# Sin3DM/Sin3DM

Hardware: AMD Instinct MI355X
Metric: DDPM-1000 triplane samples/sec @128^2 latent (higher is better)
Workload: dtype f32; 1 GPU; BASELINE configs[1]: 128^2 triplane (H,W,D)=(128,128,128), 128-ch TriplaneUNetModelSmall, DDPM-1000, batch 1 per GPU; a step = 1 denoising step; batch_per_gpu=1, parallelism=1 independent samples, prewarm_steps=150

## Files before the change

include/sin3dm_hip.h:

```cpp
#ifndef SIN3DM_HIP_H
#define SIN3DM_HIP_H

#include <stddef.h>
#include <stdint.h>

#ifdef __cplusplus
extern "C" {
#endif

#define S3D_ABI_VERSION 13
#define S3D_API __attribute__((visibility("default")))

typedef enum {
    S3D_OK = 0,
    S3D_ERR_INVALID = -1,
    S3D_ERR_MISSING = -2,
    S3D_ERR_HIP = -3,
    S3D_ERR_UNSUPPORTED = -4,
    S3D_ERR_INTERNAL = -5
} s3d_status;

S3D_API int s3d_abi_version(void);

S3D_API int s3d_set_option(const char* name, const char* value);
S3D_API int s3d_get_option(const char* name, int* value);
S3D_API int s3d_set_riders(int on);
S3D_API const char* s3d_last_error(void);
S3D_API int s3d_device_count(void);

typedef struct s3d_unet s3d_unet;

typedef struct {
    int32_t in_channels;
    int32_t model_channels;
    int32_t out_channels;
    int32_t num_res_blocks;
    int32_t n_levels;
    int32_t channel_mult[8];
    int32_t use_scale_shift_norm;
    int32_t is_rollout;
} s3d_unet_cfg;

S3D_API int s3d_unet_create(const s3d_unet_cfg* cfg, s3d_unet** out);
S3D_API void s3d_unet_destroy(s3d_unet* m);

S3D_API int s3d_unet_num_params(const s3d_unet* m);
S3D_API int s3d_unet_param_info(const s3d_unet* m, int i, const char** name, int64_t shape[4], int* ndim);

S3D_API int s3d_unet_set_param(s3d_unet* m, const char* name, const float* data, const int64_t* shape, int ndim);

S3D_API int s3d_unet_forward(s3d_unet* m, const float* x, const float* t, int B, int H, int W, int D,
                     float* out, void* stream);

S3D_API int s3d_unet_film_width(const s3d_unet* m);

#define S3D_MAX_LANES 16
S3D_API int s3d_unet_select_lane(s3d_unet* m, int lane);
S3D_API int s3d_unet_current_lane(const s3d_unet* m);
S3D_API int s3d_unet_film(s3d_unet* m, const float* t, int n, float* film, void* stream);
S3D_API int s3d_unet_forward_film(s3d_unet* m, const float* x, const float* film, int film_stride, int B, int H, int W, int D,
                          float* out, void* stream);

#define S3D_PROF_CLASSES 4
typedef struct {
    double ms[S3D_PROF_CLASSES];
    double flops[S3D_PROF_CLASSES];
    int64_t launches[S3D_PROF_CLASSES];
    int64_t forwards;
    double mfma_flops[S3D_PROF_CLASSES];
} s3d_profile;
S3D_API int s3d_unet_profile(s3d_unet* m, int every);
S3D_API int s3d_unet_profile_classes(s3d_unet* m, int mask);
S3D_API int s3d_unet_profile_read(s3d_unet* m, s3d_profile* out);
S3D_API const char* s3d_unet_profile_kernel(const s3d_unet* m, int cls);
enum { S3D_TAB_SQRT_RECIP = 0, S3D_TAB_SQRT_RECIPM1, S3D_TAB_COEF1, S3D_TAB_COEF2, S3D_TAB_LOGVAR,
       S3D_TAB_ACP, S3D_TAB_ACP_PREV, S3D_TAB_ROWS };
enum { S3D_STEP_DDPM = 0, S3D_STEP_DDIM = 1, S3D_STEP_MEAN_ONLY = 2 };
enum { S3D_MEAN_START_X = 0, S3D_MEAN_EPSILON = 1 };

typedef struct {
    int32_t mode;
    int32_t mean_type;
    int32_t clip_denoised;
    int32_t is_mask_t0;
    float eta;
    int32_t T;
    int64_t batch;
    int64_t per_sample;
    const float* model_out;
    const float* x;
    const float* noise;
    const int64_t* t;
    const float* tables;
    const float* y0;
    const float* mask;
    float* sample;
    float* pred_xstart;
    float* mean;
} s3d_sampler_args;

S3D_API int s3d_sampler_step(const s3d_sampler_args* a, void* stream);

S3D_API int s3d_unet_step_film(s3d_unet* m, const float* film, int film_stride, int B, int H, int W, int D,
                       const s3d_sampler_args* step, float* model_out, void* stream);
enum { S3D_CARRY_OUT = 1, S3D_CARRY_IN = 2 };
S3D_API int s3d_unet_step_film_carry(s3d_unet* m, const float* film, int film_stride, int B, int H, int W, int D,
                       const s3d_sampler_args* step, float* model_out, void* stream, int carry_flags);

enum { S3D_KTAB_SQRT_ACP_PREV = 0, S3D_KTAB_SQRT_1M_ACP_PREV, S3D_KTAB_SQRT_1M_BETA, S3D_KTAB_SQRT_BETA, S3D_KTAB_ROWS };
typedef struct {
    const float* y0;
    const float* mask;
    const float* noise;
    const float* tables;
} s3d_known_region;
S3D_API int s3d_sampler_step_known(const s3d_sampler_args* a, const s3d_known_region* known, void* stream);
S3D_API int s3d_unet_step_film_known(s3d_unet* m, const float* film, int film_stride, int B, int H, int W, int D,
                       const s3d_sampler_args* step, const s3d_known_region* known, float* model_out, void* stream, int carry_flags);
S3D_API int s3d_sampler_renoise(const float* x_prev, const float* noise, const float* known_tables, const int64_t* t, int32_t T,
                       int64_t batch, int64_t per_sample, float* x_t, void* stream);

S3D_API int s3d_op_triplane_conv(const float* const in[3], float* const out[3], int B, int C, int H, int W, int D,
                         int Cout, int ksize, int is_rollout, const float* const weight[3],
                         const float* const bias[3], void* stream);
S3D_API int s3d_op_triplane_norm_silu(const float* const in[3], float* const out[3], int B, int C, int H, int W, int D,
                              const float* const gamma[3], const float* const beta[3], void* stream);
S3D_API int s3d_op_triplane_resample(const float* const in[3], float* const out[3], int B, int C, const int hi[3],
                             const int wi[3], const int ho[3], const int wo[3], int mode, void* stream);
S3D_API int s3d_op_timestep_embed(const float* t, int B, int dim, float* out, void* stream);
S3D_API int s3d_op_triplane_resblock(const float* const in[3], float* const out[3], const float* emb, int B, int C,
                             int Cout, int H, int W, int D, int emb_dim, int use_scale_shift_norm, int is_rollout,
                             const char* const* names, const float* const* tensors, int n_tensors, void* stream);

typedef struct s3d_decoder s3d_decoder;

typedef struct {
    int32_t geo_feat_channels;
    int32_t tex_feat_channels;
    int32_t feat_channel_up;
    int32_t mlp_hidden_channels;
    int32_t mlp_hidden_layers;
    int32_t tex_channels;
} s3d_decoder_cfg;

S3D_API int s3d_decoder_create(const s3d_decoder_cfg* cfg, s3d_decoder** out);
S3D_API int s3d_decoder_create_variant(const s3d_decoder_cfg* cfg, int32_t variant, s3d_decoder** out);
S3D_API int s3d_decoder_out_channels(const s3d_decoder* d);
S3D_API void s3d_decoder_destroy(s3d_decoder* d);
S3D_API int s3d_decoder_num_params(const s3d_decoder* d);
S3D_API int s3d_decoder_param_info(const s3d_decoder* d, int i, const char** name, int64_t shape[4], int* ndim);
S3D_API int s3d_decoder_set_param(s3d_decoder* d, const char* name, const float* data, const int64_t* shape, int ndim);
S3D_API int s3d_decoder_prepare_triplane(s3d_decoder* d, const float* xy, const float* xz, const float* yz,
                                 int H, int W, int D, void* stream);
S3D_API int s3d_decoder_plane_features(s3d_decoder* d, int group, int plane, float* out, void* stream);
S3D_API int s3d_decoder_decode_points(s3d_decoder* d, const float* pts, int64_t N, const float aabb[6],
                              int clamp_color, float* out, void* stream);
S3D_API int s3d_decoder_grid_dims(const float aabb[6], int reso, int dims[3]);
S3D_API int s3d_decoder_decode_grid(s3d_decoder* d, int reso, const float aabb[6], float* out, void* stream);
S3D_API int s3d_decoder_sdf_grad(s3d_decoder* d, const float* pts, int64_t N, const float aabb[6], int iters, float max_step,
                         float max_move, float* pts_out, float* sdf, float* grad, void* stream);

S3D_API int64_t s3d_unet_param_numel(const s3d_unet* m);
S3D_API int s3d_unet_param_offset(const s3d_unet* m, int index, int64_t* offset);
S3D_API int s3d_unet_train_attach(s3d_unet* m, float* params, int64_t numel);
S3D_API int s3d_unet_repack(s3d_unet* m, void* stream);
S3D_API int s3d_unet_forward_train(s3d_unet* m, const float* x, const float* t, int B, int H, int W, int D, float* out,
                                   void* stream);
S3D_API int s3d_unet_backward(s3d_unet* m, const float* d_out, float* grads, void* stream);
S3D_API int s3d_unet_backward_marked(s3d_unet* m, const float* d_out, float* grads, void* stream, void** events, int n_events);

S3D_API int s3d_train_q_sample(const float* x0, int64_t x0_batch_stride, const float* noise, const float* sqrt_ac,
                               const float* sqrt_1mac, const int64_t* t, int B, int64_t per_sample, float* x_t, void* stream);
S3D_API int s3d_train_mse_terms(const float* model_out, const float* target, int64_t target_batch_stride, int B, int C, int H,
                                int W, int D, float* workspace, float* terms, void* stream);
S3D_API int s3d_train_mse_grad(const float* model_out, const float* target, int64_t target_batch_stride, const float* weight,
                               int weight_cols, float weight_divisor, int B, int C, int H, int W, int D, float* d_out,
                               void* stream);
S3D_API int s3d_train_adamw_ema(float* params, const float* grads, float* exp_avg, float* exp_avg_sq, float* const* ema,
                                const float* ema_rates, int n_ema, int64_t numel, float lr, float beta1, float beta2,
// ... 179 lines not shown
```

sin3dm_amd/_lib.py:

```python
from __future__ import annotations

import ctypes as C
import os

_HERE = os.path.dirname(os.path.abspath(__file__))
LIB_PATH = os.path.join(_HERE, "libsin3dm_hip.so")

c_fp = C.POINTER(C.c_float)
c_i64p = C.POINTER(C.c_int64)

ABI_VERSION = 13
TAB_ROWS = ("sqrt_recip", "sqrt_recipm1", "coef1", "coef2", "logvar", "acp", "acp_prev")
KTAB_ROWS = ("sqrt_acp_prev", "sqrt_1m_acp_prev", "sqrt_1m_beta", "sqrt_beta")
STEP_DDPM, STEP_DDIM, STEP_MEAN_ONLY = 0, 1, 2
CARRY_OUT, CARRY_IN = 1, 2
MEAN_START_X, MEAN_EPSILON = 0, 1
ERR_INVALID, ERR_MISSING, ERR_HIP, ERR_UNSUPPORTED, ERR_INTERNAL = -1, -2, -3, -4, -5
MAX_LANES = 16
MESHSDF_MAX_PAIRS = 1 << 27
RENDER_MAX_PAIRS = 1 << 27
RENDER_TILE, RENDER_SUBPIXEL, RENDER_MAX_COORD, RENDER_MAX_GRID = 16, 256, 1 << 20, 4096
IMGFEAT_INCEPTION, IMGFEAT_ALEXNET = 0, 1
RENDER_AMBIENT, RENDER_DIFFUSE = 0.35, 0.65
RENDER_MAX_LIGHTS, RENDER_PBR_MAX_MATERIALS, RENDER_MIN_ROUGHNESS = 4, 16, 0.089
RENDER_RIG_INTENSITY, RENDER_PBR_AMBIENT = 0.5, 0.1
RENDER_PASSES = ("shaded", "albedo", "metallic", "roughness", "normal", "geo")


class UNetCfg(C.Structure):
    _fields_ = [("in_channels", C.c_int32), ("model_channels", C.c_int32), ("out_channels", C.c_int32),
                ("num_res_blocks", C.c_int32), ("n_levels", C.c_int32), ("channel_mult", C.c_int32 * 8),
                ("use_scale_shift_norm", C.c_int32), ("is_rollout", C.c_int32)]


class SamplerArgs(C.Structure):
    _fields_ = [("mode", C.c_int32), ("mean_type", C.c_int32), ("clip_denoised", C.c_int32),
                ("is_mask_t0", C.c_int32), ("eta", C.c_float), ("T", C.c_int32), ("batch", C.c_int64),
                ("per_sample", C.c_int64), ("model_out", C.c_void_p), ("x", C.c_void_p), ("noise", C.c_void_p),
                ("t", C.c_void_p), ("tables", C.c_void_p), ("y0", C.c_void_p), ("mask", C.c_void_p),
                ("sample", C.c_void_p), ("pred_xstart", C.c_void_p), ("mean", C.c_void_p)]


class KnownRegionArgs(C.Structure):
    _fields_ = [("y0", C.c_void_p), ("mask", C.c_void_p), ("noise", C.c_void_p), ("tables", C.c_void_p)]


PROF_CLASSES = 4


class Profile(C.Structure):
    _fields_ = [("ms", C.c_double * PROF_CLASSES), ("flops", C.c_double * PROF_CLASSES), ("launches", C.c_int64 * PROF_CLASSES),
                ("forwards", C.c_int64), ("mfma_flops", C.c_double * PROF_CLASSES)]


class AeLossCfg(C.Structure):
    _fields_ = [("sdf_loss", C.c_int32), ("tex_loss", C.c_int32), ("sdf_threshold", C.c_float),
                ("tex_threshold_ratio", C.c_float), ("tex_weight", C.c_float)]


class DecoderCfg(C.Structure):
    _fields_ = [("geo_feat_channels", C.c_int32), ("tex_feat_channels", C.c_int32), ("feat_channel_up", C.c_int32),
                ("mlp_hidden_channels", C.c_int32), ("mlp_hidden_layers", C.c_int32), ("tex_channels", C.c_int32)]


SIGNATURES = {
    "s3d_abi_version": (C.c_int, []),
    "s3d_last_error": (C.c_char_p, []),
    "s3d_device_count": (C.c_int, []),
    "s3d_set_option": (C.c_int, [C.c_char_p, C.c_char_p]),
    "s3d_get_option": (C.c_int, [C.c_char_p, C.POINTER(C.c_int)]),
    "s3d_set_riders": (C.c_int, [C.c_int]),
    "s3d_unet_create": (C.c_int, [C.POINTER(UNetCfg), C.POINTER(C.c_void_p)]),
    "s3d_unet_destroy": (None, [C.c_void_p]),
    "s3d_unet_num_params": (C.c_int, [C.c_void_p]),
    "s3d_unet_param_info": (C.c_int, [C.c_void_p, C.c_int, C.POINTER(C.c_char_p), c_i64p, C.POINTER(C.c_int)]),
    "s3d_unet_set_param": (C.c_int, [C.c_void_p, C.c_char_p, C.c_void_p, c_i64p, C.c_int]),
    "s3d_unet_forward": (C.c_int, [C.c_void_p, C.c_void_p, C.c_void_p, C.c_int, C.c_int, C.c_int, C.c_int,
                                   C.c_void_p, C.c_void_p]),
    "s3d_unet_film_width": (C.c_int, [C.c_void_p]),
    "s3d_unet_film": (C.c_int, [C.c_void_p, C.c_void_p, C.c_int, C.c_void_p, C.c_void_p]),
    "s3d_unet_select_lane": (C.c_int, [C.c_void_p, C.c_int]),
    "s3d_unet_current_lane": (C.c_int, [C.c_void_p]),
    "s3d_unet_forward_film": (C.c_int, [C.c_void_p, C.c_void_p, C.c_void_p, C.c_int, C.c_int, C.c_int, C.c_int, C.c_int,
                                        C.c_void_p, C.c_void_p]),
    "s3d_unet_profile": (C.c_int, [C.c_void_p, C.c_int]),
    "s3d_unet_profile_classes": (C.c_int, [C.c_void_p, C.c_int]),
    "s3d_unet_profile_read": (C.c_int, [C.c_void_p, C.POINTER(Profile)]),
    "s3d_unet_profile_kernel": (C.c_char_p, [C.c_void_p, C.c_int]),
    "s3d_sampler_step": (C.c_int, [C.POINTER(SamplerArgs), C.c_void_p]),
    "s3d_unet_step_film": (C.c_int, [C.c_void_p, C.c_void_p, C.c_int, C.c_int, C.c_int, C.c_int, C.c_int,
                                     C.POINTER(SamplerArgs), C.c_void_p, C.c_void_p]),
    "s3d_unet_step_film_carry": (C.c_int, [C.c_void_p, C.c_void_p, C.c_int, C.c_int, C.c_int, C.c_int, C.c_int,
                                           C.POINTER(SamplerArgs), C.c_void_p, C.c_void_p, C.c_int]),
    "s3d_sampler_step_known": (C.c_int, [C.POINTER(SamplerArgs), C.POINTER(KnownRegionArgs), C.c_void_p]),
    "s3d_unet_step_film_known": (C.c_int, [C.c_void_p, C.c_void_p, C.c_int, C.c_int, C.c_int, C.c_int, C.c_int,
                                           C.POINTER(SamplerArgs), C.POINTER(KnownRegionArgs), C.c_void_p, C.c_void_p, C.c_int]),
    "s3d_sampler_renoise": (C.c_int, [C.c_void_p, C.c_void_p, C.c_void_p, C.c_void_p, C.c_int32, C.c_int64, C.c_int64, C.c_void_p,
                                      C.c_void_p]),
    "s3d_op_triplane_conv": (C.c_int, [C.POINTER(C.c_void_p), C.POINTER(C.c_void_p), C.c_int, C.c_int, C.c_int,
                                       C.c_int, C.c_int, C.c_int, C.c_int, C.c_int, C.POINTER(C.c_void_p),
                                       C.POINTER(C.c_void_p), C.c_void_p]),
    "s3d_op_triplane_norm_silu": (C.c_int, [C.POINTER(C.c_void_p), C.POINTER(C.c_void_p), C.c_int, C.c_int, C.c_int,
                                            C.c_int, C.c_int, C.POINTER(C.c_void_p), C.POINTER(C.c_void_p),
                                            C.c_void_p]),
    "s3d_op_triplane_resample": (C.c_int, [C.POINTER(C.c_void_p), C.POINTER(C.c_void_p), C.c_int, C.c_int,
                                           C.POINTER(C.c_int), C.POINTER(C.c_int), C.POINTER(C.c_int),
                                           C.POINTER(C.c_int), C.c_int, C.c_void_p]),
    "s3d_op_timestep_embed": (C.c_int, [C.c_void_p, C.c_int, C.c_int, C.c_void_p, C.c_void_p]),
    "s3d_op_triplane_resblock": (C.c_int, [C.POINTER(C.c_void_p), C.POINTER(C.c_void_p), C.c_void_p, C.c_int, C.c_int,
                                           C.c_int, C.c_int, C.c_int, C.c_int, C.c_int, C.c_int, C.c_int,
                                           C.POINTER(C.c_char_p), C.POINTER(C.c_void_p), C.c_int, C.c_void_p]),
    "s3d_decoder_create": (C.c_int, [C.POINTER(DecoderCfg), C.POINTER(C.c_void_p)]),
    "s3d_decoder_create_variant": (C.c_int, [C.POINTER(DecoderCfg), C.c_int32, C.POINTER(C.c_void_p)]),
    "s3d_decoder_out_channels": (C.c_int, [C.c_void_p]),
    "s3d_decoder_plane_features": (C.c_int, [C.c_void_p, C.c_int, C.c_int, C.c_void_p, C.c_void_p]),
    "s3d_decoder_destroy": (None, [C.c_void_p]),
    "s3d_decoder_num_params": (C.c_int, [C.c_void_p]),
    "s3d_decoder_param_info": (C.c_int, [C.c_void_p, C.c_int, C.POINTER(C.c_char_p), c_i64p, C.POINTER(C.c_int)]),
    "s3d_decoder_set_param": (C.c_int, [C.c_void_p, C.c_char_p, C.c_void_p, c_i64p, C.c_int]),
    "s3d_decoder_prepare_triplane": (C.c_int, [C.c_void_p, C.c_void_p, C.c_void_p, C.c_void_p, C.c_int, C.c_int,
                                               C.c_int, C.c_void_p]),
    "s3d_decoder_decode_points": (C.c_int, [C.c_void_p, C.c_void_p, C.c_int64, c_fp, C.c_int, C.c_void_p,
                                            C.c_void_p]),
    "s3d_decoder_sdf_grad": (C.c_int, [C.c_void_p, C.c_void_p, C.c_int64, c_fp, C.c_int, C.c_float, C.c_float, C.c_void_p,
                                       C.c_void_p, C.c_void_p, C.c_void_p]),
    "s3d_decoder_grid_dims": (C.c_int, [c_fp, C.c_int, C.POINTER(C.c_int)]),
    "s3d_decoder_decode_grid": (C.c_int, [C.c_void_p, C.c_int, c_fp, C.c_void_p, C.c_void_p]),
    "s3d_mc_create": (C.c_int, [C.POINTER(C.c_void_p)]),
    "s3d_mc_destroy": (None, [C.c_void_p]),
    "s3d_mc_count": (C.c_int, [C.c_void_p, C.c_void_p, C.c_int, C.c_int, C.c_int, C.c_int, C.c_float, C.c_int, C.c_float,
                               c_i64p, c_i64p, C.c_void_p]),
    "s3d_mc_extract": (C.c_int, [C.c_void_p, C.c_void_p, C.c_void_p, C.c_int, C.c_void_p, C.c_void_p]),
    "s3d_mesh_components": (C.c_int, [C.c_void_p, C.c_int64, C.c_int64, C.c_void_p, C.c_void_p]),
    "s3d_mesh_cluster_keys": (C.c_int, [C.c_void_p, C.c_int64, c_fp, C.c_float, C.POINTER(C.c_int), C.c_void_p, C.c_void_p]),
    "s3d_mesh_cluster_means": (C.c_int, [C.c_void_p, C.c_int, C.c_void_p, C.c_void_p, C.c_int64, C.c_int64, C.c_void_p, C.c_void_p]),
    "s3d_mesh_remap_faces": (C.c_int, [C.c_void_p, C.c_int64, C.c_void_p, C.c_int64, C.c_int64, C.c_void_p, C.c_void_p, C.c_void_p]),
    "s3d_tex_face_corner0": (C.c_int, [C.c_void_p, C.c_int64, C.c_void_p, C.c_int64, C.c_void_p, C.c_void_p]),
    "s3d_tex_texel_positions": (C.c_int, [C.c_void_p, C.c_int64, C.c_void_p, C.c_void_p, C.c_int64, C.c_int, C.c_int, C.c_int,
                                          C.c_void_p, C.c_void_p, C.c_void_p]),
    "s3d_tex_quantize": (C.c_int, [C.c_void_p, C.c_void_p, C.c_int64, C.c_int, C.c_int, C.c_void_p, C.c_void_p]),
    "s3d_tex_dilate": (C.c_int, [C.c_void_p, C.c_void_p, C.c_int, C.c_int, C.c_void_p, C.c_void_p]),
    "s3d_mesh_qem_quadrics": (C.c_int, [C.c_void_p, C.c_int64, C.c_void_p, C.c_int64, C.c_void_p, C.c_void_p, C.c_void_p, C.c_void_p]),
    "s3d_mesh_qem_edge_cost": (C.c_int, [C.c_void_p, C.c_int64, C.c_void_p, C.c_void_p, C.c_void_p, C.c_int64, C.c_void_p, C.c_void_p,
                                         C.c_void_p]),
    "s3d_mesh_qem_edge_valid": (C.c_int, [C.c_void_p, C.c_int64, C.c_void_p, C.c_int64, C.c_void_p, C.c_void_p, C.c_void_p, C.c_int64,
                                          C.c_void_p, C.c_void_p, C.c_int64, C.c_void_p, C.c_void_p, C.c_void_p, C.c_void_p, C.c_void_p,
                                          C.c_void_p]),
    "s3d_mesh_qem_select": (C.c_int, [C.c_void_p, C.c_void_p, C.c_void_p, C.c_void_p, C.c_int64, C.c_void_p, C.c_void_p, C.c_int64,
                                      C.c_int64, C.c_void_p, C.c_void_p, C.c_void_p, C.c_void_p, C.c_void_p]),
    "s3d_mesh_qem_apply": (C.c_int, [C.c_void_p, C.c_int64, C.c_void_p, C.c_void_p, C.c_int64, C.c_void_p, C.c_void_p, C.c_int64,
                                     C.c_void_p, C.c_void_p, C.c_int, C.c_void_p, C.c_void_p]),
    "s3d_mesh_qem_remap_faces": (C.c_int, [C.c_void_p, C.c_int64, C.c_void_p, C.c_int64, C.c_void_p, C.c_void_p, C.c_void_p]),
    "s3d_meshsdf_bin_count": (C.c_int, [C.c_void_p, C.c_int64, C.c_float, c_fp, C.c_float, C.POINTER(C.c_int), C.c_void_p, C.c_void_p]),
    "s3d_meshsdf_bin_fill": (C.c_int, [C.c_void_p, C.c_int64, C.c_float, c_fp, C.c_float, C.POINTER(C.c_int), C.c_void_p, C.c_int64,
                                       C.c_void_p, C.c_void_p, C.c_void_p]),
    "s3d_meshsdf_closest": (C.c_int, [C.c_void_p, C.c_int64, C.c_void_p, C.c_int64, C.c_float, c_fp, C.c_float, C.POINTER(C.c_int),
                                      C.c_void_p, C.c_void_p, C.c_int64, C.c_void_p, C.c_void_p, C.c_void_p, C.c_void_p]),
    "s3d_meshsdf_winding": (C.c_int, [C.c_void_p, C.c_int64, C.c_void_p, C.c_int64, C.c_void_p, C.c_void_p]),
    "s3d_meshsdf_face_areas": (C.c_int, [C.c_void_p, C.c_int64, C.c_void_p, C.c_void_p]),
    "s3d_meshsdf_sample_surface": (C.c_int, [C.c_void_p, C.c_int64, C.c_void_p, C.c_void_p, C.c_int64, C.c_void_p, C.c_void_p,
                                             C.c_void_p, C.c_void_p]),
    "s3d_meshsdf_texture": (C.c_int, [C.c_void_p, C.c_void_p, C.c_int64, C.c_void_p, C.c_void_p, C.c_int64, C.c_void_p, C.c_void_p,
                                      C.c_int, C.c_void_p, C.c_int64, C.c_void_p, C.c_void_p]),
    "s3d_meshsdf_texture_pbr": (C.c_int, [C.c_void_p, C.c_void_p, C.c_int64, C.c_void_p, C.c_void_p, C.c_int64, C.c_void_p, C.c_void_p,
                                          C.c_int, C.c_void_p, C.c_int64, C.c_void_p, C.c_void_p]),
    "s3d_eval_pool_or": (C.c_int, [C.c_void_p, C.POINTER(C.c_int), C.POINTER(C.c_int), C.c_void_p, C.c_void_p]),
    "s3d_eval_patch_counts": (C.c_int, [C.POINTER(C.c_int), C.c_int, C.c_int, C.POINTER(C.c_int)]),
    "s3d_eval_patch_valid": (C.c_int, [C.c_void_p, C.POINTER(C.c_int), C.c_int, C.c_int, C.c_void_p, C.c_void_p]),
    "s3d_eval_pack_patches": (C.c_int, [C.c_void_p, C.POINTER(C.c_int), C.c_int, C.c_int, C.c_void_p, C.c_int64, C.c_int, C.c_void_p,
                                        C.c_void_p, C.c_void_p]),
    "s3d_eval_lp_max": (C.c_int, [C.c_void_p, C.c_void_p, C.c_int64, C.c_void_p, C.c_void_p, C.c_int64, C.c_int, C.c_void_p, C.c_void_p,
                                  C.c_void_p]),
    "s3d_eval_pack_volumes": (C.c_int, [C.c_void_p, C.c_int64, C.c_int64, C.c_void_p, C.c_void_p]),
    "s3d_eval_pairwise_counts": (C.c_int, [C.c_void_p, C.c_int64, C.c_int64, C.c_void_p, C.c_void_p, C.c_void_p]),
    "s3d_ssfid_create": (C.c_int, [C.POINTER(C.c_void_p)]),
    "s3d_ssfid_destroy": (None, [C.c_void_p]),
    "s3d_ssfid_set_param": (C.c_int, [C.c_void_p, C.c_char_p, C.c_void_p, c_i64p, C.c_int]),
    "s3d_ssfid_out_dims": (C.c_int, [C.POINTER(C.c_int), C.c_int, C.POINTER(C.c_int), C.POINTER(C.c_int)]),
    "s3d_ssfid_features": (C.c_int, [C.c_void_p, C.c_void_p, C.POINTER(C.c_int), C.c_int, C.c_void_p, C.c_void_p, C.c_void_p, C.c_void_p]),
    "s3d_ssfid_profile": (C.c_int, [C.c_void_p, C.c_int]),
    "s3d_ssfid_profile_read": (C.c_int, [C.c_void_p, C.POINTER(C.c_double)]),
    "s3d_imgfeat_create": (C.c_int, [C.c_int, C.POINTER(C.c_void_p)]),
    "s3d_imgfeat_destroy": (None, [C.c_void_p]),
    "s3d_imgfeat_set_param": (C.c_int, [C.c_void_p, C.c_char_p, C.c_void_p, c_i64p, C.c_int]),
    "s3d_imgfeat_out_dims": (C.c_int, [C.c_int, C.c_int, C.c_int, C.c_int, C.POINTER(C.c_int), C.POINTER(C.c_int), C.POINTER(C.c_int)]),
    "s3d_imgfeat_features": (C.c_int, [C.c_void_p, C.c_void_p, C.c_int, C.c_int, C.c_int, C.c_int, C.c_int, C.POINTER(C.c_void_p),
                                       C.c_void_p]),
    "s3d_imgfeat_stats": (C.c_int, [C.c_void_p, C.c_void_p, C.c_void_p, C.c_void_p]),
    "s3d_imgfeat_pairs": (C.c_int, [C.c_void_p, C.c_void_p, C.c_void_p, C.c_void_p]),
    "s3d_imgfeat_profile": (C.c_int, [C.c_void_p, C.c_int]),
    "s3d_imgfeat_profile_read": (C.c_int, [C.c_void_p, C.POINTER(C.c_double)]),
    "s3d_render_project": (C.c_int, [C.c_void_p, C.c_int64, c_fp, C.c_int, C.c_int, C.c_float, C.c_void_p, C.c_void_p, C.c_void_p]),
    "s3d_render_bin_count": (C.c_int, [C.c_void_p, C.c_void_p, C.c_int64, C.c_void_p, C.c_int64, C.c_int, C.c_int, C.c_void_p, C.c_void_p,
                                       C.c_void_p]),
    "s3d_render_bin_fill": (C.c_int, [C.c_void_p, C.c_void_p, C.c_int64, C.c_void_p, C.c_int64, C.c_int, C.c_int, C.c_void_p, C.c_int64,
                                      C.c_void_p, C.c_void_p, C.c_void_p]),
    "s3d_render_raster": (C.c_int, [C.c_void_p, C.c_void_p, C.c_int64, C.c_void_p, C.c_int64, C.c_int, C.c_int, C.c_void_p, C.c_void_p,
                                    C.c_int64, C.c_void_p, C.c_void_p, C.c_void_p, C.c_void_p]),
    "s3d_render_shade": (C.c_int, [C.c_void_p, C.c_void_p, C.c_void_p, C.c_int64, C.c_void_p, C.c_int64, C.c_void_p, C.c_int, C.c_int, C.c_int,
                                   c_fp, c_fp, C.c_void_p, C.c_void_p, C.c_void_p, C.c_void_p, C.c_void_p, C.c_int, C.c_void_p, C.c_int64,
                                   C.c_void_p, C.c_void_p]),
    "s3d_pbr_vertex_normals": (C.c_int, [C.c_void_p, C.c_int64, C.c_void_p, C.c_int64, C.c_void_p, C.c_void_p, C.c_void_p, C.c_void_p]),
    "s3d_pbr_face_tangents": (C.c_int, [C.c_void_p, C.c_int64, C.c_void_p, C.c_int64, C.c_void_p, C.c_void_p, C.c_void_p]),
    "s3d_pbr_shade": (C.c_int, [C.c_void_p, C.c_void_p, C.c_void_p, C.c_int64, C.c_void_p, C.c_int64, C.c_void_p, C.c_int, C.c_int, C.c_int,
                                       c_fp, C.c_void_p, C.c_void_p, C.c_void_p, C.c_void_p, C.c_void_p, C.c_int, C.c_void_p, C.c_int64,
                                       C.c_void_p, C.c_void_p, c_i64p, c_fp, c_fp, c_fp, C.c_int, C.c_float, C.c_int, C.c_void_p, C.c_void_p]),
    "s3d_rng_create": (C.c_int, [C.POINTER(C.c_void_p)]),
    "s3d_rng_destroy": (None, [C.c_void_p]),
    "s3d_rng_set_state": (C.c_int, [C.c_void_p, C.POINTER(C.c_uint32), C.c_int, C.c_void_p]),
    "s3d_rng_get_state": (C.c_int, [C.c_void_p, C.POINTER(C.c_uint32), C.POINTER(C.c_int), C.c_void_p]),
    "s3d_rng_reserve": (C.c_int, [C.c_void_p, C.c_int64]),
    "s3d_rng_randn": (C.c_int, [C.c_void_p, C.c_void_p, C.c_int64, C.c_int, C.c_void_p]),
    "s3d_rng_rand": (C.c_int, [C.c_void_p, C.c_void_p, C.c_int64, C.c_void_p]),
    "s3d_ae_create": (C.c_int, [C.POINTER(DecoderCfg), C.POINTER(C.c_void_p)]),
    "s3d_ae_create_variant": (C.c_int, [C.POINTER(DecoderCfg), C.c_int32, C.POINTER(C.c_void_p)]),
    "s3d_ae_out_channels": (C.c_int, [C.c_void_p]),
    "s3d_ae_destroy": (None, [C.c_void_p]),
    "s3d_ae_num_params": (C.c_int, [C.c_void_p]),
    "s3d_ae_param_info": (C.c_int, [C.c_void_p, C.c_int, C.POINTER(C.c_char_p), c_i64p, C.POINTER(C.c_int), c_i64p]),
    "s3d_ae_param_numel": (C.c_int64, [C.c_void_p, c_i64p]),
    "s3d_ae_attach": (C.c_int, [C.c_void_p, C.c_void_p, C.c_int64]),
    "s3d_ae_repack": (C.c_int, [C.c_void_p, C.c_void_p]),
    "s3d_ae_set_volume": (C.c_int, [C.c_void_p, C.c_void_p, C.c_int, C.c_int, C.c_int, C.c_int, C.c_void_p]),
    "s3d_ae_encode": (C.c_int, [C.c_void_p, C.c_void_p, C.c_void_p, C.c_void_p, C.c_void_p]),
    "s3d_ae_forward": (C.c_int, [C.c_void_p, C.c_void_p, C.c_int64, c_fp, C.c_void_p, C.c_void_p]),
    "s3d_ae_loss_grads": (C.c_int, [C.c_void_p, C.c_void_p, C.c_void_p, C.c_void_p, C.c_int64, c_fp, C.POINTER(AeLossCfg),
                                    C.c_void_p, C.c_void_p, C.c_void_p, C.c_void_p]),
    "s3d_ae_loss_grads_groups": (C.c_int, [C.c_void_p, C.c_void_p, C.c_void_p, C.c_void_p, C.c_int64, c_fp, C.POINTER(AeLossCfg),
                                           C.c_void_p, C.c_void_p, C.c_void_p, C.c_void_p]),
    "s3d_unet_param_numel": (C.c_int64, [C.c_void_p]),
    "s3d_unet_param_offset": (C.c_int, [C.c_void_p, C.c_int, c_i64p]),
    "s3d_unet_train_attach": (C.c_int, [C.c_void_p, C.c_void_p, C.c_int64]),
    "s3d_unet_repack": (C.c_int, [C.c_void_p, C.c_void_p]),
    "s3d_unet_forward_train": (C.c_int, [C.c_void_p, C.c_void_p, C.c_void_p, C.c_int, C.c_int, C.c_int, C.c_int,
                                         C.c_void_p, C.c_void_p]),
    "s3d_unet_backward": (C.c_int, [C.c_void_p, C.c_void_p, C.c_void_p, C.c_void_p]),
    "s3d_unet_backward_marked": (C.c_int, [C.c_void_p, C.c_void_p, C.c_void_p, C.c_void_p, C.POINTER(C.c_void_p), C.c_int]),
    "s3d_train_q_sample": (C.c_int, [C.c_void_p, C.c_int64, C.c_void_p, C.c_void_p, C.c_void_p, C.c_void_p, C.c_int, C.c_int64,
                                     C.c_void_p, C.c_void_p]),
    "s3d_train_mse_terms": (C.c_int, [C.c_void_p, C.c_void_p, C.c_int64, C.c_int, C.c_int, C.c_int, C.c_int, C.c_int, C.c_void_p,
                                      C.c_void_p, C.c_void_p]),
    "s3d_train_mse_grad": (C.c_int, [C.c_void_p, C.c_void_p, C.c_int64, C.c_void_p, C.c_int, C.c_float, C.c_int, C.c_int, C.c_int,
                                     C.c_int, C.c_int, C.c_void_p, C.c_void_p]),
    "s3d_train_adamw_ema": (C.c_int, [C.c_void_p, C.c_void_p, C.c_void_p, C.c_void_p, C.POINTER(C.c_void_p), c_fp, C.c_int,
                                      C.c_int64, C.c_float, C.c_float, C.c_float, C.c_float, C.c_float, C.c_int,
                                      C.c_void_p]),
}

_lib = None


class Sin3DMHipError(RuntimeError):
    pass


def load():
    global _lib
    if _lib is not None:
        return _lib
    if not os.path.exists(LIB_PATH):
        raise ImportError(
            f"{LIB_PATH} is missing: build it with `python -c 'import __graft_entry__ as g; g.build()'` or "
            f"`make -C sin3dm_amd/csrc`. sin3dm_amd has no CPU fallback.")
    lib = C.CDLL(LIB_PATH)
    for name, (res, args) in SIGNATURES.items():
        fn = getattr(lib, name)
        fn.restype = res
        fn.argtypes = args
    v = lib.s3d_abi_version()
    if v != ABI_VERSION:
        raise ImportError(f"libsin3dm_hip.so ABI {v} != binding ABI {ABI_VERSION}")
    _lib = lib
    return lib


def last_error():
    return (load().s3d_last_error() or b"").decode(errors="replace")


def check(rc):
    if rc == 0:
        return
    msg = last_error()
    if rc == ERR_INVALID:
        raise AssertionError(msg)
    if rc == ERR_MISSING:
        raise RuntimeError("Error(s) in loading state_dict: " + msg)
    if rc == ERR_UNSUPPORTED:
        raise NotImplementedError(msg)
    raise Sin3DMHipError(msg)


def require_gpu(t=None):
    import torch
    if t is not None and not t.is_cuda:
        raise Sin3DMHipError("sin3dm_amd runs on an MI355X: tensor is on %s and there is no CPU fallback" % t.device)
    if not torch.cuda.is_available():
        raise Sin3DMHipError("sin3dm_amd needs a visible MI355X (torch.cuda.is_available() is False); "
                             "there is no CPU fallback")


def set_option(name, value):
    check(load().s3d_set_option(str(name).encode(), None if value is None else str(value).encode()))


def get_option(name):
    v = C.c_int(0)
    check(load().s3d_get_option(str(name).encode(), C.byref(v)))
    return None if v.value == -1 else v.value


def set_riders(on):
    check(load().s3d_set_riders(1 if on else 0))


def stream_ptr():
    import torch
    return C.c_void_p(torch.cuda.current_stream().cuda_stream)


def ptr(t):
    return C.c_void_p(t.data_ptr()) if t is not None else C.c_void_p(0)


def ptr3(ts):
    return (C.c_void_p * 3)(*[C.c_void_p(t.data_ptr()) for t in ts])
```

sin3dm_amd/csrc/s3d_common.h:

```cpp
#pragma once
#include <hip/hip_runtime.h>

#include <atomic>
#include <cstdarg>
#include <cstdint>
#include <cstdio>
#include <cstring>
#include <map>
#include <string>
#include <vector>

#include "../../include/sin3dm_hip.h"

namespace s3d {

void set_error(const char* fmt, ...) __attribute__((format(printf, 1, 2)));
const char* get_error();

#define S3D_HIP(call)                                                                              \
    do {                                                                                           \
        hipError_t e__ = (call);                                                                   \
        if (e__ != hipSuccess) {                                                                   \
            s3d::set_error("%s failed: %s (%s:%d)", #call, hipGetErrorString(e__), __FILE__, __LINE__); \
            return S3D_ERR_HIP;                                                                    \
        }                                                                                          \
    } while (0)

#define S3D_CHECK(cond, code, ...)                                                                 \
    do {                                                                                           \
        if (!(cond)) {                                                                             \
            s3d::set_error(__VA_ARGS__);                                                           \
            return (code);                                                                         \
        }                                                                                          \
    } while (0)

#define S3D_TRY(expr)                                                                              \
    do {                                                                                           \
        int rc__ = (expr);                                                                         \
        if (rc__ != 0) return rc__;                                                                \
    } while (0)

inline int ensure_dynamic_lds(const void* kernel, int bytes, std::atomic<unsigned long long>& opted) {
    int dev = 0;
    S3D_HIP(hipGetDevice(&dev));
    const unsigned long long bit = dev >= 0 && dev < 64 ? 1ull << dev : 0ull;
    if (bit && (opted.load(std::memory_order_acquire) & bit)) return 0;
    S3D_HIP(hipFuncSetAttribute(kernel, hipFuncAttributeMaxDynamicSharedMemorySize, bytes));
    if (bit) opted.fetch_or(bit, std::memory_order_release);
    return 0;
}

struct DevBuf {
    void* p = nullptr;
    size_t cap = 0;
    int reserve(size_t bytes);
    void release();
    ~DevBuf() { release(); }
    DevBuf() = default;
    DevBuf(const DevBuf&) = delete;
    DevBuf& operator=(const DevBuf&) = delete;
};

struct Arena {
    DevBuf buf;
    size_t off = 0, high = 0;
    size_t peak = 0;
    bool measuring = false;
    void reset() { off = 0; }
    template <class T>
    T* alloc(size_t n) {
        size_t bytes = (n * sizeof(T) + 255) & ~size_t(255);
        size_t o = off;
        off += bytes;
        if (off > high) high = off;
        if (off > peak) peak = off;
        if (measuring) return reinterpret_cast<T*>(uintptr_t(256));
        return reinterpret_cast<T*>(static_cast<char*>(buf.p) + o);
    }
};

int upload(DevBuf& dst, const void* host, size_t bytes);
int workspace_overrun(const char* what, size_t run_peak, size_t measured);

enum Opt { OPT_WINO = 0, OPT_WINO24W, OPT_VCAT, OPT_WGRAD_WINO, OPT_RANK1_SLICES, OPT_RANK1_BATCH, OPT_CONV_IMPL, OPT_CONV1X1_T,
           OPT_GN_FUSED, OPT_BWD_SIDE, OPT_GNB_FUSED, OPT_EDGE_SIGNAL, OPT_COUNT };
constexpr const char* kOptNames[] = {"WINO", "WINO24W", "VCAT", "WGRAD_WINO", "RANK1_SLICES", "RANK1_BATCH", "CONV_IMPL", "CONV1X1_T",
                                     "GN_FUSED", "BWD_SIDE", "GNB_FUSED", "EDGE_SIGNAL"};
static_assert(sizeof kOptNames / sizeof kOptNames[0] == OPT_COUNT, "one name per option");
constexpr int kOptUnset = -1;
int opt(Opt o);
long long opt_generation();
inline bool opt_on(Opt o) { return opt(o) != 0; }
bool riders_enabled();
int device_cus();

struct Geo {
    int h[3], w[3];
    static Geo from_hwd(int H, int W, int D) { return Geo{{H, H, W}, {W, D, D}}; }
    Geo half() const { return Geo{{h[0] / 2, h[1] / 2, h[2] / 2}, {w[0] / 2, w[1] / 2, w[2] / 2}}; }
    Geo twice() const { return Geo{{h[0] * 2, h[1] * 2, h[2] * 2}, {w[0] * 2, w[1] * 2, w[2] * 2}}; }
    bool operator==(const Geo& o) const {
        for (int i = 0; i < 3; ++i) if (h[i] != o.h[i] || w[i] != o.w[i]) return false;
        return true;
    }
    size_t pixels() const { return size_t(h[0]) * w[0] + size_t(h[1]) * w[1] + size_t(h[2]) * w[2]; }
};

struct GnPartials { double* p; int maxparts; int nparts[3]; int nsub; };
struct Tri {
    float* p[3] = {nullptr, nullptr, nullptr};
    int C = 0;
    Geo g{};
    float* gn = nullptr;
    GnPartials part{nullptr, 0, {0, 0, 0}, 0};
};

struct ConvJob {
    const float* in;
    const float* wgt;
    const float* wgt_wino;
    const float* wgt_wino24s;
    const float* wgt_r1f;
    const float* bias;
    const float* bbias;
    const float* rrow;
    const float* rcol;
    const float* res;
    int res_up;
    float* out;
    int h, w;
    int bbias_stride;
    double* gn_part;
    int tiles_x, tiles_per_img, n_tiles_n;
    int block_begin;
};
constexpr int kMaxConvJobs = 8;
struct GnbArgs {
    const float* x[3];
    const float* rowadd[3]; const float* coladd[3];
    float rowscale[3], colscale[3];
    const float* gamma[3]; const float* beta[3];
    const float* mr;
    const float* film; int film_stride;
    int groups;
};
struct ConvArgs {
    ConvJob job[kMaxConvJobs];
    int njobs;
    int B, cin, cout;
    int gn_sg, gn_nsub, gn_maxparts;
    int relu;
    int xcd_swizzle;
    int r1_slices;
    const GnbArgs* gnb;
};
enum ConvKind { CONV_3x3 = 0, CONV_1x1 = 1, CONV_1x3_VEC = 2, CONV_5x5 = 3, CONV_1x3_ROLL = 4 };
struct GnFinArgs {
    const double* part; float* mr;
    int maxparts, nparts[3], nsub, subs_per_group;
    double count[3];
};
struct GnPartUpArgs {
    const float* u[3];
    int hi[3], wi[3];
    int C, cq, pl, sg, nsub, maxparts;
    double* part;
};
struct GnFinCatArgs {
    const double* pu; const double* ps; float* mr;
    int maxparts_u, maxparts_s, nparts_u[3], nparts_s[3], nsub_u, nsub_s, subs_per_group;
    double count[3];
};
enum RiderKind { RIDER_NONE = 0, RIDER_GN_PARTIALS_UP, RIDER_GN_FINALIZE, RIDER_GN_FINALIZE_CAT };
struct ConvRider {
    int kind;
    int n_blocks;
    int gx;
    union { GnPartUpArgs up; GnFinArgs fin; GnFinCatArgs cat; };
};
constexpr int kRiderLdsBytes = 16384;
int launch_conv(ConvKind kind, ConvArgs& a, hipStream_t st, const ConvRider* rider = nullptr);
bool conv1x1_takes_rider(const Geo& g, int B, int cout);
int launch_conv_naive(ConvKind kind, ConvArgs& a, hipStream_t st);
bool conv_use_naive();
void conv_note_kernel(const char* name);
const char* conv_last_kernel();
double conv_exec_fraction(ConvKind kind, const ConvArgs& a);

struct ConvW {
    size_t dense[3] = {0, 0, 0};
    size_t bias[3] = {0, 0, 0};
    size_t rrow[3] = {0, 0, 0};
    size_t rcol[3] = {0, 0, 0};
    size_t rrow_f[3] = {0, 0, 0};
    size_t rcol_f[3] = {0, 0, 0};
    size_t wino[3] = {0, 0, 0};
    size_t wino24s[3] = {0, 0, 0};
    int cin = 0, cout = 0, k = 0;
    bool rollout = false;
    bool only24_current = false;
};
size_t push(std::vector<float>& stage, const float* src, size_t n);
__host__ __device__ inline size_t rank1_frag_index(int cin, int tap, int o, int co, int c) {
    const int g = co >> 5, i = co & 31, chunk = c >> 7, cc = c & 127, w = cc >> 5, k8 = (cc >> 3) & 3, half = (cc >> 2) & 1, e = cc & 3;
    const size_t step = size_t(g * 4 + w) * (cin / 128 * 12) + chunk * 12 + tap * 4 + k8;
    return ((step * 3 + o) * 64 + half * 32 + i) * 4 + e;
}
inline size_t rank1_frag_floats(int cin, int cout) { return size_t((cout + 31) / 32) * cin * 288; }
void pack_tconv_raw(std::vector<float>& stage, const float* const W[3], const float* const bias[3], int cin, int cout,
                    int k, bool roll, ConvW& cw);

int launch_nchw_to_nhwc(const float* in, float* out, int B, int C, int h, int w, hipStream_t st);
int launch_nhwc_to_nchw(const float* in, float* out, int B, int C, int h, int w, hipStream_t st);

struct GnPartials;
bool in_conv_gn_parts(const Geo& g, int Cin, int Cout, int nparts[3]);
int launch_in_conv(const float* x, int B, int Cin, int H, int W, int D, const float* wT, const float* bias,
                   int Cout, Tri& out, hipStream_t st, const GnPartials* part = nullptr);

constexpr int kGnChunks = 256;
struct GnStats { float* mr; };
inline int gn_subgroup(int C) {
    int cg = C / 32, sg = 1;
    while (sg < 32 && cg % (sg * 2) == 0) sg *= 2;
    return sg;
}
int launch_gn_partials(const Tri& x, int B, GnPartials out, hipStream_t st);
int launch_gn_finalize(const GnPartials& part, const Geo& g, int C, int B, GnStats out, hipStream_t st);
bool gn_finalize_rider(const GnPartials& part, const Geo& g, int C, int B, GnStats out, ConvRider& r);
bool gn_partials_up_rider(const Tri& u, int B, int sg, GnPartials out, ConvRider& r);
bool gn_finalize_cat_rider(const GnPartials& pu, const GnPartials& ps, const Geo& g, int C, int B, GnStats out, ConvRider& r);
void gn_up_parts(const Geo& out_g, int nparts[3]);
int launch_gn_partials_up(const Tri& u, int B, int sg, GnPartials out, hipStream_t st);
int launch_gn_finalize_cat(const GnPartials& pu, const GnPartials& ps, const Geo& g, int C, int B, GnStats out, hipStream_t st);
void conv_gn_parts(ConvKind kind, const Geo& g, int nparts[3], bool wino24 = false);
bool conv_use_wino();
void wino_gn_parts(const Geo& g, int nparts[3]);
size_t pack_wino_weights(std::vector<float>& stage, const float* W, int cout, int ctot, int cin);
int launch_conv_wino(ConvArgs& a, hipStream_t st);
double wino_exec_fraction();
bool conv_use_wino24();
bool conv_wino24_channels(int cin, int cout);
size_t wino24_packed_floats(int cout, int cin);
size_t pack_wino24s_weights(std::vector<float>& stage, const float* W, int cout, int ctot, int cin);
int launch_conv_wino24s(ConvArgs& a, hipStream_t st);
int launch_conv_wino24_narrow(ConvArgs& a, hipStream_t st);
int launch_conv_wino24_wide(ConvArgs& a, hipStream_t st);

struct ActArgs {
    const float* gamma[3];
    const float* beta[3];
    const float* film;
    int film_stride;
};
constexpr int kActRows = 8, kActCols = 8;
struct MeanPartials {
    float* rowpart[3];
    float* colpart[3];
};
int launch_gn_act(const Tri& x, int B, GnStats stats, const ActArgs& a, Tri& y, const MeanPartials* mp,
                  hipStream_t st, const GnPartials* stats_part = nullptr);
bool gn_act_can_add_parts(const GnPartials& part, int C);
bool gn_parts_in_consumer(long long consumer_blocks);
int gn_act_threads(int C);
long long gn_act_blocks(const Geo& g, int B);
int launch_gn_finalize_as(const GnPartials& part, const Geo& g, int C, int B, int threads, GnStats out, hipStream_t st);
int launch_gn_act_cat(const Tri& u, const Tri& sk, int B, GnStats stats, const ActArgs& a, Tri& y, const MeanPartials* mp,
                      hipStream_t st);
struct MeanVecs { float* rowmean[3]; float* colmean[3]; };
struct MeanFinArgs {
    const float* src[6];
    float* dst[6];
    int len[6], nt[6];
    float inv[6];
    int C, cq, B;
};
MeanFinArgs means_finalize_args(const Geo& g, int C, int B, const MeanPartials& mp, const MeanVecs& mv);
int launch_means_finalize(const Geo& g, int C, int B, const MeanPartials& mp, MeanVecs mv, hipStream_t st);

int conv_rank1_slices(int cin);

int launch_avgpool(const Tri& x, int B, Tri& y, hipStream_t st, const GnPartials* part = nullptr);
int launch_bilinear(const float* in, int B, int C, int hi, int wi, float* out, int ho, int wo, int out_cstride,
                    int out_coff, hipStream_t st);
bool upcat_gn_parts(const Geo& out_g, int C, int nparts[3]);
int launch_upcat(const Tri& u, const Tri& sk, int B, Tri& out, hipStream_t st, const GnPartials* part = nullptr);
int launch_copy_slice(const float* in, int B, int C, int h, int w, float* out, int out_cstride, int out_coff,
                      hipStream_t st);

struct InConvCarry { const float* wT; const float* bias; float* out[3]; double* part; int maxparts, Cin; };
int launch_out_head(const Tri& x, int B, GnStats stats, const ActArgs& a, const float* w ,
                    const float* bias , int Cout, int H, int W, int D, float* out, hipStream_t st,
                    const s3d_sampler_args* fuse = nullptr, const GnPartials* part = nullptr, const InConvCarry* carry = nullptr,
                    const s3d_known_region* known = nullptr);
bool out_head_can_carry(int C, int Cin, int Cout_head);
bool out_head_fuses_sampler(int C, int Cout, int B);
bool out_head_px_takes(int C, int Cout);
bool out_head_adds_parts(const GnPartials& part, int C, int Cout);
long long out_head_px_blocks(const Geo& g, int B);

int launch_linear(const float* in, int B, int I, const float* W, const float* bias, int O, float* out,
                  int in_mode, int out_silu, hipStream_t st);

int launch_sampler(const s3d_sampler_args& a, hipStream_t st);
int launch_sampler_known(const s3d_sampler_args& a, const s3d_known_region& kr, hipStream_t st);
int launch_renoise(const float* xprev, const float* er, const float* ktab, const int64_t* t, int T, long long batch, long long per_sample,
                   float* xt, hipStream_t st);

}
```

sin3dm_amd/csrc/s3d_conv.hip:

```cpp
#include "s3d_common.h"
#include "s3d_rank1.h"
#include "s3d_riders.h"

namespace s3d {

typedef float f32x16 __attribute__((ext_vector_type(16)));

#ifndef S3D_ABLATE
#define S3D_ABLATE 0
#endif
constexpr int KC = 32;
constexpr int LDP = KC + 4;

__device__ __forceinline__ float up2x_blend(float ly0, float ly1, float lx0, float lx1, float v00, float v01, float v10, float v11) {
    const float top = __fmaf_rn(lx1, v01, __fmul_rn(lx0, v00));
    const float bot = __fmaf_rn(lx1, v11, __fmul_rn(lx0, v10));
    return __fmaf_rn(ly1, bot, __fmul_rn(ly0, top));
}

template <int TH_, int TW_, int KH_, int KW_, int WM_, int WN_, int MTW_, int NTW_, int KS_ = 1, int PF_ = 0, bool TR_ = false>
struct ConvCfg {
    static constexpr int KS = KS_;
    static constexpr int PF = PF_;
    static constexpr bool TR = TR_;
    static constexpr int TH = TH_, TW = TW_, KH = KH_, KW = KW_, WM = WM_, WN = WN_, MTW = MTW_, NTW = NTW_;
    static constexpr int BM = TH * TW, BN = WN * NTW * 32;
    static constexpr int HH = TH + KH - 1, HW = TW + KW - 1;
    static constexpr int A_ELEMS = HH * HW * LDP, B_ELEMS = BN * LDP;
    static constexpr int A_ITEMS = HH * HW * (KC / 4), B_ITEMS = BN * (KC / 4);
    static constexpr int NA = (A_ITEMS + 255) / 256, NB = (B_ITEMS + 255) / 256;
    static_assert(WM * WN == 4, "4 waves per block");
    static_assert(BM == WM * MTW * 32, "pixel tile must match the wave grid");
    static_assert(32 % TW == 0 || TW % 32 == 0, "an MFMA row block must cover whole tile rows");
};

typedef float f32x4 __attribute__((ext_vector_type(4)));
typedef const f32x4 __attribute__((address_space(1)))* gf4ptr;
__device__ __forceinline__ gf4ptr to_global4(const float* p) { return (gf4ptr)(uintptr_t)p; }

__device__ __forceinline__ int edge_variant(int idx, int n) {
    return n == 1 ? 3 : (idx == 0 ? 1 : (idx == n - 1 ? 2 : 0));
}

template <bool RIDER> struct RiderArg {};
template <> struct RiderArg<true> { ConvRider r; };
template <class CFG, bool RIDER = false>
__global__ __launch_bounds__(256) void k_conv_mfma(ConvArgs args, RiderArg<RIDER> rider) {
    constexpr int TW = CFG::TW, KH = CFG::KH, KW = CFG::KW, MTW = CFG::MTW, NTW = CFG::NTW;
    constexpr int HW = CFG::HW, TAPS = KH * KW;
    __shared__ __attribute__((aligned(16))) float smem[2 * (CFG::A_ELEMS + CFG::B_ELEMS)];
    float* const Abase = smem;
    float* const Bbase = smem + 2 * CFG::A_ELEMS;

    int bid = blockIdx.x;
    int nblocks = gridDim.x;
    if constexpr (RIDER) {
        static_assert(sizeof smem >= size_t(kRiderLdsBytes) && KH == 1 && !CFG::TR, "the rider bodies work in the 1x1 convolution's LDS");
        if (bid < rider.r.n_blocks) { run_rider(rider.r, bid, smem); return; }
        bid -= rider.r.n_blocks; nblocks -= rider.r.n_blocks;
    }
    if (args.xcd_swizzle) {
        const int chunk = nblocks >> 3;
        if (bid < (chunk << 3)) bid = (bid & 7) * chunk + (bid >> 3);
    }
    int j = 0;
#pragma unroll
    for (int k = 1; k < kMaxConvJobs; ++k) j += (k < args.njobs && bid >= args.job[k].block_begin) ? 1 : 0;
    const ConvJob& J = args.job[j];
    int local = bid - J.block_begin;
    const int ntile = local % J.n_tiles_n; local /= J.n_tiles_n;
    const int b = local / J.tiles_per_img; local %= J.tiles_per_img;
    const int ty0 = (local / J.tiles_x) * CFG::TH, tx0 = (local % J.tiles_x) * TW;
    const int n0 = ntile * CFG::BN;
    const int h = J.h, w = J.w, cin = args.cin, cout = args.cout;

    const int tid = threadIdx.x, lane = tid & 63, wid = tid >> 6;
    const int wm = wid / CFG::WN, wn = wid % CFG::WN;

    int offA[MTW], offB[NTW];
#pragma unroll
    for (int mt = 0; mt < MTW; ++mt) {
        const int p = (wm * MTW + mt) * 32 + (lane & 31);
        offA[mt] = ((p / TW) * HW + (p % TW)) * LDP + (lane >> 5) * 4;
    }
#pragma unroll
    for (int nt = 0; nt < NTW; ++nt) offB[nt] = ((wn * NTW + nt) * 32 + (lane & 31)) * LDP + (lane >> 5) * 4;

    gf4ptr aSrc[CFG::NA]; int aDst[CFG::NA]; bool aOk[CFG::NA];
#pragma unroll
    for (int it = 0; it < CFG::NA; ++it) {
        const int idx = min(it * 256 + tid, CFG::A_ITEMS - 1);
        const int pix = idx >> 3, q = idx & 7;
        const int gy = ty0 + pix / HW - KH / 2, gx = tx0 + pix % HW - KW / 2;
        aOk[it] = gy >= 0 && gy < h && gx >= 0 && gx < w;
        aDst[it] = pix * LDP + q * 4;
        aSrc[it] = to_global4(J.in + ((size_t(b) * h + (aOk[it] ? gy : 0)) * w + (aOk[it] ? gx : 0)) * cin + q * 4);
    }
    gf4ptr bSrc[CFG::NB]; int bDst[CFG::NB]; bool bOk[CFG::NB];
#pragma unroll
    for (int it = 0; it < CFG::NB; ++it) {
        const int idx = min(it * 256 + tid, CFG::B_ITEMS - 1);
        const int n = idx >> 3, q = idx & 7;
        bOk[it] = n0 + n < cout;
        bDst[it] = n * LDP + q * 4;
        bSrc[it] = to_global4(J.wgt + size_t(bOk[it] ? n0 + n : 0) * cin + q * 4);
    }
    const size_t tapStride4 = size_t(cout) * cin / 4;

    constexpr int KS = CFG::KS;
    f32x16 acc[KS][MTW][NTW];
#pragma unroll
    for (int ks = 0; ks < KS; ++ks)
#pragma unroll
        for (int mt = 0; mt < MTW; ++mt)
#pragma unroll
            for (int nt = 0; nt < NTW; ++nt)
#pragma unroll
                for (int r = 0; r < 16; ++r) acc[ks][mt][nt][r] = 0.f;

    const int nchunks = cin / KC;
    f32x4 ra[CFG::NA], rb[CFG::NB];
    const f32x4 zero4 = {0.f, 0.f, 0.f, 0.f};

#pragma unroll
    for (int it = 0; it < CFG::NA; ++it) { ra[it] = aSrc[it][0]; if (!aOk[it]) ra[it] = zero4; }
#pragma unroll
    for (int it = 0; it < CFG::NB; ++it) { rb[it] = bSrc[it][0]; if (!bOk[it]) rb[it] = zero4; }
#pragma unroll
    for (int it = 0; it < CFG::NA; ++it) *reinterpret_cast<f32x4*>(Abase + aDst[it]) = ra[it];
#pragma unroll
    for (int it = 0; it < CFG::NB; ++it) *reinterpret_cast<f32x4*>(Bbase + bDst[it]) = rb[it];
    __syncthreads();

    if constexpr (TAPS == 1 && CFG::PF > 0) {
        constexpr int PF = CFG::PF;
        f32x4 qa[PF][CFG::NA], qb[PF][CFG::NB];
#pragma unroll
        for (int d = 0; d < PF; ++d) {
            const int ch = min(1 + d, nchunks - 1);
#pragma unroll
            for (int it = 0; it < CFG::NA; ++it) qa[d][it] = aSrc[it][ch * (KC / 4)];
#pragma unroll
            for (int it = 0; it < CFG::NB; ++it) qb[d][it] = bSrc[it][ch * (KC / 4)];
        }
        for (int c0 = 0; c0 < nchunks; c0 += PF) {
#pragma unroll
            for (int d = 0; d < PF; ++d) {
                const int chunk = c0 + d;
                if (chunk < nchunks) {
                    const float* As = Abase + (chunk & 1) * CFG::A_ELEMS;
                    const float* Bs = Bbase + (chunk & 1) * CFG::B_ELEMS;
#pragma unroll
                    for (int k8 = 0; k8 < KC / 8; ++k8) {
                        f32x4 a4[MTW], b4[NTW];
#pragma unroll
                        for (int mt = 0; mt < MTW; ++mt) a4[mt] = *reinterpret_cast<const f32x4*>(As + offA[mt] + k8 * 8);
#pragma unroll
                        for (int nt = 0; nt < NTW; ++nt) b4[nt] = *reinterpret_cast<const f32x4*>(Bs + offB[nt] + k8 * 8);
#pragma unroll
                        for (int e = 0; e < 4; ++e)
#pragma unroll
                            for (int mt = 0; mt < MTW; ++mt)
#pragma unroll
                                for (int nt = 0; nt < NTW; ++nt)
                                    acc[(k8 * 4 + e) % KS][mt][nt] = CFG::TR ? __builtin_amdgcn_mfma_f32_32x32x2f32(b4[nt][e], a4[mt][e], acc[(k8 * 4 + e) % KS][mt][nt], 0, 0, 0)
                                                                             : __builtin_amdgcn_mfma_f32_32x32x2f32(a4[mt][e], b4[nt][e], acc[(k8 * 4 + e) % KS][mt][nt], 0, 0, 0);
                    }
                    if (chunk + 1 < nchunks) {
                        float* Ad = Abase + ((chunk + 1) & 1) * CFG::A_ELEMS;
                        float* Bd = Bbase + ((chunk + 1) & 1) * CFG::B_ELEMS;
#pragma unroll
                        for (int it = 0; it < CFG::NA; ++it) if (!(S3D_ABLATE & 2)) *reinterpret_cast<f32x4*>(Ad + aDst[it]) = aOk[it] ? qa[d][it] : zero4; else asm volatile("" :: "v"(qa[d][it]));
#pragma unroll
                        for (int it = 0; it < CFG::NB; ++it) if (!(S3D_ABLATE & 2)) *reinterpret_cast<f32x4*>(Bd + bDst[it]) = bOk[it] ? qb[d][it] : zero4; else asm volatile("" :: "v"(qb[d][it]));
                        const int ch = min(chunk + 1 + PF, nchunks - 1);
                        if (chunk + 1 + PF < nchunks) {
#pragma unroll
                            for (int it = 0; it < CFG::NA; ++it) qa[d][it] = aSrc[it][ch * (KC / 4)];
#pragma unroll
                            for (int it = 0; it < CFG::NB; ++it) qb[d][it] = bSrc[it][ch * (KC / 4)];
                        }
                    }
                    __syncthreads();
                }
            }
        }
    } else
    for (int chunk = 0; chunk < nchunks; ++chunk) {
        const int nch = min(chunk + 1, nchunks - 1);
#pragma unroll
        for (int it = 0; it < CFG::NA; ++it) if (!(S3D_ABLATE & 1)) ra[it] = aSrc[it][nch * (KC / 4)];
#pragma unroll
        for (int tap = 0; tap < TAPS; ++tap) {
            constexpr int kLast = TAPS - 1;
            const int ntap = tap == kLast ? 0 : tap + 1;
            const int bch = tap == kLast ? nch : chunk;
#pragma unroll
            for (int it = 0; it < CFG::NB; ++it) if (!(S3D_ABLATE & 1)) rb[it] = bSrc[it][ntap * tapStride4 + bch * (KC / 4)];
            __builtin_amdgcn_sched_barrier(0);
            const int stage = chunk * TAPS + tap;
            const float* As = Abase + (chunk & 1) * CFG::A_ELEMS + ((tap / KW) * HW + (tap % KW)) * LDP;
            const float* Bs = Bbase + (stage & 1) * CFG::B_ELEMS;
#pragma unroll
            for (int k8 = 0; k8 < KC / 8; ++k8) {
                f32x4 a4[MTW], b4[NTW];
#pragma unroll
                for (int mt = 0; mt < MTW; ++mt)
                    a4[mt] = (S3D_ABLATE & 8) ? ra[0] + float(k8) : *reinterpret_cast<const f32x4*>(As + offA[mt] + k8 * 8);
#pragma unroll
                for (int nt = 0; nt < NTW; ++nt)
                    b4[nt] = (S3D_ABLATE & 8) ? rb[0] + float(k8) : *reinterpret_cast<const f32x4*>(Bs + offB[nt] + k8 * 8);
#pragma unroll
                for (int e = 0; e < 4; ++e)
#pragma unroll
                    for (int mt = 0; mt < MTW; ++mt)
#pragma unroll
                        for (int nt = 0; nt < NTW; ++nt) {
                            constexpr int dummy = 0; (void)dummy;
                            const int ks = (k8 * 4 + e) % KS;
                            acc[ks][mt][nt] = __builtin_amdgcn_mfma_f32_32x32x2f32(a4[mt][e], b4[nt][e], acc[ks][mt][nt], 0, 0, 0);
                        }
            }
            __builtin_amdgcn_sched_barrier(0);
            float* Bd = Bbase + ((stage + 1) & 1) * CFG::B_ELEMS;
// ... 95 lines not shown
        for (int mt = 0; mt < MTW; ++mt)
#pragma unroll
        for (int rh = 0; rh < 2; ++rh) {
            float addv[8];
            bool ok[8];
            unsigned oidx[8];
            const size_t plane0 = size_t(b) * h * w * cout;
#pragma unroll
            for (int rr = 0; rr < 8; ++rr) {
                const int r = rh * 8 + rr;
                const int p = (wm * MTW + mt) * 32 + (r & 3) + 8 * (r >> 2) + 4 * (lane >> 5);
                const int y = ty0 + p / TW, x = tx0 + p % TW;
                ok[rr] = y < h && x < w && co_ok;
                oidx[rr] = ok[rr] ? unsigned(y * w + x) * unsigned(cout) + unsigned(co) : 0u;
                addv[rr] = base;
            }
            if (p_rcol) {
#pragma unroll
                for (int rr = 0; rr < 8; ++rr) {
                    const int r = rh * 8 + rr;
                    const int p = (wm * MTW + mt) * 32 + (r & 3) + 8 * (r >> 2) + 4 * (lane >> 5);
                    const int y = ty0 + p / TW, x = tx0 + p % TW;
                    const float t = p_rcol[ok[rr] ? ((size_t(b) * w + x) * 4 + edge_variant(y, h)) * cout + co : 0];
                    addv[rr] += ok[rr] ? t : 0.f;
                }
            }
            if (p_rrow) {
#pragma unroll
                for (int rr = 0; rr < 8; ++rr) {
                    const int r = rh * 8 + rr;
                    const int p = (wm * MTW + mt) * 32 + (r & 3) + 8 * (r >> 2) + 4 * (lane >> 5);
                    const int y = ty0 + p / TW, x = tx0 + p % TW;
                    const float t = p_rrow[ok[rr] ? ((img + y) * 4 + edge_variant(x, w)) * cout + co : 0];
                    addv[rr] += ok[rr] ? t : 0.f;
                }
            }
            if (p_res && !J.res_up) {
#pragma unroll
                for (int rr = 0; rr < 8; ++rr) addv[rr] += p_res[plane0 + oidx[rr]];
            }
            if (p_res && J.res_up) {
                const int hi = h >> 1, wi = w >> 1;
                const float* rb = p_res + size_t(b) * hi * wi * cout + coc;
#pragma unroll
                for (int rr = 0; rr < 8; ++rr) {
                    const int r = rh * 8 + rr;
                    const int p = (wm * MTW + mt) * 32 + (r & 3) + 8 * (r >> 2) + 4 * (lane >> 5);
                    const int y = min(ty0 + p / TW, h - 1), x = min(tx0 + p % TW, w - 1);
                    float fy = 0.5f * (float(y) + 0.5f) - 0.5f; fy = fy < 0.f ? 0.f : fy;
                    float fx = 0.5f * (float(x) + 0.5f) - 0.5f; fx = fx < 0.f ? 0.f : fx;
                    int y0 = int(fy); y0 = y0 > hi - 1 ? hi - 1 : y0;
                    int x0 = int(fx); x0 = x0 > wi - 1 ? wi - 1 : x0;
                    const int y1 = y0 + (y0 < hi - 1 ? 1 : 0), x1 = x0 + (x0 < wi - 1 ? 1 : 0);
                    const float ly1 = fy - float(y0), ly0 = 1.f - ly1, lx1 = fx - float(x0), lx0 = 1.f - lx1;
                    const float v00 = rb[(size_t(y0) * wi + x0) * cout], v01 = rb[(size_t(y0) * wi + x1) * cout];
                    const float v10 = rb[(size_t(y1) * wi + x0) * cout], v11 = rb[(size_t(y1) * wi + x1) * cout];
                    addv[rr] += up2x_blend(ly0, ly1, lx0, lx1, v00, v01, v10, v11);
                }
            }
#pragma unroll
            for (int rr = 0; rr < 8; ++rr) {
                const int r = rh * 8 + rr;
                float v = acc[0][mt][nt][r];
#pragma unroll
                for (int ks = 1; ks < KS; ++ks) v += acc[ks][mt][nt][r];
                v += addv[rr];
                if (args.relu) v = fmaxf(v, 0.f);
                if (ok[rr]) {
                    p_out[plane0 + oidx[rr]] = v;
                    gs += v; gss = fmaf(v, v, gss);
                }
            }
        }
        if (p_gn) {
            gs += __shfl_xor(gs, 32, 64); gss += __shfl_xor(gss, 32, 64);
            for (int off = 1; off < args.gn_sg; off <<= 1) { gs += __shfl_xor(gs, off, 64); gss += __shfl_xor(gss, off, 64); }
            if (lane < 32 && co_ok && (co % args.gn_sg) == 0) {
                const int part = tile_idx * CFG::WM + wm;
                double* dst = p_gn + ((size_t(b) * 3 * args.gn_nsub + co / args.gn_sg) * args.gn_maxparts + part) * 2;
                dst[0] = double(gs); dst[1] = double(gss);
            }
        }
    }
}

__global__ void k_conv_naive(ConvArgs args, int KH, int KW) {
    for (int j = 0; j < args.njobs; ++j) {
        const ConvJob& J = args.job[j];
        const long long n = (long long)args.B * J.h * J.w * args.cout;
        for (long long i = (long long)blockIdx.x * blockDim.x + threadIdx.x; i < n; i += (long long)gridDim.x * blockDim.x) {
            const int co = int(i % args.cout);
            long long r = i / args.cout;
            const int x = int(r % J.w); r /= J.w;
            const int y = int(r % J.h);
            const int b = int(r / J.h);
            float acc = 0.f;
            for (int kh = 0; kh < KH; ++kh)
                for (int kw = 0; kw < KW; ++kw) {
                    const int gy = y + kh - KH / 2, gx = x + kw - KW / 2;
                    if (gy < 0 || gy >= J.h || gx < 0 || gx >= J.w) continue;
                    const float* xi = J.in + ((size_t(b) * J.h + gy) * J.w + gx) * args.cin;
                    const float* wr = J.wgt + (size_t(kh * KW + kw) * args.cout + co) * args.cin;
                    for (int c = 0; c < args.cin; ++c) acc = fmaf(xi[c], wr[c], acc);
                }
            float v = acc + (J.bias ? J.bias[co] : 0.f);
            if (J.bbias) v += J.bbias[size_t(b) * J.bbias_stride + co];
            if (J.rcol) v += J.rcol[((size_t(b) * J.w + x) * 4 + edge_variant(y, J.h)) * args.cout + co];
            if (J.rrow) v += J.rrow[((size_t(b) * J.h + y) * 4 + edge_variant(x, J.w)) * args.cout + co];
            if (J.res && !J.res_up) v += J.res[i];
            if (J.res && J.res_up) {
                const int hi = J.h / 2, wi = J.w / 2;
                float fy = 0.5f * (float(y) + 0.5f) - 0.5f; fy = fy < 0.f ? 0.f : fy;
                float fx = 0.5f * (float(x) + 0.5f) - 0.5f; fx = fx < 0.f ? 0.f : fx;
                int y0 = int(fy); y0 = y0 > hi - 1 ? hi - 1 : y0;
                int x0 = int(fx); x0 = x0 > wi - 1 ? wi - 1 : x0;
                const int y1 = y0 + (y0 < hi - 1 ? 1 : 0), x1 = x0 + (x0 < wi - 1 ? 1 : 0);
                const float ly1 = fy - float(y0), ly0 = 1.f - ly1, lx1 = fx - float(x0), lx0 = 1.f - lx1;
                const float* rb = J.res + size_t(b) * hi * wi * args.cout + co;
                v += ly0 * (lx0 * rb[(size_t(y0) * wi + x0) * args.cout] + lx1 * rb[(size_t(y0) * wi + x1) * args.cout]) +
                     ly1 * (lx0 * rb[(size_t(y1) * wi + x0) * args.cout] + lx1 * rb[(size_t(y1) * wi + x1) * args.cout]);
            }
            if (args.relu) v = fmaxf(v, 0.f);
            J.out[i] = v;
        }
    }
}

template <bool ROLL3, int NS = 1>
__global__ __launch_bounds__(256) void k_rank1(ConvArgs args) {
    extern __shared__ __attribute__((aligned(16))) float lds_dyn[];
    __shared__ __attribute__((aligned(16))) float lds_static[NS == 1 ? kR1LdsFloats : 4];
    float* lds = NS == 1 ? lds_static : lds_dyn;
    const int bid = blockIdx.x;
    int j = 0;
#pragma unroll
    for (int k = 1; k < kMaxConvJobs; ++k) j += (k < args.njobs && bid >= args.job[k].block_begin) ? 1 : 0;
    const ConvJob& J = args.job[j];
    int local = bid - J.block_begin;
    R1Block blk;
    const int nsl = ROLL3 && args.r1_slices > 1 ? args.r1_slices : 1;
    const int sl = local % nsl; local /= nsl;
    blk.ntile = local % J.n_tiles_n; local /= J.n_tiles_n;
    blk.b = (local / J.tiles_per_img) * NS; blk.mtile = local % J.tiles_per_img;
    blk.bcount = min(NS, args.B - blk.b);
    blk.vin = J.in; blk.wgt = J.wgt; blk.L = J.w; blk.cin = args.cin; blk.cout4 = args.cout; blk.n_tiles_n = J.n_tiles_n;
    blk.out = J.out + size_t(sl) * args.B * J.w * 4 * args.cout;
    if (nsl > 1) {
        const int nchunks = args.cin / kR1Chunk, first = (nchunks + 1) / 2;
        blk.chunk0 = sl ? first : 0; blk.nch = sl ? nchunks - first : first;
    }
    rank1_block<ROLL3, NS>(blk, lds);
}

constexpr int kR1bLdsFloats = 4 * 48 * 64;
__global__ __launch_bounds__(256) void k_rank1b(ConvArgs args) {
    extern __shared__ __attribute__((aligned(16))) float lds_dyn[];
    int bid = blockIdx.x;
    if ((gridDim.x & 7) == 0) bid = (bid & 7) * int(gridDim.x >> 3) + (bid >> 3);
    int j = 0;
#pragma unroll
    for (int k = 1; k < kMaxConvJobs; ++k) j += (k < args.njobs && bid >= args.job[k].block_begin) ? 1 : 0;
    const ConvJob& J = args.job[j];
    int local = bid - J.block_begin;
    const int L = J.w, cin = args.cin, cout = args.cout, B = args.B;
    const int mtile = local % J.tiles_per_img; local /= J.tiles_per_img;
    const int b = local % B; local /= B;
    const int g = local % J.n_tiles_n, sl = local / J.n_tiles_n;
    const int nchunks = cin / kR1Chunk;
    int chunk0 = 0, nch = nchunks;
    if (args.r1_slices > 1) { const int first = (nchunks + 1) / 2; chunk0 = sl ? first : 0; nch = sl ? nchunks - first : first; }
    const int csl = nch * kR1Chunk, ld = csl + 4;
    const int tid = threadIdx.x, lane = tid & 63, wid = __builtin_amdgcn_readfirstlane(tid >> 6), i = lane & 31, half = lane >> 5;
    const int nsteps = nch * 12;
    const r1_f32x4* pf = reinterpret_cast<const r1_f32x4*>(J.wgt_r1f) + (size_t(g * 4 + wid) * (nchunks * 12) + chunk0 * 12) * 192 + lane;
    constexpr int D = 3;
    r1_f32x4 ring[D][3];
    int pf_s = 0;
    auto prefetch = [&](int slot) {
        ring[slot][0] = ((r1_gf4ptr)(uintptr_t)pf)[0];
        ring[slot][1] = ((r1_gf4ptr)(uintptr_t)(pf + 64))[0];
        ring[slot][2] = ((r1_gf4ptr)(uintptr_t)(pf + 128))[0];
        ++pf_s;
        pf += pf_s < nsteps ? 192 : 0;
    };
#pragma unroll
    for (int d = 0; d < D; ++d) prefetch(d);
    {
        const int q4 = csl / 4, items = 34 * q4;
        const float* vb = J.in + (size_t(b) * L) * cin + chunk0 * kR1Chunk;
        const r1_f32x4 zero4 = {0.f, 0.f, 0.f, 0.f};
        for (int it0 = tid; it0 < items; it0 += 256 * 5) {
            r1_f32x4 v[5];
#pragma unroll
            for (int u = 0; u < 5; ++u) {
                const int it = it0 + 256 * u, row = it / q4, q = it - row * q4, pos = mtile * 32 - 1 + row;
                const bool ok = it < items && pos >= 0 && pos < L;
                v[u] = ((r1_gf4ptr)(uintptr_t)(vb + size_t(ok ? pos : 0) * cin + (ok ? q : 0) * 4))[0];
                if (!ok) v[u] = zero4;
            }
#pragma unroll
            for (int u = 0; u < 5; ++u) {
                const int it = it0 + 256 * u, row = it / q4, q = it - row * q4;
                if (it < items) *reinterpret_cast<r1_f32x4*>(lds_dyn + row * ld + q * 4) = v[u];
            }
        }
    }
    __syncthreads();
    r1_f32x16 q[3];
#pragma unroll
    for (int o = 0; o < 3; ++o)
#pragma unroll
        for (int r = 0; r < 16; ++r) q[o][r] = 0.f;
    const float* Ab = lds_dyn + i * ld + half * 4 + wid * 32;
    for (int ch = 0; ch < nch; ++ch) {
        const float* Ac = Ab + ch * kR1Chunk;
#pragma unroll
        for (int st = 0; st < 12; ++st) {
            const int tap = st >> 2, k8 = st & 3;
            const r1_f32x4 a4 = *reinterpret_cast<const r1_f32x4*>(Ac + tap * ld + k8 * 8);
            r1_f32x4 b4[3];
#pragma unroll
            for (int o = 0; o < 3; ++o) b4[o] = ring[st % D][o];
            __builtin_amdgcn_sched_barrier(0);
#pragma unroll
            for (int e = 0; e < 4; ++e)
#pragma unroll
                for (int o = 0; o < 3; ++o) q[o] = __builtin_amdgcn_mfma_f32_32x32x2f32(a4[e], b4[o][e], q[o], 0, 0, 0);
            __builtin_amdgcn_sched_barrier(0);
            prefetch(st % D);
            __builtin_amdgcn_sched_barrier(0);
        }
    }
    __syncthreads();
    float* red = lds_dyn;
#pragma unroll
    for (int o = 0; o < 3; ++o)
#pragma unroll
        for (int r = 0; r < 16; ++r) red[((wid * 3 + o) * 16 + r) * 64 + lane] = q[o][r];
    __syncthreads();
    float* out = J.out + size_t(sl) * B * L * 4 * cout;
#pragma unroll
    for (int k = 0; k < 4; ++k) {
        const int it = tid + 256 * k, r = it >> 6, l = it & 63;
        float u[3];
#pragma unroll
        for (int o = 0; o < 3; ++o) {
            const float* p = red + (o * 16 + r) * 64 + l;
            u[o] = ((p[0] + p[3 * 1024]) + p[2 * 3 * 1024]) + p[3 * 3 * 1024];
        }
        const int row = mtile * 32 + (r & 3) + 8 * (r >> 2) + 4 * (l >> 5), co = g * 32 + (l & 31);
        if (row < L && co < cout) {
            float* o4 = out + (size_t(b) * L + row) * 4 * cout + co;
            o4[0] = (u[0] + u[1]) + u[2]; o4[cout] = u[1] + u[2]; o4[2 * cout] = u[0] + u[1]; o4[3 * cout] = u[1];
        }
    }
}
bool rank1b_takes(const ConvArgs& a) {
    if (a.cin % kR1Chunk != 0) return false;
    for (int j = 0; j < a.njobs; ++j) if (!a.job[j].wgt_r1f) return false;
    const int nchunks = a.cin / kR1Chunk, maxch = a.r1_slices > 1 ? (nchunks + 1) / 2 : nchunks;
    if (34 * (maxch * kR1Chunk + 4) > kR1bLdsFloats) return false;
    return opt_on(OPT_RANK1_BATCH);
}

int conv_rank1_slices(int cin) {
    return opt_on(OPT_RANK1_SLICES) && cin >= 2 * kR1Chunk && cin % kR1Chunk == 0 ? 2 : 1;
}

__global__ void k_rank1_roll_naive(ConvArgs args) {
    for (int j = 0; j < args.njobs; ++j) {
        const ConvJob& J = args.job[j];
        const int L = J.w, cout = args.cout, cin = args.cin, nt = (cout + 7) / 8;
        const long long n = (long long)args.B * L * cout;
        for (long long i = (long long)blockIdx.x * blockDim.x + threadIdx.x; i < n; i += (long long)gridDim.x * blockDim.x) {
            const int co = int(i % cout), pos = int((i / cout) % L), b = int(i / cout / L);
            float u[3] = {0.f, 0.f, 0.f};
            for (int o = 0; o < 3; ++o)
                for (int t = 0; t < 3; ++t) {
                    const int q = pos + t - 1;
                    if (q < 0 || q >= L) continue;
                    const float* v = J.in + (size_t(b) * L + q) * cin;
                    const float* wr = J.wgt + (size_t(t) * nt * 24 + (co / 8) * 24 + o * 8 + (co & 7)) * cin;
                    for (int c = 0; c < cin; ++c) u[o] = fmaf(v[c], wr[c], u[o]);
                }
            float* o4 = J.out + (size_t(b) * L + pos) * 4 * cout + co;
            o4[0] = (u[0] + u[1]) + u[2]; o4[cout] = u[1] + u[2]; o4[2 * cout] = u[0] + u[1]; o4[3 * cout] = u[1];
        }
    }
}

int launch_rank1(ConvArgs& a, hipStream_t st, bool roll3) {
    S3D_CHECK(a.njobs >= 1 && a.njobs <= kMaxConvJobs && a.cin % KC == 0, S3D_ERR_INVALID, "rank1: bad arguments");
    S3D_CHECK(a.r1_slices <= 1 || (roll3 && !conv_use_naive() && a.r1_slices == 2 && a.cin % kR1Chunk == 0 && a.cin >= 2 * kR1Chunk), S3D_ERR_INVALID, "rank1: two K slices of whole 128-channel chunks");
    if (conv_use_naive()) {
        if (!roll3) return launch_conv_naive(CONV_1x3_VEC, a, st);
        hipLaunchKernelGGL(k_rank1_roll_naive, dim3(512), dim3(256), 0, st, a);
        S3D_HIP(hipGetLastError());
        return 0;
    }
    if (roll3 && rank1b_takes(a)) {
        int blocks = 0;
        for (int j = 0; j < a.njobs; ++j) {
            ConvJob& J = a.job[j];
            J.tiles_x = J.tiles_per_img = (J.w + 31) / 32;
            J.n_tiles_n = (a.cout + 31) / 32;
            J.block_begin = blocks;
            blocks += J.tiles_per_img * a.B * J.n_tiles_n * (a.r1_slices > 1 ? a.r1_slices : 1);
        }
        if (!blocks) return 0;
        conv_note_kernel("k_rank1b (three-tap rollout tables, fragment-order weights)");
        hipLaunchKernelGGL(k_rank1b, dim3(blocks), dim3(256), kR1bLdsFloats * sizeof(float), st, a);
        S3D_HIP(hipGetLastError());
        return 0;
    }
    const bool pair_ok = opt_on(OPT_RANK1_BATCH);
    const int ns = roll3 && pair_ok && a.B >= 2 ? 2 : 1;
    int blocks = 0;
    for (int j = 0; j < a.njobs; ++j) {
        ConvJob& J = a.job[j];
        J.tiles_x = J.tiles_per_img = (J.w + 31) / 32;
        J.n_tiles_n = roll3 ? (a.cout + 7) / 8 : (a.cout + 31) / 32;
        J.block_begin = blocks;
        blocks += J.tiles_per_img * J.n_tiles_n * ((a.B + ns - 1) / ns) * (roll3 && a.r1_slices > 1 ? a.r1_slices : 1);
    }
    if (!blocks) return 0;
    conv_note_kernel(roll3 ? "k_rank1<true> (three-tap rollout tables)" : "k_rank1<false>");
    constexpr size_t lds1 = kR1LdsFloats * sizeof(float), lds2 = lds1 + 34 * kR1Ld * sizeof(float);
    if (ns == 2) {
        static std::atomic<unsigned long long> opted{0};
        S3D_TRY(ensure_dynamic_lds(reinterpret_cast<const void*>(&k_rank1<true, 2>), int(lds2), opted));
        hipLaunchKernelGGL((k_rank1<true, 2>), dim3(blocks), dim3(256), lds2, st, a);
    } else if (roll3) hipLaunchKernelGGL(k_rank1<true>, dim3(blocks), dim3(256), 0, st, a);
    else hipLaunchKernelGGL(k_rank1<false>, dim3(blocks), dim3(256), 0, st, a);
    S3D_HIP(hipGetLastError());
    return 0;
}

void conv_gn_parts(ConvKind kind, const Geo& g, int nparts[3], bool wino24) {
    (void)kind;
    if (wino24 && conv_use_wino24()) {
        for (int p = 0; p < 3; ++p) nparts[p] = ((g.w[p] + 15) / 16) * ((g.h[p] + 7) / 8);
        return;
    }
    if (conv_use_wino()) { wino_gn_parts(g, nparts); return; }
    using CFG = ConvCfg<8, 8, 3, 3, 2, 2, 1, 1>;
    for (int p = 0; p < 3; ++p)
        nparts[p] = ((g.w[p] + CFG::TW - 1) / CFG::TW) * ((g.h[p] + CFG::TH - 1) / CFG::TH) * CFG::WM;
}

static thread_local const char* t_last_kernel = "";
void conv_note_kernel(const char* name) { t_last_kernel = name; }
const char* conv_last_kernel() { return t_last_kernel; }

bool conv_use_naive() {
    return opt(OPT_CONV_IMPL) == 1;
}

static void kind_taps(ConvKind kind, int& KH, int& KW) {
    switch (kind) {
        case CONV_3x3: KH = 3; KW = 3; break;
        case CONV_1x1: KH = 1; KW = 1; break;
        case CONV_1x3_VEC: case CONV_1x3_ROLL: KH = 1; KW = 3; break;
        default: KH = 5; KW = 5; break;
    }
}

int launch_conv_naive(ConvKind kind, ConvArgs& a, hipStream_t st) {
    int KH, KW;
    kind_taps(kind, KH, KW);
    conv_note_kernel("k_conv_naive (one thread per output, S3D_CONV_IMPL=naive)");
    hipLaunchKernelGGL(k_conv_naive, dim3(2048), dim3(256), 0, st, a, KH, KW);
    S3D_HIP(hipGetLastError());
    return 0;
}

static const char* rider_name(int kind) {
    return kind == RIDER_GN_PARTIALS_UP ? "k_conv_mfma<1x1> direct MFMA convolution carrying k_gn_partials_up"
         : kind == RIDER_GN_FINALIZE ? "k_conv_mfma<1x1> direct MFMA convolution carrying k_gn_finalize (plain)"
                                     : "k_conv_mfma<1x1> direct MFMA convolution carrying k_gn_finalize_cat";
}
template <class CFG>
static int launch_cfg(ConvArgs& a, hipStream_t st, const ConvRider* rider = nullptr) {
    int blocks = 0;
    for (int j = 0; j < a.njobs; ++j) {
        ConvJob& J = a.job[j];
        J.tiles_x = (J.w + CFG::TW - 1) / CFG::TW;
        J.tiles_per_img = J.tiles_x * ((J.h + CFG::TH - 1) / CFG::TH);
        J.n_tiles_n = (a.cout + CFG::BN - 1) / CFG::BN;
        J.block_begin = blocks;
        blocks += J.tiles_per_img * J.n_tiles_n * a.B;
        S3D_CHECK((long long)J.h * J.w * a.cout < (1LL << 32), S3D_ERR_INVALID, "conv: a plane of one sample must stay below 2^32 elements");
    }
    if (!blocks) return 0;
    a.xcd_swizzle = 1;
    conv_note_kernel(CFG::KH == 3 ? "k_conv_mfma<3x3> direct MFMA convolution" : (CFG::KH == 1 ? (CFG::TR ? "k_conv_mfma<1x1, transposed accumulators> direct MFMA convolution" : "k_conv_mfma<1x1> direct MFMA convolution") : "k_conv_mfma<5x5> direct MFMA convolution"));
    if constexpr (CFG::KH == 1 && !CFG::TR) {
        if (rider && rider->n_blocks > 0) {
            conv_note_kernel(rider_name(rider->kind));
            hipLaunchKernelGGL((k_conv_mfma<CFG, true>), dim3(blocks + rider->n_blocks), dim3(256), 0, st, a, RiderArg<true>{*rider});
            S3D_HIP(hipGetLastError());
            return 0;
        }
    }
    hipLaunchKernelGGL(k_conv_mfma<CFG>, dim3(blocks), dim3(256), 0, st, a, RiderArg<false>());
    S3D_HIP(hipGetLastError());
    return 0;
}

template <int TH, int TW>
static long long count_tiles(const ConvArgs& a) {
    long long t = 0;
    for (int j = 0; j < a.njobs; ++j) t += (long long)((a.job[j].w + TW - 1) / TW) * ((a.job[j].h + TH - 1) / TH);
    return t * a.B;
}

bool conv_wino24_channels(int cin, int cout) { return conv_use_wino24() && cout % 4 == 0 && cin % 32 == 0; }
static bool takes_wino24(const ConvArgs& a) { return conv_wino24_channels(a.cin, a.cout) && a.job[0].wgt_wino24s; }
double conv_exec_fraction(ConvKind kind, const ConvArgs& a) {
    if (kind == CONV_3x3 && !conv_use_naive() && takes_wino24(a)) return 1.0 / 3.0;
    if (kind == CONV_3x3 && !conv_use_naive() && conv_use_wino() && a.job[0].wgt_wino && a.cout % 4 == 0) return wino_exec_fraction();
    return 1.0;
}

static bool conv1x1_transposed(int cout, long long blocks) {
    const int tr_mode = opt(OPT_CONV1X1_T);
    return tr_mode != 0 && cout % 4 == 0 && (tr_mode == 1 || blocks >= 4 * 768);
}
static long long conv1x1_blocks(const Geo& g, int B, int cout) {
    long long blocks = 0;
    for (int p = 0; p < 3; ++p) blocks += (long long)((g.w[p] + 7) / 8) * ((g.h[p] + 7) / 8) * ((cout + 63) / 64) * B;
    return blocks;
}
bool conv1x1_takes_rider(const Geo& g, int B, int cout) {
    return riders_enabled() && !conv_use_naive() && opt(OPT_CONV1X1_T) == kOptUnset && !conv1x1_transposed(cout, conv1x1_blocks(g, B, cout));
}

int launch_conv(ConvKind kind, ConvArgs& a, hipStream_t st, const ConvRider* rider) {
    S3D_CHECK(!rider || (kind == CONV_1x1 && !conv_use_naive() && opt(OPT_CONV1X1_T) == kOptUnset), S3D_ERR_INTERNAL, "conv: a rider on a launch that cannot carry one");
    S3D_CHECK(a.njobs >= 1 && a.njobs <= kMaxConvJobs, S3D_ERR_INVALID, "conv: %d jobs", a.njobs);
    S3D_CHECK(a.cin % KC == 0 && a.cin > 0, S3D_ERR_INVALID, "conv: cin=%d must be a positive multiple of %d", a.cin, KC);
    if (conv_use_naive()) return kind == CONV_1x3_ROLL ? launch_rank1(a, st, true) : launch_conv_naive(kind, a, st);
    switch (kind) {
        case CONV_3x3:
            if (takes_wino24(a)) {
                for (int j = 0; j < a.njobs; ++j) a.job[j].wgt = a.job[j].wgt_wino24s;
                return launch_conv_wino24s(a, st);
            }
            if (conv_use_wino() && a.job[0].wgt_wino && a.cout % 4 == 0) {
                for (int j = 0; j < a.njobs; ++j) a.job[j].wgt = a.job[j].wgt_wino;
                return launch_conv_wino(a, st);
            }
            return launch_cfg<ConvCfg<8, 8, 3, 3, 2, 2, 1, 1>>(a, st);
        case CONV_1x1:
            {
                bool plain = true;
                long long blocks = 0;
                for (int j = 0; j < a.njobs; ++j) {
                    plain = plain && !a.job[j].rrow && !a.job[j].rcol && !a.job[j].gn_part;
                    blocks += (long long)((a.job[j].w + 7) / 8) * ((a.job[j].h + 7) / 8) * ((a.cout + 63) / 64) * a.B;
                }
                if (plain && conv1x1_transposed(a.cout, blocks)) {
                    S3D_CHECK(!rider, S3D_ERR_INTERNAL, "conv: a rider on a launch of the transposed 1x1 form");
                    return launch_cfg<ConvCfg<8, 8, 1, 1, 2, 2, 1, 1, 1, 2, true>>(a, st);
                }
            }
            return launch_cfg<ConvCfg<8, 8, 1, 1, 2, 2, 1, 1, 1, 2>>(a, st, rider);
        case CONV_1x3_VEC:
            return launch_rank1(a, st, false);
        case CONV_1x3_ROLL:
            return launch_rank1(a, st, true);
        case CONV_5x5:
            return launch_cfg<ConvCfg<8, 8, 5, 5, 2, 2, 1, 1>>(a, st);
    }
    set_error("conv: unknown kind %d", int(kind));
    return S3D_ERR_INVALID;
}

}
```

sin3dm_amd/csrc/s3d_kernels.hip:

```cpp
#include "s3d_common.h"
#include "s3d_rank1.h"
#include "s3d_riders.h"
#include "s3d_sampler.h"

namespace s3d {

__device__ __forceinline__ float silu_f(float v) { return v * __builtin_amdgcn_rcpf(1.0f + __expf(-v)); }

static inline int cdiv(int a, int b) { return (a + b - 1) / b; }

__global__ void k_nchw_to_nhwc(const float* __restrict__ in, float* __restrict__ out, int B, int C, int hw) {
    size_t i = size_t(blockIdx.x) * blockDim.x + threadIdx.x;
    size_t n = size_t(B) * C * hw;
    if (i >= n) return;
    int c = int(i % C);
    size_t r = i / C;
    int pix = int(r % hw);
    int b = int(r / hw);
    out[i] = in[(size_t(b) * C + c) * hw + pix];
}
__global__ void k_nhwc_to_nchw(const float* __restrict__ in, float* __restrict__ out, int B, int C, int hw) {
    size_t i = size_t(blockIdx.x) * blockDim.x + threadIdx.x;
    size_t n = size_t(B) * C * hw;
    if (i >= n) return;
// ... 75 lines not shown
        acc.z = fmaf(v, wv.z, acc.z); acc.w = fmaf(v, wv.w, acc.w);
    }
    reinterpret_cast<float4*>(a.out[p] + ((size_t(b) * a.h[p] + y) * a.w[p] + xx) * a.Cout)[q] = acc;
}
template <int PX, int CQ>
__global__ __launch_bounds__(256) void k_in_conv_lds(InConvArgs a, int segs0, int segs1, int segs2, double* part, int maxparts) {
    constexpr int LANES = 256 / CQ, C = 4 * CQ;
    __shared__ __attribute__((aligned(16))) float sx[PX][16];
    __shared__ float sred[2][LANES][C];
    const int b = blockIdx.y;
    int blk = blockIdx.x, p = 0;
    if (blk >= segs0) { blk -= segs0; p = 1; if (blk >= segs1) { blk -= segs1; p = 2; } }
    const int h = a.h[p], w = a.w[p];
    const int len = p == 2 ? h : w, nseg = (len + PX - 1) / PX;
    const int line = blk / nseg, s0 = (blk % nseg) * PX;
    const int Hc = a.H + a.D, Wc = a.W + a.D;
    const float* xb = a.x + size_t(b) * a.Cin * Hc * Wc;
    const int sy = p == 2 ? a.H + line : line, sx0 = p == 1 ? a.W + s0 : s0;
    for (int it = threadIdx.x; it < 16 * PX; it += 256) {
        const int ci = it / PX, e = it - ci * PX;
        sx[e][ci] = ci < a.Cin && s0 + e < len ? xb[(size_t(ci) * Hc + sy) * Wc + sx0 + e] : 0.f;
    }
    const int q = threadIdx.x % CQ, lp = threadIdx.x / CQ;
    const float4* wq = reinterpret_cast<const float4*>(a.wT + size_t(p) * a.Cin * a.Cout) + q;
    float4 wv[16];
#pragma unroll
    for (int ci = 0; ci < 16; ++ci) wv[ci] = ci < a.Cin ? wq[size_t(ci) * CQ] : make_float4(0, 0, 0, 0);
    const float4 bias = reinterpret_cast<const float4*>(a.bias + size_t(p) * a.Cout)[q];
    __syncthreads();
    float gs[4] = {0.f, 0.f, 0.f, 0.f}, gss[4] = {0.f, 0.f, 0.f, 0.f};
#pragma unroll
    for (int k = 0; k < PX / LANES; ++k) {
        const int e = k * LANES + lp;
        if (s0 + e >= len) continue;
        float4 acc = bias;
#pragma unroll
        for (int c4 = 0; c4 < 4; ++c4) {
            const float4 v = *reinterpret_cast<const float4*>(&sx[e][c4 * 4]);
            const float vv[4] = {v.x, v.y, v.z, v.w};
#pragma unroll
            for (int j = 0; j < 4; ++j) {
                const float4 ww = wv[c4 * 4 + j];
                acc.x = fmaf(vv[j], ww.x, acc.x); acc.y = fmaf(vv[j], ww.y, acc.y);
                acc.z = fmaf(vv[j], ww.z, acc.z); acc.w = fmaf(vv[j], ww.w, acc.w);
            }
        }
        const int y = p == 2 ? s0 + e : line, xx = p == 2 ? line : s0 + e;
        reinterpret_cast<float4*>(a.out[p] + ((size_t(b) * h + y) * w + xx) * a.Cout)[q] = acc;
        gs[0] += acc.x; gs[1] += acc.y; gs[2] += acc.z; gs[3] += acc.w;
        gss[0] = fmaf(acc.x, acc.x, gss[0]); gss[1] = fmaf(acc.y, acc.y, gss[1]); gss[2] = fmaf(acc.z, acc.z, gss[2]); gss[3] = fmaf(acc.w, acc.w, gss[3]);
    }
    if (part) {
#pragma unroll
        for (int k = 0; k < 4; ++k) { sred[0][lp][4 * q + k] = gs[k]; sred[1][lp][4 * q + k] = gss[k]; }
        __syncthreads();
        if (threadIdx.x < 32) {
            constexpr int cg = C / 32;
            const int g = threadIdx.x;
            double S = 0, SS = 0;
            for (int l = 0; l < LANES; ++l)
#pragma unroll
                for (int k = 0; k < cg; ++k) { S += sred[0][l][cg * g + k]; SS += sred[1][l][cg * g + k]; }
            double* o = part + (((size_t(b) * 3 + p) * 32 + g) * maxparts + blk) * 2;
            o[0] = S; o[1] = SS;
        }
    }
}
constexpr int kInConvPx = 32;
bool in_conv_gn_parts(const Geo& g, int Cin, int Cout, int nparts[3]) {
    if (!((Cout == 64 || Cout == 128 || Cout == 256) && Cin <= 16)) return false;
    for (int p = 0; p < 3; ++p) { const int len = p == 2 ? g.h[p] : g.w[p], lines = p == 2 ? g.w[p] : g.h[p]; nparts[p] = lines * ((len + kInConvPx - 1) / kInConvPx); }
    return true;
}
int launch_in_conv(const float* x, int B, int Cin, int H, int W, int D, const float* wT, const float* bias,
                   int Cout, Tri& out, hipStream_t st, const GnPartials* part) {
    InConvArgs a;
    a.x = x; a.wT = wT; a.bias = bias; a.B = B; a.Cin = Cin; a.Cout = Cout; a.H = H; a.W = W; a.D = D;
    a.pix_begin[0] = 0;
    for (int p = 0; p < 3; ++p) {
        a.out[p] = out.p[p]; a.h[p] = out.g.h[p]; a.w[p] = out.g.w[p];
        a.pix_begin[p + 1] = a.pix_begin[p] + (long long)a.h[p] * a.w[p];
    }
    long long n = a.pix_begin[3] * (Cout / 4) * B;
    if (!n) return 0;
    int segs[3];
    if (in_conv_gn_parts(out.g, Cin, Cout, segs)) {
        S3D_CHECK(!part || (part->nsub == 32 && part->nparts[0] == segs[0] && part->nparts[1] == segs[1] && part->nparts[2] == segs[2]), S3D_ERR_INVALID, "in_conv: GroupNorm partial layout");
        const dim3 grid(segs[0] + segs[1] + segs[2], B);
        double* pp = part ? part->p : nullptr;
        const int mp = part ? part->maxparts : 0;
        if (Cout == 64) hipLaunchKernelGGL((k_in_conv_lds<kInConvPx, 16>), grid, dim3(256), 0, st, a, segs[0], segs[1], segs[2], pp, mp);
        else if (Cout == 128) hipLaunchKernelGGL((k_in_conv_lds<kInConvPx, 32>), grid, dim3(256), 0, st, a, segs[0], segs[1], segs[2], pp, mp);
        else hipLaunchKernelGGL((k_in_conv_lds<kInConvPx, 64>), grid, dim3(256), 0, st, a, segs[0], segs[1], segs[2], pp, mp);
        S3D_HIP(hipGetLastError());
        return 0;
    }
    S3D_CHECK(!part, S3D_ERR_INVALID, "in_conv: this shape does not emit GroupNorm partials");
    hipLaunchKernelGGL(k_in_conv, dim3((unsigned)((n + 255) / 256)), dim3(256), 0, st, a);
    S3D_HIP(hipGetLastError());
    return 0;
}

struct GnPartArgs {
    const float* x[3];
    int h[3], w[3];
    int C, cq, pl;
    double* part;
};
__global__ void k_gn_partials(GnPartArgs a) {
    extern __shared__ __attribute__((aligned(16))) char smem_raw[];
    double* sm = reinterpret_cast<double*>(smem_raw);
    const int chunk = blockIdx.x, p = blockIdx.y, b = blockIdx.z;
    const int npix = a.h[p] * a.w[p];
    const int per = (npix + kGnChunks - 1) / kGnChunks;
    const int p0 = chunk * per, p1 = min(npix, p0 + per);
    const int q = threadIdx.x % a.cq, l = threadIdx.x / a.cq;
    double s[4] = {0, 0, 0, 0}, ss[4] = {0, 0, 0, 0};
    const float4* src = reinterpret_cast<const float4*>(a.x[p] + size_t(b) * npix * a.C) + q;
#pragma unroll 8
    for (int pix = p0 + l; pix < p1; pix += a.pl) {
        const float4 v = src[size_t(pix) * a.cq];
        s[0] += v.x; ss[0] += double(v.x) * v.x;
        s[1] += v.y; ss[1] += double(v.y) * v.y;
        s[2] += v.z; ss[2] += double(v.z) * v.z;
        s[3] += v.w; ss[3] += double(v.w) * v.w;
    }
    gn_chunk_reduce(sm, s, ss, q, l, a.C, a.pl, a.part + ((size_t(b) * 3 + p) * 32 * kGnChunks + chunk) * 2, kGnChunks);
}
int launch_gn_partials(const Tri& x, int B, GnPartials out, hipStream_t st) {
    GnPartArgs a;
    for (int p = 0; p < 3; ++p) { a.x[p] = x.p[p]; a.h[p] = x.g.h[p]; a.w[p] = x.g.w[p]; }
    a.C = x.C; thread_shape(x.C, a.cq, a.pl); a.part = out.p;
    S3D_CHECK(x.C % 32 == 0 && a.cq <= 1024, S3D_ERR_INVALID, "GroupNorm(32, C): C=%d must be a multiple of 32 and <= 4096", x.C);
    size_t shm = size_t(a.pl) * a.C * 2 * sizeof(double);
    hipLaunchKernelGGL(k_gn_partials, dim3(kGnChunks, 3, B), dim3(a.cq * a.pl), shm, st, a);
    S3D_HIP(hipGetLastError());
    return 0;
}

__global__ __launch_bounds__(256) void k_gn_finalize(GnFinArgs a) {
    __shared__ double sm4[4];
    gn_finalize_block(a, blockIdx.x, blockIdx.y, blockIdx.z, sm4);
}
static bool gn_finalize_args(const GnPartials& part, const Geo& g, int C, GnStats out, GnFinArgs& a) {
    a.part = part.p; a.mr = out.mr; a.maxparts = part.maxparts; a.nsub = part.nsub;
    if (part.nsub % 32 != 0) return false;
    a.subs_per_group = part.nsub / 32;
    for (int p = 0; p < 3; ++p) { a.nparts[p] = part.nparts[p]; a.count[p] = double(C / 32) * g.h[p] * g.w[p]; }
    return true;
}
bool gn_finalize_rider(const GnPartials& part, const Geo& g, int C, int B, GnStats out, ConvRider& r) {
    memset(&r, 0, sizeof r);
    if (!B || !gn_finalize_args(part, g, C, out, r.fin)) return false;
    r.kind = RIDER_GN_FINALIZE; r.gx = 32; r.n_blocks = 32 * 3 * B;
    return true;
}
int launch_gn_finalize(const GnPartials& part, const Geo& g, int C, int B, GnStats out, hipStream_t st) {
    GnFinArgs a;
    S3D_CHECK(gn_finalize_args(part, g, C, out, a), S3D_ERR_INVALID, "gn_finalize: nsub=%d", part.nsub);
    if (!B) return 0;
    hipLaunchKernelGGL(k_gn_finalize, dim3(32, 3, B), dim3(256), 0, st, a);
    S3D_HIP(hipGetLastError());
    return 0;
}

__device__ __forceinline__ float4 up2x_sample(const float4* __restrict__ src, int hi, int wi, int cuq, int yo, int xo) {
    float fy = 0.5f * (float(yo) + 0.5f) - 0.5f; fy = fy < 0.f ? 0.f : fy;
    float fx = 0.5f * (float(xo) + 0.5f) - 0.5f; fx = fx < 0.f ? 0.f : fx;
    int y0 = int(fy); y0 = y0 > hi - 1 ? hi - 1 : y0;
    int x0 = int(fx); x0 = x0 > wi - 1 ? wi - 1 : x0;
    const int y1 = y0 + (y0 < hi - 1 ? 1 : 0), x1 = x0 + (x0 < wi - 1 ? 1 : 0);
    const float ly1 = fy - float(y0), ly0 = 1.f - ly1, lx1 = fx - float(x0), lx0 = 1.f - lx1;
    const float4 v00 = src[(size_t(y0) * wi + x0) * cuq], v01 = src[(size_t(y0) * wi + x1) * cuq];
    const float4 v10 = src[(size_t(y1) * wi + x0) * cuq], v11 = src[(size_t(y1) * wi + x1) * cuq];
    float4 o;
    o.x = ly0 * (lx0 * v00.x + lx1 * v01.x) + ly1 * (lx0 * v10.x + lx1 * v11.x);
    o.y = ly0 * (lx0 * v00.y + lx1 * v01.y) + ly1 * (lx0 * v10.y + lx1 * v11.y);
    o.z = ly0 * (lx0 * v00.z + lx1 * v01.z) + ly1 * (lx0 * v10.z + lx1 * v11.z);
    o.w = ly0 * (lx0 * v00.w + lx1 * v01.w) + ly1 * (lx0 * v10.w + lx1 * v11.w);
    return o;
}


__global__ void k_gn_partials_up(GnPartUpArgs a) {
    extern __shared__ __attribute__((aligned(16))) char smem_raw[];
    gn_partials_up_block(a, blockIdx.x, blockIdx.y, blockIdx.z, reinterpret_cast<double*>(smem_raw));
}
void gn_up_parts(const Geo& out_g, int nparts[3]) {
    for (int p = 0; p < 3; ++p) nparts[p] = cdiv(out_g.h[p], kActRows) * cdiv(out_g.w[p], kActCols);
}
static bool gn_partials_up_args(const Tri& u, int sg, GnPartials out, GnPartUpArgs& a, int& maxtiles) {
    maxtiles = 0;
    for (int p = 0; p < 3; ++p) {
        a.u[p] = u.p[p]; a.hi[p] = u.g.h[p]; a.wi[p] = u.g.w[p];
        maxtiles = std::max(maxtiles, cdiv(2 * u.g.h[p], kActRows) * cdiv(2 * u.g.w[p], kActCols));
    }
    a.C = u.C; thread_shape(u.C, a.cq, a.pl); a.sg = sg; a.nsub = u.C / sg; a.part = out.p; a.maxparts = out.maxparts;
    return u.C % sg == 0 && a.cq <= 1024 && out.nsub == a.nsub && out.maxparts >= maxtiles;
}
int launch_gn_partials_up(const Tri& u, int B, int sg, GnPartials out, hipStream_t st) {
    GnPartUpArgs a;
    int maxtiles = 0;
    S3D_CHECK(gn_partials_up_args(u, sg, out, a, maxtiles), S3D_ERR_INVALID, "gn_partials_up: layout");
    if (!maxtiles || !B) return 0;
    hipLaunchKernelGGL(k_gn_partials_up, dim3(maxtiles, 3, B), dim3(a.cq * a.pl), size_t(a.pl) * a.C * 2 * sizeof(double), st, a);
    S3D_HIP(hipGetLastError());
    return 0;
}
bool gn_partials_up_rider(const Tri& u, int B, int sg, GnPartials out, ConvRider& r) {
    memset(&r, 0, sizeof r);
    int maxtiles = 0;
    if (!gn_partials_up_args(u, sg, out, r.up, maxtiles) || !maxtiles || !B) return false;
    if (r.up.cq * r.up.pl != 256 || size_t(r.up.pl) * r.up.C * 2 * sizeof(double) > size_t(kRiderLdsBytes)) return false;
    r.kind = RIDER_GN_PARTIALS_UP; r.gx = maxtiles; r.n_blocks = maxtiles * 3 * B;
    return true;
}
__global__ __launch_bounds__(256) void k_gn_finalize_cat(GnFinCatArgs a) {
    __shared__ double sm4[4];
    gn_finalize_cat_block(a, blockIdx.x, blockIdx.y, blockIdx.z, sm4);
}
static bool gn_finalize_cat_args(const GnPartials& pu, const GnPartials& ps, const Geo& g, int C, GnStats out, GnFinCatArgs& a) {
    a.pu = pu.p; a.ps = ps.p; a.mr = out.mr; a.maxparts_u = pu.maxparts; a.maxparts_s = ps.maxparts; a.nsub_u = pu.nsub; a.nsub_s = ps.nsub;
    if ((pu.nsub + ps.nsub) % 32 != 0) return false;
    a.subs_per_group = (pu.nsub + ps.nsub) / 32;
    for (int p = 0; p < 3; ++p) { a.nparts_u[p] = pu.nparts[p]; a.nparts_s[p] = ps.nparts[p]; a.count[p] = double(C / 32) * g.h[p] * g.w[p]; }
    return true;
}
bool gn_finalize_cat_rider(const GnPartials& pu, const GnPartials& ps, const Geo& g, int C, int B, GnStats out, ConvRider& r) {
    memset(&r, 0, sizeof r);
    if (!B || !gn_finalize_cat_args(pu, ps, g, C, out, r.cat)) return false;
    r.kind = RIDER_GN_FINALIZE_CAT; r.gx = 32; r.n_blocks = 32 * 3 * B;
    return true;
}
int launch_gn_finalize_cat(const GnPartials& pu, const GnPartials& ps, const Geo& g, int C, int B, GnStats out, hipStream_t st) {
    GnFinCatArgs a;
    S3D_CHECK(gn_finalize_cat_args(pu, ps, g, C, out, a), S3D_ERR_INVALID, "gn_finalize_cat: nsub=%d+%d", pu.nsub, ps.nsub);
    if (!B) return 0;
    hipLaunchKernelGGL(k_gn_finalize_cat, dim3(32, 3, B), dim3(256), 0, st, a);
    S3D_HIP(hipGetLastError());
    return 0;
}

struct GnPartSrc { const double* part; int nparts[3], maxparts, nsub, spg; double count[3]; };
__device__ __forceinline__ float* gn_stats_from_parts(const GnPartSrc& a, int b, int p, double* sd, float* mr_out) {
    const int L = int(blockDim.x) >> 5, tid = threadIdx.x;
    if (tid < 32 * L) {
        const int g = tid / L, j = tid - g * L;
        const int n = a.nparts[p], tot = a.spg * n;
        const double2* base = reinterpret_cast<const double2*>(a.part) + ((size_t(b) * 3 + p) * a.nsub + size_t(g) * a.spg) * a.maxparts;
        double S = 0, SS = 0;
        constexpr int NB = 16;
        for (int k0 = j; k0 < tot; k0 += NB * L) {
            double2 v[NB];
#pragma unroll
            for (int u = 0; u < NB; ++u) {
                const int k = k0 + u * L, kc = k < tot ? k : j;
                const int sub = kc / n, part = kc - sub * n;
                v[u] = base[size_t(sub) * a.maxparts + part];
                if (k >= tot) v[u] = make_double2(0.0, 0.0);
            }
#pragma unroll
            for (int u = 0; u < NB; ++u) { S += v[u].x; SS += v[u].y; }
        }
        sd[tid * 2] = S; sd[tid * 2 + 1] = SS;
    }
    __syncthreads();
    float* stf = reinterpret_cast<float*>(sd + 2 * blockDim.x);
    if (tid < 32) {
        double S = 0, SS = 0;
        for (int j = 0; j < L; ++j) { S += sd[(tid * L + j) * 2]; SS += sd[(tid * L + j) * 2 + 1]; }
        const double m = S / a.count[p];
        double var = SS / a.count[p] - m * m;
        if (var < 0) var = 0;
        stf[tid] = float(m); stf[32 + tid] = float(1.0 / sqrt(var + 1e-5));
        if (mr_out) {
            float* o = mr_out + ((size_t(b) * 3 + p) * 32 + tid) * 2;
            o[0] = stf[tid]; o[1] = stf[32 + tid];
        }
    }
    return stf;
}

static GnPartSrc gn_part_src(const GnPartials& part, const Geo& g, int C) {
    GnPartSrc s;
    s.part = part.p; s.maxparts = part.maxparts; s.nsub = part.nsub; s.spg = part.nsub / 32;
    for (int p = 0; p < 3; ++p) { s.nparts[p] = part.nparts[p]; s.count[p] = double(C / 32) * g.h[p] * g.w[p]; }
    return s;
}

__global__ void k_gn_finalize_as(GnPartSrc ps, float* mr) {
    extern __shared__ __attribute__((aligned(16))) char smem_raw[];
    gn_stats_from_parts(ps, blockIdx.y, blockIdx.x, reinterpret_cast<double*>(smem_raw), mr);
}
int launch_gn_finalize_as(const GnPartials& part, const Geo& g, int C, int B, int threads, GnStats out, hipStream_t st) {
    S3D_CHECK(gn_act_can_add_parts(part, C) && threads >= 32 && threads % 32 == 0 && out.mr, S3D_ERR_INVALID, "gn_finalize_as: layout");
    if (!B) return 0;
    const GnPartSrc ps = gn_part_src(part, g, C);
    hipLaunchKernelGGL(k_gn_finalize_as, dim3(3, B), dim3(threads), size_t(threads) * 2 * sizeof(double) + 64 * sizeof(float), st, ps, out.mr);
    S3D_HIP(hipGetLastError());
    return 0;
}

struct GnActArgs {
    const float* x[3]; float* y[3];
    const float* gamma[3]; const float* beta[3];
    float* rowpart[3]; float* colpart[3];
    const float* mr;
    const float* film; int film_stride;
    int h[3], w[3];
    int C, cq, pl, with_means;
    GnPartSrc ps;
    float* mr_out;
};
__global__ __launch_bounds__(256) void k_gn_act(GnActArgs a) {
    extern __shared__ __attribute__((aligned(16))) char smem_raw[];
    float* sm = reinterpret_cast<float*>(smem_raw);
    const int p = blockIdx.y, b = blockIdx.z;
    const int h = a.h[p], w = a.w[p];
    const int ntc = (w + kActCols - 1) / kActCols, ntr = (h + kActRows - 1) / kActRows;
    if (int(blockIdx.x) >= ntc * ntr) return;
    const int tr = blockIdx.x / ntc, tc = blockIdx.x % ntc;
    const bool ident = a.mr == nullptr && a.ps.part == nullptr;
    const int q = threadIdx.x % a.cq, l = threadIdx.x / a.cq;
    const int i0 = tr * kActRows, j0 = tc * kActCols;
    const int i1 = min(h, i0 + kActRows), j1 = min(w, j0 + kActCols);
    const float4* xs = reinterpret_cast<const float4*>(a.x[p] + size_t(b) * h * w * a.C) + q;
    float4* ys = reinterpret_cast<float4*>(a.y[p] + size_t(b) * h * w * a.C) + q;
    float4 xfirst[kActRows];
    {
        const int j = min(j0 + l, j1 - 1);
#pragma unroll
        for (int r = 0; r < kActRows; ++r) xfirst[r] = xs[(size_t(min(i0 + r, i1 - 1)) * w + j) * a.cq];
    }
    const bool film = a.film != nullptr;
    float4 gam4 = make_float4(1, 1, 1, 1), bet4 = make_float4(0, 0, 0, 0), fsc4 = make_float4(0, 0, 0, 0), fsh4 = make_float4(0, 0, 0, 0);
    if (!ident) { gam4 = reinterpret_cast<const float4*>(a.gamma[p])[q]; bet4 = reinterpret_cast<const float4*>(a.beta[p])[q]; }
    if (film) {
        fsc4 = reinterpret_cast<const float4*>(a.film + size_t(b) * a.film_stride)[q];
        fsh4 = reinterpret_cast<const float4*>(a.film + size_t(b) * a.film_stride + a.C)[q];
    }
    if (a.mr) {
        if (threadIdx.x < 32) {
            const float* mr = a.mr + ((size_t(b) * 3 + p) * 32 + threadIdx.x) * 2;
            sm[threadIdx.x] = mr[0]; sm[32 + threadIdx.x] = mr[1];
        }
    } else if (a.ps.part) {
        sm = gn_stats_from_parts(a.ps, b, p, reinterpret_cast<double*>(smem_raw), a.mr_out && blockIdx.x == 0 ? a.mr_out : nullptr);
    }
    __syncthreads();
    const int cg = a.C / 32;
    float A[4], Bc[4], sc[4], sh[4];
    {
        const float gv[4] = {gam4.x, gam4.y, gam4.z, gam4.w}, bv[4] = {bet4.x, bet4.y, bet4.z, bet4.w};
        const float s1[4] = {fsc4.x, fsc4.y, fsc4.z, fsc4.w}, s2[4] = {fsh4.x, fsh4.y, fsh4.z, fsh4.w};
#pragma unroll
        for (int k = 0; k < 4; ++k) {
            const int c = 4 * q + k, g = c / cg;
            const float scale = ident ? 1.0f : sm[32 + g] * gv[k];
            A[k] = scale;
            Bc[k] = ident ? 0.0f : bv[k] - scale * sm[g];
            sc[k] = film ? 1.0f + s1[k] : 1.0f;
            sh[k] = film ? s2[k] : 0.0f;
        }
    }
    __syncthreads();
    float4 rowacc[kActRows];
#pragma unroll
    for (int r = 0; r < kActRows; ++r) rowacc[r] = make_float4(0, 0, 0, 0);
    for (int j = j0 + l; j < j1; j += a.pl) {
        float4 colacc = make_float4(0, 0, 0, 0);
        float4 xin[kActRows];
        if (j == j0 + l) {
#pragma unroll
            for (int r = 0; r < kActRows; ++r) xin[r] = xfirst[r];
        } else {
#pragma unroll
            for (int r = 0; r < kActRows; ++r) xin[r] = xs[(size_t(min(i0 + r, i1 - 1)) * w + j) * a.cq];
        }
#pragma unroll
        for (int r = 0; r < kActRows; ++r) {
            const int i = i0 + r;
            if (i < i1) {
                const size_t off = (size_t(i) * w + j) * a.cq;
                const float4 v = xin[r];
// ... 963 lines not shown
```

sin3dm_amd/csrc/s3d_model.h:

```cpp
#pragma once
#include <algorithm>
#include <cmath>
#include <memory>

#include "s3d_common.h"

namespace s3d {

static const char* kPlane[3] = {"xy", "xz", "yz"};

struct ParamSpec {
    std::string name;
    std::vector<int64_t> shape;
    size_t numel() const { size_t n = 1; for (auto d : shape) n *= size_t(d); return n; }
};

struct NormW { size_t gamma[3], beta[3]; };
struct ResBlockW {
    std::string prefix;
    int C, Cout;
    NormW n1, n2;
    ConvW c1, c2, skip;
    ConvW skip_a, skip_b;
    int c_up = 0;
// ... 85 lines not shown
    float* flat = nullptr;
    int64_t flat_numel = 0;
    std::vector<size_t> flat_off;
    std::map<std::string, size_t> flat_index;
    long long train_key[5] = {-1, -1, -1, -1, -1};
    size_t train_high = 0;
    DevBuf tbuf, descs_dev;
    std::vector<PackDesc> descs;
    int pack_blocks = 0;
    std::vector<ResBlockWT> in_blocks_t, out_blocks_t;
    Tape tape;
    const float* tdev(size_t off) const { return static_cast<const float*>(tbuf.p) + off; }
    hipStream_t bwd_side = nullptr;
    std::vector<hipEvent_t> bwd_events;

    struct ProfRec { int cls; hipEvent_t e0, e1; double flops, mfma_flops; };
    int prof_every = 0;
    long fwd_count = 0;
    bool prof_now = false;
    int prof_mask = 15;
    bool prof_train = false;
    std::vector<ProfRec> prof_recs;
    std::vector<hipEvent_t> prof_pool;
    int64_t prof_forwards = 0;
    std::string prof_kernel[S3D_PROF_CLASSES];
    void note_prof_kernel(int cls) {
        if (cls < 0 || cls >= S3D_PROF_CLASSES) return;
        const std::string n = conv_last_kernel();
        if (n.empty() || prof_kernel[cls].find(n) != std::string::npos) return;
        prof_kernel[cls] += (prof_kernel[cls].empty() ? "" : " + ") + n;
    }
    hipEvent_t prof_event() {
        hipEvent_t e = nullptr;
        if (!prof_pool.empty()) { e = prof_pool.back(); prof_pool.pop_back(); }
        else if (hipEventCreate(&e) != hipSuccess) e = nullptr;
        return e;
    }
    int timed_conv(int cls, ConvKind kind, ConvArgs& ca, hipStream_t st, const ConvRider* rider = nullptr) {
        if (!prof_now || !((prof_mask >> cls) & 1)) return launch_conv(kind, ca, st, rider);
        int taps = kind == CONV_3x3 ? 9 : (kind == CONV_1x1 ? 1 : (kind == CONV_1x3_VEC ? 3 : (kind == CONV_1x3_ROLL ? 9 : 25)));
        double pix = 0;
        for (int j = 0; j < ca.njobs; ++j) pix += double(ca.job[j].h) * ca.job[j].w;
        ProfRec r{cls, prof_event(), prof_event(), 2.0 * taps * ca.cin * ca.cout * pix * ca.B, 0.0};
        r.mfma_flops = r.flops * conv_exec_fraction(kind, ca);
        if (r.e0) (void)hipEventRecord(r.e0, st);
        int rc = launch_conv(kind, ca, st, rider);
        note_prof_kernel(cls);
        if (r.e1) (void)hipEventRecord(r.e1, st);
        prof_recs.push_back(r);
        return rc;
    }
    template <class F>
    int timed_launch(int cls, double flops, double mfma_flops, hipStream_t st, F fn) {
        if (!prof_now || !((prof_mask >> cls) & 1)) return fn();
        ProfRec r{cls, prof_event(), prof_event(), flops, mfma_flops};
        if (r.e0) (void)hipEventRecord(r.e0, st);
        int rc = fn();
        note_prof_kernel(cls);
        if (r.e1) (void)hipEventRecord(r.e1, st);
        prof_recs.push_back(r);
        return rc;
    }
    ~s3d_unet() {
        for (auto e : bwd_events) (void)hipEventDestroy(e);
        if (bwd_side) (void)hipStreamDestroy(bwd_side);
        for (auto& r : prof_recs) { if (r.e0) (void)hipEventDestroy(r.e0); if (r.e1) (void)hipEventDestroy(r.e1); }
        for (auto e : prof_pool) (void)hipEventDestroy(e);
    }

    const float* dev(size_t off) const { return static_cast<const float*>(wbuf.p) + off; }
};

namespace s3d {

int pack_all(s3d_unet* m);
int finalize_pack_plan(std::vector<PackDesc>& descs, DevBuf& dev, int& blocks_out);
int launch_repack_generic(const PackDesc* descs_dev, int ndesc, int blocks, const float* flat, float* wbuf, float* tbuf, hipStream_t st);
int run_forward(s3d_unet* m, const float* x, const float* t, int B, int H, int W, int D, float* out, hipStream_t st,
                Tape* tape, const float* ext_film = nullptr, int ext_film_stride = 0, const s3d_sampler_args* fuse = nullptr,
                int carry_flags = 0, const s3d_known_region* known = nullptr);

struct Fwd {
    s3d_unet* m;
    int B;
    hipStream_t st;
    const float* film;
    int film_stride = -1;
    int fstride() const { return film_stride >= 0 ? film_stride : m->film_total; }
    Tape* tape = nullptr;
    RBTape last_rb;
    Arena& ar() { return m->arena; }

    Tri alloc_tri(int C, const Geo& g) {
        Tri t; t.C = C; t.g = g;
        for (int p = 0; p < 3; ++p) t.p[p] = ar().alloc<float>(size_t(B) * g.h[p] * g.w[p] * C);
        return t;
    }
    struct ChunkStats { GnPartials part; GnStats gs; };
    ChunkStats chunk_stats(const int* nparts = nullptr) {
        ChunkStats c;
        int mx = 0;
        for (int p = 0; p < 3; ++p) { c.part.nparts[p] = nparts ? nparts[p] : kGnChunks; mx = std::max(mx, c.part.nparts[p]); }
        c.part.maxparts = mx; c.part.nsub = 32;
        c.part.p = ar().alloc<double>(size_t(B) * 3 * mx * 64);
        c.gs.mr = ar().alloc<float>(size_t(B) * 3 * 64);
        return c;
    }
    int finish(const ChunkStats& c, Tri& t) {
        t.gn = c.gs.mr;
        if (ar().measuring) return 0;
        return launch_gn_finalize(c.part, t.g, t.C, B, c.gs, st);
    }
    int stats_of(const Tri& x, GnStats& out) {
        if (x.gn) { out.mr = x.gn; return 0; }
        if (x.part.p) {
            out.mr = ar().alloc<float>(size_t(B) * 3 * 64);
            if (ar().measuring) return 0;
            return launch_gn_finalize(x.part, x.g, x.C, B, out, st);
        }
        GnPartials part;
        part.p = ar().alloc<double>(size_t(B) * 3 * kGnChunks * 64);
        part.maxparts = kGnChunks; part.nsub = 32;
        for (int p = 0; p < 3; ++p) part.nparts[p] = kGnChunks;
        out.mr = ar().alloc<float>(size_t(B) * 3 * 64);
        if (ar().measuring) return 0;
        S3D_TRY(launch_gn_partials(x, B, part, st));
        return launch_gn_finalize(part, x.g, x.C, B, out, st);
    }

    int r1_slices_for(const Tri& y, const ConvW& cw) const {
        if (cw.k != 3 || !cw.rollout || conv_use_naive()) return 1;
        if (cw.wino24s[0] == 0 || !conv_wino24_channels(cw.cin, cw.cout)) return 1;
        return conv_rank1_slices(y.C);
    }
    int roll_buffers(const Tri& y, const ConvW& cw, bool roll, MeanPartials& mp, MeanVecs& mv, const float* rrow[3], const float* rcol[3]) {
        for (int p = 0; p < 3; ++p) { rrow[p] = rcol[p] = nullptr; }
        if (!roll) return 0;
        size_t mtot = 0;
        for (int p = 0; p < 3; ++p) mtot += size_t(B) * (y.g.h[p] + y.g.w[p]) * y.C;
        float* means = ar().alloc<float>(mtot);
        for (int p = 0; p < 3; ++p) {
            const int h = y.g.h[p], w = y.g.w[p];
            const int ntc = (w + kActCols - 1) / kActCols, ntr = (h + kActRows - 1) / kActRows;
            mp.rowpart[p] = ar().alloc<float>(size_t(B) * ntc * h * y.C);
            mp.colpart[p] = ar().alloc<float>(size_t(B) * ntr * w * y.C);
            mv.rowmean[p] = means; means += size_t(B) * h * y.C;
            mv.colmean[p] = means; means += size_t(B) * w * y.C;
            const int nsl = r1_slices_for(y, cw);
            rrow[p] = ar().alloc<float>(size_t(nsl) * B * h * 4 * cw.cout);
            rcol[p] = ar().alloc<float>(size_t(nsl) * B * w * 4 * cw.cout);
        }
        return 0;
    }
    int rank1_tables(const Tri& y, const ConvW& cw, const MeanPartials& mp, const MeanVecs& mv, const float* const rrow[3], const float* const rcol[3]) {
        S3D_TRY(launch_means_finalize(y.g, y.C, B, mp, mv, st));
        ConvArgs ca; memset(&ca, 0, sizeof ca);
        ca.B = B; ca.cin = y.C; ca.cout = cw.cout; ca.njobs = 6;
        ca.r1_slices = r1_slices_for(y, cw);
        const float* rowvec[3] = {mv.rowmean[1], mv.rowmean[0], mv.colmean[0]};
        const float* colvec[3] = {mv.rowmean[2], mv.colmean[2], mv.colmean[1]};
        for (int p = 0; p < 3; ++p) {
            ConvJob& jr = ca.job[2 * p];
            jr.in = rowvec[p]; jr.wgt = m->dev(cw.rrow[p]); jr.out = const_cast<float*>(rrow[p]); jr.h = 1; jr.w = y.g.h[p];
            jr.wgt_r1f = cw.rrow_f[p] ? m->dev(cw.rrow_f[p]) : nullptr;
            ConvJob& jc = ca.job[2 * p + 1];
            jc.in = colvec[p]; jc.wgt = m->dev(cw.rcol[p]); jc.out = const_cast<float*>(rcol[p]); jc.h = 1; jc.w = y.g.w[p];
            jc.wgt_r1f = cw.rcol_f[p] ? m->dev(cw.rcol_f[p]) : nullptr;
        }
        return m->timed_conv(2, CONV_1x3_ROLL, ca, st);
    }
    int norm_act(const Tri& x, const NormW& nw, const float* film_ptr, const ConvW* cw, Tri& y, const float* rrow[3],
                 const float* rcol[3], NormTape* nt = nullptr) {
        const bool measuring = ar().measuring;
        GnStats stats{nullptr};
        const bool few_parts = !x.gn && gn_act_can_add_parts(x.part, x.C);
        const bool add_parts = few_parts && gn_parts_in_consumer(gn_act_blocks(x.g, B));
        if (few_parts && !add_parts) {
            stats.mr = ar().alloc<float>(size_t(B) * 3 * 64);
            if (!measuring) S3D_TRY(launch_gn_finalize_as(x.part, x.g, x.C, B, gn_act_threads(x.C), stats, st));
        } else if (!add_parts) S3D_TRY(stats_of(x, stats));
        else if (nt) stats.mr = ar().alloc<float>(size_t(B) * 3 * 64);
        if (nt) { nt->stats = stats; nt->roll = cw && cw->rollout; }
        y = alloc_tri(x.C, x.g);
        ActArgs aa;
        for (int p = 0; p < 3; ++p) { aa.gamma[p] = m->dev(nw.gamma[p]); aa.beta[p] = m->dev(nw.beta[p]); }
        aa.film = film_ptr; aa.film_stride = fstride();
        const bool roll = cw && cw->rollout;
        MeanPartials mp; MeanVecs mv;
        if (roll) S3D_TRY(roll_buffers(y, *cw, true, mp, mv, rrow, rcol));
        else for (int p = 0; p < 3; ++p) { rrow[p] = rcol[p] = nullptr; }
        if (nt && roll) nt->mv = mv;
        if (measuring) return 0;
        S3D_TRY(launch_gn_act(x, B, stats, aa, y, roll ? &mp : nullptr, st, add_parts ? &x.part : nullptr));
        if (!roll) return 0;
        return rank1_tables(y, *cw, mp, mv, rrow, rcol);
    }

    bool riders_on() const { return !tape && riders_enabled() && opt_on(OPT_VCAT); }
    bool rides(const ConvW& cw, const Geo& g) const { return riders_on() && cw.k == 1 && conv1x1_takes_rider(g, B, cw.cout); }

    int conv(const Tri& y, const ConvW& cw, const float* bbias, const float* const rrow[3], const float* const rcol[3],
             const Tri* res, Tri& out, int want_stats = 0, hipStream_t on = nullptr, bool no_bias = false, bool res_up = false,
             const ConvRider* rider = nullptr) {
        hipStream_t st = on ? on : this->st;
        out = alloc_tri(cw.cout, y.g);
        if (!(cw.k == 3 && !conv_use_naive())) want_stats = 0;
        const bool w24 = cw.k == 3 && cw.wino24s[0] != 0 && conv_wino24_channels(cw.cin, cw.cout);
        S3D_CHECK(!(cw.only24_current && (!w24 || conv_use_naive())), S3D_ERR_INVALID,
                  "conv %dx%d %d->%d: the kernel form selected now reads a weight image the training handle's repack plan does not keep "
                  "current (options changed after s3d_unet_train_attach): attach again", cw.k, cw.k, cw.cin, cw.cout);
        GnPartials part; GnStats gs{nullptr};
        if (want_stats) {
            conv_gn_parts(CONV_3x3, y.g, part.nparts, w24);
            part.maxparts = std::max(part.nparts[0], std::max(part.nparts[1], part.nparts[2]));
            part.nsub = cw.cout / gn_subgroup(cw.cout);
            part.p = ar().alloc<double>(size_t(B) * 3 * part.maxparts * part.nsub * 2);
            if (want_stats == 1) { gs.mr = ar().alloc<float>(size_t(B) * 3 * 64); out.gn = gs.mr; }
            else out.part = part;
        }
        if (ar().measuring) return 0;
        ConvArgs ca; memset(&ca, 0, sizeof ca);
        ca.B = B; ca.cin = cw.cin; ca.cout = cw.cout; ca.njobs = 3;
        if (want_stats) { ca.gn_sg = gn_subgroup(cw.cout); ca.gn_nsub = part.nsub; ca.gn_maxparts = part.maxparts; }
        ca.r1_slices = rrow && rcol && rrow[0] ? r1_slices_for(y, cw) : 1;
        for (int p = 0; p < 3; ++p) {
            ConvJob& J = ca.job[p];
            J.in = y.p[p]; J.wgt = m->dev(cw.dense[p]); J.bias = no_bias ? nullptr : m->dev(cw.bias[p]);
            J.wgt_wino = cw.k == 3 && !w24 ? m->dev(cw.wino[p]) : nullptr;
            J.wgt_wino24s = w24 ? m->dev(cw.wino24s[p]) : nullptr;
            J.bbias = bbias; J.bbias_stride = fstride();
            J.rrow = rrow ? rrow[p] : nullptr; J.rcol = rcol ? rcol[p] : nullptr;
            J.res = res ? res->p[p] : nullptr; J.res_up = res && res_up ? 1 : 0; J.out = out.p[p]; J.h = y.g.h[p]; J.w = y.g.w[p];
            J.gn_part = want_stats ? part.p + size_t(p) * part.maxparts * part.nsub * 2 : nullptr;
        }
        S3D_TRY(m->timed_conv(cw.k == 3 ? 0 : 1, cw.k == 3 ? CONV_3x3 : CONV_1x1, ca, st, rider));
        if (want_stats == 1) S3D_TRY(launch_gn_finalize(part, y.g, cw.cout, B, gs, st));
        return 0;
    }

    int resblock_cat(const ResBlockW& rb, const Tri& u, const Tri& sk, Tri& out, int out_stats) {
        const bool ssn = m->cfg.use_scale_shift_norm != 0;
        const float* film_ptr = film ? film + rb.film_off : nullptr;
        const bool measuring = ar().measuring;
        const int C = u.C + sk.C, sg = gn_subgroup(C);
        GnPartials pu; GnStats stats;
        pu.nsub = u.C / sg;
        gn_up_parts(sk.g, pu.nparts);
        pu.maxparts = std::max(pu.nparts[0], std::max(pu.nparts[1], pu.nparts[2]));
        pu.p = ar().alloc<double>(size_t(B) * 3 * pu.nsub * pu.maxparts * 2);
        stats.mr = ar().alloc<float>(size_t(B) * 3 * 64);
        Tri z, skip;
        ConvRider r_up, r_fin;
        const bool up_rides = !measuring && rides(rb.skip_a, u.g) && gn_partials_up_rider(u, B, sg, pu, r_up);
        const bool fin_rides = up_rides && rides(rb.skip_b, sk.g) && gn_finalize_cat_rider(pu, sk.part, sk.g, C, B, stats, r_fin);
        S3D_TRY(conv(u, rb.skip_a, nullptr, nullptr, nullptr, nullptr, z, 0, nullptr, true, false, up_rides ? &r_up : nullptr));
        S3D_TRY(conv(sk, rb.skip_b, nullptr, nullptr, nullptr, &z, skip, 0, nullptr, false, true, fin_rides ? &r_fin : nullptr));
        if (!measuring) {
            if (!up_rides) S3D_TRY(launch_gn_partials_up(u, B, sg, pu, st));
            if (!fin_rides) S3D_TRY(launch_gn_finalize_cat(pu, sk.part, sk.g, C, B, stats, st));
        }
        Tri y1, h1, y2;
        y1 = alloc_tri(C, sk.g);
        const float *rr[3], *rc[3];
        {
            ActArgs aa;
            for (int p = 0; p < 3; ++p) { aa.gamma[p] = m->dev(rb.n1.gamma[p]); aa.beta[p] = m->dev(rb.n1.beta[p]); }
            aa.film = nullptr; aa.film_stride = fstride();
            const bool roll = rb.c1.rollout;
            MeanPartials mp; MeanVecs mv;
            S3D_TRY(roll_buffers(y1, rb.c1, roll, mp, mv, rr, rc));
            if (!measuring) {
                S3D_TRY(launch_gn_act_cat(u, sk, B, stats, aa, y1, roll ? &mp : nullptr, st));
                if (roll) S3D_TRY(rank1_tables(y1, rb.c1, mp, mv, rr, rc));
            }
        }
        S3D_TRY(conv(y1, rb.c1, ssn ? nullptr : film_ptr, rr, rc, nullptr, h1, 2));
        S3D_TRY(norm_act(h1, rb.n2, ssn ? film_ptr : nullptr, &rb.c2, y2, rr, rc, nullptr));
        S3D_TRY(conv(y2, rb.c2, nullptr, rr, rc, &skip, out, out_stats));
        return 0;
    }

    int resblock(const ResBlockW& rb, const Tri& x, Tri& out, bool out_feeds_norm, int out_stats_override = -1, const ChunkStats* fin = nullptr) {
        const bool ssn = m->cfg.use_scale_shift_norm != 0;
        const float* film_ptr = film ? film + rb.film_off : nullptr;
        Tri y1, h1, y2;
        const float *rr[3], *rc[3];
        Tri skip;
        const Tri* res = &x;
        ConvRider r_fin;
        const bool fin_rides = fin && !ar().measuring && rb.has_skip && rides(rb.skip, x.g) && gn_finalize_rider(fin->part, x.g, x.C, B, fin->gs, r_fin);
        if (fin && !fin_rides && !ar().measuring) S3D_TRY(launch_gn_finalize(fin->part, x.g, x.C, B, fin->gs, st));
        if (rb.has_skip) {
            S3D_TRY(conv(x, rb.skip, nullptr, nullptr, nullptr, nullptr, skip, false, nullptr, false, false, fin_rides ? &r_fin : nullptr));
            res = &skip;
        }
        RBTape rt;
        RBTape* T = tape ? &rt : nullptr;
        S3D_TRY(norm_act(x, rb.n1, nullptr, &rb.c1, y1, rr, rc, T ? &T->n1 : nullptr));
        S3D_TRY(conv(y1, rb.c1, ssn ? nullptr : film_ptr, rr, rc, nullptr, h1, 2));
        S3D_TRY(norm_act(h1, rb.n2, ssn ? film_ptr : nullptr, &rb.c2, y2, rr, rc, T ? &T->n2 : nullptr));
        S3D_TRY(conv(y2, rb.c2, nullptr, rr, rc, res, out, out_stats_override >= 0 ? out_stats_override : (out_feeds_norm ? 1 : 0)));
        if (T) {
            rt.rb = &rb; rt.x = x; rt.y1 = y1; rt.h1 = h1; rt.y2 = y2;
            last_rb = rt;
        }
        return 0;
    }
};

}
```

sin3dm_amd/csrc/s3d_riders.h:

```cpp
#pragma once
#include "s3d_common.h"

namespace s3d {

__device__ __forceinline__ void gn_acc(double s[4], double ss[4], const float4& v) {
    s[0] += v.x; ss[0] += double(v.x) * v.x;
    s[1] += v.y; ss[1] += double(v.y) * v.y;
    s[2] += v.z; ss[2] += double(v.z) * v.z;
    s[3] += v.w; ss[3] += double(v.w) * v.w;
}

__device__ __forceinline__ double block_sum256(double v, double* sm4) {
#pragma unroll
    for (int off = 32; off >= 1; off >>= 1) v += __shfl_xor(v, off, 64);
    if ((threadIdx.x & 63) == 0) sm4[threadIdx.x >> 6] = v;
    __syncthreads();
    const double r = (sm4[0] + sm4[1]) + (sm4[2] + sm4[3]);
    __syncthreads();
    return r;
}

struct Up8Rows { int rk[6]; float ly0[8], ly1[8]; };
__device__ __forceinline__ Up8Rows up8_rows(int i0, int hi) {
    Up8Rows R;
    const int base = (i0 >> 1) - 1;
#pragma unroll
    for (int k = 0; k < 6; ++k) { const int r = base + k; R.rk[k] = r < 0 ? 0 : (r > hi - 1 ? hi - 1 : r); }
#pragma unroll
    for (int r = 0; r < 8; ++r) {
        float fy = 0.5f * (float(i0 + r) + 0.5f) - 0.5f; fy = fy < 0.f ? 0.f : fy;
        int y0 = int(fy); y0 = y0 > hi - 1 ? hi - 1 : y0;
        R.ly1[r] = fy - float(y0); R.ly0[r] = 1.f - R.ly1[r];
    }
    return R;
}
__device__ __forceinline__ void up8_column(const float4* __restrict__ src, int wi, int cuq, const Up8Rows& R, int j, float4 out[8]) {
    float fx = 0.5f * (float(j) + 0.5f) - 0.5f; fx = fx < 0.f ? 0.f : fx;
    int x0 = int(fx); x0 = x0 > wi - 1 ? wi - 1 : x0;
    const int x1 = x0 + (x0 < wi - 1 ? 1 : 0);
    const float lx1 = fx - float(x0), lx0 = 1.f - lx1;
    float4 hl[6];
#pragma unroll
    for (int k = 0; k < 6; ++k) {
        const float4 a = src[(size_t(R.rk[k]) * wi + x0) * cuq], b = src[(size_t(R.rk[k]) * wi + x1) * cuq];
        hl[k].x = lx0 * a.x + lx1 * b.x; hl[k].y = lx0 * a.y + lx1 * b.y; hl[k].z = lx0 * a.z + lx1 * b.z; hl[k].w = lx0 * a.w + lx1 * b.w;
    }
#pragma unroll
    for (int r = 0; r < 8; ++r) {
        const float4 p = hl[(r + 1) >> 1], q = hl[((r + 1) >> 1) + 1];
        out[r].x = R.ly0[r] * p.x + R.ly1[r] * q.x; out[r].y = R.ly0[r] * p.y + R.ly1[r] * q.y;
        out[r].z = R.ly0[r] * p.z + R.ly1[r] * q.z; out[r].w = R.ly0[r] * p.w + R.ly1[r] * q.w;
    }
}

__device__ __forceinline__ void gn_finalize_block(const GnFinArgs& a, int g, int p, int b, double* sm4) {
    const int tid = threadIdx.x;
    const double* base = a.part + (size_t(b) * 3 + p) * a.maxparts * a.nsub * 2;
    double S = 0, SS = 0;
    for (int k = 0; k < a.subs_per_group; ++k) {
        const double2* row = reinterpret_cast<const double2*>(base + (size_t(g) * a.subs_per_group + k) * a.maxparts * 2);
        for (int part = tid; part < a.nparts[p]; part += 256) { const double2 v = row[part]; S += v.x; SS += v.y; }
    }
    S = block_sum256(S, sm4);
    SS = block_sum256(SS, sm4);
    if (tid == 0) {
        const double m = S / a.count[p];
        double var = SS / a.count[p] - m * m;
        if (var < 0) var = 0;
        float* o = a.mr + ((size_t(b) * 3 + p) * 32 + g) * 2;
        o[0] = float(m);
        o[1] = float(1.0 / sqrt(var + 1e-5));
    }
}

__device__ __forceinline__ void gn_partials_up_block(const GnPartUpArgs& a, int tile, int p, int b, double* sm) {
    const int hi = a.hi[p], wi = a.wi[p], h = 2 * hi, w = 2 * wi;
    const int ntc = (w + kActCols - 1) / kActCols, ntr = (h + kActRows - 1) / kActRows;
    if (tile >= ntc * ntr) return;
    const int tr = tile / ntc, tc = tile % ntc;
    const int i0 = tr * kActRows, j0 = tc * kActCols, i1 = min(h, i0 + kActRows), j1 = min(w, j0 + kActCols);
    const int q = threadIdx.x % a.cq, l = threadIdx.x / a.cq;
    double s[4] = {0, 0, 0, 0}, ss[4] = {0, 0, 0, 0};
    const float4* src = reinterpret_cast<const float4*>(a.u[p] + size_t(b) * hi * wi * a.C) + q;
    const Up8Rows R = up8_rows(i0, hi);
    for (int j = j0 + l; j < j1; j += a.pl) {
        float4 v[8];
        up8_column(src, wi, a.cq, R, j, v);
#pragma unroll
        for (int r = 0; r < 8; ++r) if (i0 + r < i1) gn_acc(s, ss, v[r]);
    }
    for (int k = 0; k < 4; ++k) {
        sm[(size_t(l) * a.C + 4 * q + k) * 2 + 0] = s[k];
        sm[(size_t(l) * a.C + 4 * q + k) * 2 + 1] = ss[k];
    }
    __syncthreads();
    for (int sub = threadIdx.x; sub < a.nsub; sub += blockDim.x) {
        double S = 0, SS = 0;
        for (int ll = 0; ll < a.pl; ++ll)
            for (int c = sub * a.sg; c < (sub + 1) * a.sg; ++c) { S += sm[(size_t(ll) * a.C + c) * 2]; SS += sm[(size_t(ll) * a.C + c) * 2 + 1]; }
        double* o = a.part + (((size_t(b) * 3 + p) * a.nsub + sub) * a.maxparts + tile) * 2;
        o[0] = S; o[1] = SS;
    }
}

__device__ __forceinline__ void gn_finalize_cat_block(const GnFinCatArgs& a, int g, int p, int b, double* sm4) {
    const int tid = threadIdx.x;
    double S = 0, SS = 0;
    for (int k = 0; k < a.subs_per_group; ++k) {
        const int sub = g * a.subs_per_group + k;
        const bool up = sub < a.nsub_u;
        const double2* row = reinterpret_cast<const double2*>(
            up ? a.pu + (((size_t(b) * 3 + p) * a.nsub_u + sub) * a.maxparts_u) * 2
               : a.ps + (((size_t(b) * 3 + p) * a.nsub_s + (sub - a.nsub_u)) * a.maxparts_s) * 2);
        const int n = up ? a.nparts_u[p] : a.nparts_s[p];
        for (int part = tid; part < n; part += 256) { const double2 v = row[part]; S += v.x; SS += v.y; }
    }
    S = block_sum256(S, sm4);
    SS = block_sum256(SS, sm4);
    if (tid == 0) {
        const double m = S / a.count[p];
        double var = SS / a.count[p] - m * m;
        if (var < 0) var = 0;
        float* o = a.mr + ((size_t(b) * 3 + p) * 32 + g) * 2;
        o[0] = float(m);
        o[1] = float(1.0 / sqrt(var + 1e-5));
    }
}

__device__ __forceinline__ void run_rider(const ConvRider& r, int idx, void* lds) {
    const int x = idx % r.gx, p = (idx / r.gx) % 3, b = idx / (3 * r.gx);
    double* sm = static_cast<double*>(lds);
    if (r.kind == RIDER_GN_PARTIALS_UP) gn_partials_up_block(r.up, x, p, b, sm);
    else if (r.kind == RIDER_GN_FINALIZE) gn_finalize_block(r.fin, x, p, b, sm);
    else if (r.kind == RIDER_GN_FINALIZE_CAT) gn_finalize_cat_block(r.cat, x, p, b, sm);
}

}
```

sin3dm_amd/csrc/s3d_runtime.hip:

```cpp
#include "s3d_common.h"
#include <atomic>

namespace s3d {

static thread_local char g_err[1024] = "";

void set_error(const char* fmt, ...) {
    va_list ap;
    va_start(ap, fmt);
    vsnprintf(g_err, sizeof g_err, fmt, ap);
    va_end(ap);
}
const char* get_error() { return g_err; }

int DevBuf::reserve(size_t bytes) {
    if (bytes <= cap) return 0;
    release();
    S3D_HIP(hipMalloc(&p, bytes));
    cap = bytes;
    return 0;
}
void DevBuf::release() {
    if (p) (void)hipFree(p);
    p = nullptr;
    cap = 0;
}
int workspace_overrun(const char* what, size_t run_peak, size_t measured) {
    if (run_peak <= measured) return 0;
    set_error("%s: the run pass took %zu bytes of workspace, the measuring pass found %zu (internal error: the workspace key "
              "misses something the allocations depend on)", what, run_peak, measured);
    return S3D_ERR_INTERNAL;
}
int upload(DevBuf& dst, const void* host, size_t bytes) {
    S3D_TRY(dst.reserve(bytes));
    S3D_HIP(hipMemcpy(dst.p, host, bytes, hipMemcpyHostToDevice));
    return 0;
}

static std::atomic<int> g_opt[OPT_COUNT];
static std::atomic<int> g_opt_state[OPT_COUNT];
static std::atomic<long long> g_opt_gen{0};
long long opt_generation() { return g_opt_gen.load(std::memory_order_acquire); }
static int parse_opt(int o, const char* v) {
    if (o == OPT_CONV_IMPL) return strcmp(v, "naive") == 0 ? 1 : 0;
    char* end = nullptr;
    const long n = strtol(v, &end, 10);
    if (end == v || *end) return kOptUnset;
    return (o == OPT_WINO ? n == 0 || n == 4 || n == 24 : n == 0 || n == 1) ? int(n) : kOptUnset;
}
static const char* opt_values(int o) { return o == OPT_WINO ? "0, 4 or 24" : "0 or 1"; }
int opt(Opt o) {
    if (g_opt_state[o].load(std::memory_order_acquire) == 0) {
        const std::string env = std::string("S3D_") + kOptNames[o];
        const char* e = getenv(env.c_str());
        int expect = 0;
        const int v = e ? parse_opt(o, e) : kOptUnset;
        if (g_opt_state[o].compare_exchange_strong(expect, -1, std::memory_order_acq_rel)) {
            g_opt[o].store(v, std::memory_order_relaxed);
            g_opt_state[o].store(1, std::memory_order_release);
        } else while (g_opt_state[o].load(std::memory_order_acquire) < 0) {}
    }
    return g_opt[o].load(std::memory_order_relaxed);
}
static int find_opt(const char* name) {
    if (!name) return -1;
    if (strncmp(name, "S3D_", 4) == 0) name += 4;
    for (int o = 0; o < OPT_COUNT; ++o) if (strcmp(name, kOptNames[o]) == 0) return o;
    return -1;
}
static std::atomic<int> g_riders{-1};
bool riders_enabled() {
    int v = g_riders.load(std::memory_order_acquire);
    if (v < 0) {
        const char* e = getenv("S3D_RIDERS");
        int expect = -1;
        g_riders.compare_exchange_strong(expect, e && strcmp(e, "0") == 0 ? 0 : 1, std::memory_order_acq_rel);
        v = g_riders.load(std::memory_order_acquire);
    }
    return v != 0;
}
int device_cus() {
    static std::atomic<int> cache[64];
    int dev = 0;
    if (hipGetDevice(&dev) != hipSuccess || dev < 0 || dev >= 64) dev = 0;
    int n = cache[dev].load(std::memory_order_relaxed);
    if (n > 0) return n;
    n = 256;
    if (hipDeviceGetAttribute(&n, hipDeviceAttributeMultiprocessorCount, dev) != hipSuccess || n <= 0) n = 256;
    cache[dev].store(n, std::memory_order_relaxed);
    return n;
}

}

extern "C" {

int s3d_set_option(const char* name, const char* value) {
    using namespace s3d;
    const int o = find_opt(name);
    S3D_CHECK(o >= 0, S3D_ERR_INVALID, "set_option: unknown option '%s'", name ? name : "(null)");
    const bool given = value && *value;
    const int v = given ? parse_opt(o, value) : kOptUnset;
    S3D_CHECK(!given || v != kOptUnset, S3D_ERR_INVALID, "set_option: %s takes %s, not '%s'", kOptNames[o], opt_values(o), value);
    g_opt[o].store(v, std::memory_order_relaxed);
    g_opt_state[o].store(2, std::memory_order_release);
    g_opt_gen.fetch_add(1, std::memory_order_acq_rel);
    return 0;
}

int s3d_get_option(const char* name, int* value) {
    using namespace s3d;
    const int o = find_opt(name);
    S3D_CHECK(o >= 0 && value, S3D_ERR_INVALID, "get_option: unknown option '%s'", name ? name : "(null)");
    *value = opt(Opt(o));
    return 0;
}

int s3d_set_riders(int on) {
    s3d::g_riders.store(on ? 1 : 0, std::memory_order_release);
    return 0;
}

int s3d_abi_version(void) { return S3D_ABI_VERSION; }
const char* s3d_last_error(void) { return s3d::get_error(); }

int s3d_device_count(void) {
    int n = 0;
    hipError_t e = hipGetDeviceCount(&n);
    if (e != hipSuccess) {
        s3d::set_error("hipGetDeviceCount failed: %s", hipGetErrorString(e));
        return S3D_ERR_HIP;
    }
    return n;
}

int s3d_sampler_step(const s3d_sampler_args* a, void* stream) {
    using namespace s3d;
    S3D_CHECK(a != nullptr, S3D_ERR_INVALID, "sampler_step: null args");
    S3D_CHECK(a->model_out && a->x && a->t && a->tables && a->pred_xstart, S3D_ERR_INVALID,
              "sampler_step: model_out, x, t, tables and pred_xstart are required");
    S3D_CHECK(a->mode == S3D_STEP_DDPM || a->mode == S3D_STEP_DDIM || a->mode == S3D_STEP_MEAN_ONLY, S3D_ERR_INVALID,
              "sampler_step: bad mode %d", a->mode);
    S3D_CHECK(a->mode == S3D_STEP_MEAN_ONLY || a->sample, S3D_ERR_INVALID, "sampler_step: sample output required");
    S3D_CHECK(a->mode != S3D_STEP_DDPM || a->noise, S3D_ERR_INVALID, "sampler_step: DDPM step needs noise");
    S3D_CHECK(a->mode != S3D_STEP_DDIM || a->eta == 0.f || a->noise, S3D_ERR_INVALID, "sampler_step: eta>0 needs noise");
    S3D_CHECK((a->y0 == nullptr) == (a->mask == nullptr), S3D_ERR_INVALID, "sampler_step: y0 and mask go together");
    S3D_CHECK(a->T > 0 && a->batch >= 0 && a->per_sample >= 0, S3D_ERR_INVALID, "sampler_step: bad sizes");
    return launch_sampler(*a, static_cast<hipStream_t>(stream));
}

int s3d_sampler_step_known(const s3d_sampler_args* a, const s3d_known_region* known, void* stream) {
    using namespace s3d;
    S3D_CHECK(a != nullptr && known != nullptr, S3D_ERR_INVALID, "sampler_step_known: null args");
    S3D_CHECK(a->model_out && a->x && a->t && a->tables && a->pred_xstart && a->sample, S3D_ERR_INVALID,
              "sampler_step_known: model_out, x, t, tables, sample and pred_xstart are required");
    S3D_CHECK(a->mode == S3D_STEP_DDPM || a->mode == S3D_STEP_DDIM, S3D_ERR_INVALID, "sampler_step_known: a DDPM or DDIM step, not mode %d", a->mode);
    S3D_CHECK(a->mode != S3D_STEP_DDPM || a->noise, S3D_ERR_INVALID, "sampler_step_known: DDPM step needs noise");
    S3D_CHECK(a->mode != S3D_STEP_DDIM || a->eta == 0.f || a->noise, S3D_ERR_INVALID, "sampler_step_known: eta>0 needs noise");
    S3D_CHECK(!a->y0 && !a->mask, S3D_ERR_INVALID, "sampler_step_known: the step's own y0 / mask (x0 replacement) cannot be combined with a known region");
    S3D_CHECK(known->y0 && known->mask && known->noise && known->tables, S3D_ERR_INVALID, "sampler_step_known: y0, mask, noise and tables are required");
    S3D_CHECK(a->T > 0 && a->batch >= 0 && a->per_sample >= 0, S3D_ERR_INVALID, "sampler_step_known: bad sizes");
    return launch_sampler_known(*a, *known, static_cast<hipStream_t>(stream));
}

int s3d_sampler_renoise(const float* x_prev, const float* noise, const float* known_tables, const int64_t* t, int32_t T, int64_t batch,
                        int64_t per_sample, float* x_t, void* stream) {
    using namespace s3d;
    S3D_CHECK(x_prev && noise && known_tables && t && x_t, S3D_ERR_INVALID, "sampler_renoise: null argument");
    S3D_CHECK(T > 0 && batch >= 0 && per_sample >= 0, S3D_ERR_INVALID, "sampler_renoise: bad sizes");
    return launch_renoise(x_prev, noise, known_tables, t, T, batch, per_sample, x_t, static_cast<hipStream_t>(stream));
}

}
```

Baseline: 1.194 samples/s.

## Split skip 1x1 conv into tile ranges that carry rank-1 rollout blocks as riders

```diff
diff --git a/include/sin3dm_hip.h b/include/sin3dm_hip.h
--- a/include/sin3dm_hip.h
+++ b/include/sin3dm_hip.h
@@ -25,6 +25,7 @@
 S3D_API int s3d_set_option(const char* name, const char* value);
 S3D_API int s3d_get_option(const char* name, int* value);
 S3D_API int s3d_set_riders(int on);
+S3D_API int s3d_set_skip_split(int mode);
 S3D_API const char* s3d_last_error(void);
 S3D_API int s3d_device_count(void);
 
diff --git a/sin3dm_amd/_lib.py b/sin3dm_amd/_lib.py
--- a/sin3dm_amd/_lib.py
+++ b/sin3dm_amd/_lib.py
@@ -70,6 +70,7 @@
     "s3d_set_option": (C.c_int, [C.c_char_p, C.c_char_p]),
     "s3d_get_option": (C.c_int, [C.c_char_p, C.POINTER(C.c_int)]),
     "s3d_set_riders": (C.c_int, [C.c_int]),
+    "s3d_set_skip_split": (C.c_int, [C.c_int]),
     "s3d_unet_create": (C.c_int, [C.POINTER(UNetCfg), C.POINTER(C.c_void_p)]),
     "s3d_unet_destroy": (None, [C.c_void_p]),
     "s3d_unet_num_params": (C.c_int, [C.c_void_p]),
@@ -314,6 +315,10 @@
     check(load().s3d_set_riders(1 if on else 0))
 
 
+def set_skip_split(mode):
+    check(load().s3d_set_skip_split(-1 if mode is None else int(mode)))
+
+
 def stream_ptr():
     import torch
     return C.c_void_p(torch.cuda.current_stream().cuda_stream)
diff --git a/sin3dm_amd/csrc/s3d_common.h b/sin3dm_amd/csrc/s3d_common.h
--- a/sin3dm_amd/csrc/s3d_common.h
+++ b/sin3dm_amd/csrc/s3d_common.h
@@ -92,6 +92,7 @@
 long long opt_generation();
 inline bool opt_on(Opt o) { return opt(o) != 0; }
 bool riders_enabled();
+int skip_split_mode();
 int device_cus();
 
 struct Geo {
@@ -171,16 +172,24 @@
     int maxparts_u, maxparts_s, nparts_u[3], nparts_s[3], nsub_u, nsub_s, subs_per_group;
     double count[3];
 };
-enum RiderKind { RIDER_NONE = 0, RIDER_GN_PARTIALS_UP, RIDER_GN_FINALIZE, RIDER_GN_FINALIZE_CAT };
+struct Rank1bJob { const float* in; const float* wgt_r1f; float* out; int w, tiles_per_img, n_tiles_n, block_begin; };
+struct Rank1bArgs { Rank1bJob job[kMaxConvJobs]; int njobs, B, cin, cout, r1_slices; };
+struct Rank1bBlock { const float* in; const float* wgt_r1f; float* out; int L, tiles_per_img, n_tiles_n, local, B, cin, cout, r1_slices; };
+enum RiderKind { RIDER_NONE = 0, RIDER_GN_PARTIALS_UP, RIDER_GN_FINALIZE, RIDER_GN_FINALIZE_CAT, RIDER_RANK1B };
 struct ConvRider {
     int kind;
     int n_blocks;
     int gx;
-    union { GnPartUpArgs up; GnFinArgs fin; GnFinCatArgs cat; };
+    int tile_ranged;
+    int tile_begin[kMaxConvJobs], tile_count[kMaxConvJobs];
+    union { GnPartUpArgs up; GnFinArgs fin; GnFinCatArgs cat; Rank1bArgs r1b; };
 };
 constexpr int kRiderLdsBytes = 16384;
+constexpr int kR1bLdsFloats = 4 * 48 * 64;
 int launch_conv(ConvKind kind, ConvArgs& a, hipStream_t st, const ConvRider* rider = nullptr);
 bool conv1x1_takes_rider(const Geo& g, int B, int cout);
+void conv1x1_tiles(const Geo& g, int tiles[3]);
+bool rank1b_rider(ConvArgs& a, ConvRider& r);
 int launch_conv_naive(ConvKind kind, ConvArgs& a, hipStream_t st);
 bool conv_use_naive();
 void conv_note_kernel(const char* name);
diff --git a/sin3dm_amd/csrc/s3d_conv.hip b/sin3dm_amd/csrc/s3d_conv.hip
--- a/sin3dm_amd/csrc/s3d_conv.hip
+++ b/sin3dm_amd/csrc/s3d_conv.hip
@@ -42,21 +42,26 @@
     return n == 1 ? 3 : (idx == 0 ? 1 : (idx == n - 1 ? 2 : 0));
 }
 
-template <bool RIDER> struct RiderArg {};
-template <> struct RiderArg<true> { ConvRider r; };
-template <class CFG, bool RIDER = false>
-__global__ __launch_bounds__(256) void k_conv_mfma(ConvArgs args, RiderArg<RIDER> rider) {
+template <int RIDER> struct RiderArg { ConvRider r; };
+template <> struct RiderArg<0> {};
+template <class CFG, int RIDER = 0>
+__global__ __launch_bounds__(256, RIDER == 2 ? 3 : 1) void k_conv_mfma(ConvArgs args, RiderArg<RIDER> rider) {
     constexpr int TW = CFG::TW, KH = CFG::KH, KW = CFG::KW, MTW = CFG::MTW, NTW = CFG::NTW;
     constexpr int HW = CFG::HW, TAPS = KH * KW;
-    __shared__ __attribute__((aligned(16))) float smem[2 * (CFG::A_ELEMS + CFG::B_ELEMS)];
+    constexpr int kConvLds = 2 * (CFG::A_ELEMS + CFG::B_ELEMS);
+    __shared__ __attribute__((aligned(16))) float smem[RIDER == 2 && kR1bLdsFloats > kConvLds ? kR1bLdsFloats : kConvLds];
     float* const Abase = smem;
     float* const Bbase = smem + 2 * CFG::A_ELEMS;
 
     int bid = blockIdx.x;
     int nblocks = gridDim.x;
-    if constexpr (RIDER) {
+    if constexpr (RIDER != 0) {
         static_assert(sizeof smem >= size_t(kRiderLdsBytes) && KH == 1 && !CFG::TR, "the rider bodies work in the 1x1 convolution's LDS");
-        if (bid < rider.r.n_blocks) { run_rider(rider.r, bid, smem); return; }
+        if (bid < rider.r.n_blocks) {
+            if constexpr (RIDER == 2) run_rank1b_rider(rider.r, bid, smem);
+            else run_rider(rider.r, bid, smem);
+            return;
+        }
         bid -= rider.r.n_blocks; nblocks -= rider.r.n_blocks;
     }
     if (args.xcd_swizzle) {
@@ -69,7 +74,9 @@
     const ConvJob& J = args.job[j];
     int local = bid - J.block_begin;
     const int ntile = local % J.n_tiles_n; local /= J.n_tiles_n;
-    const int b = local / J.tiles_per_img; local %= J.tiles_per_img;
+    int tbegin = 0, tcount = J.tiles_per_img;
+    if constexpr (RIDER != 0) { tbegin = rider.r.tile_begin[j]; tcount = rider.r.tile_count[j]; }
+    const int b = local / tcount; local = tbegin + local % tcount;
     const int ty0 = (local / J.tiles_x) * CFG::TH, tx0 = (local % J.tiles_x) * TW;
     const int n0 = ntile * CFG::BN;
     const int h = J.h, w = J.w, cin = args.cin, cout = args.cout;
@@ -471,7 +478,6 @@
     rank1_block<ROLL3, NS>(blk, lds);
 }
 
-constexpr int kR1bLdsFloats = 4 * 48 * 64;
 __global__ __launch_bounds__(256) void k_rank1b(ConvArgs args) {
     extern __shared__ __attribute__((aligned(16))) float lds_dyn[];
     int bid = blockIdx.x;
@@ -480,99 +486,7 @@
 #pragma unroll
     for (int k = 1; k < kMaxConvJobs; ++k) j += (k < args.njobs && bid >= args.job[k].block_begin) ? 1 : 0;
     const ConvJob& J = args.job[j];
-    int local = bid - J.block_begin;
-    const int L = J.w, cin = args.cin, cout = args.cout, B = args.B;
-    const int mtile = local % J.tiles_per_img; local /= J.tiles_per_img;
-    const int b = local % B; local /= B;
-    const int g = local % J.n_tiles_n, sl = local / J.n_tiles_n;
-    const int nchunks = cin / kR1Chunk;
-    int chunk0 = 0, nch = nchunks;
-    if (args.r1_slices > 1) { const int first = (nchunks + 1) / 2; chunk0 = sl ? first : 0; nch = sl ? nchunks - first : first; }
-    const int csl = nch * kR1Chunk, ld = csl + 4;
-    const int tid = threadIdx.x, lane = tid & 63, wid = __builtin_amdgcn_readfirstlane(tid >> 6), i = lane & 31, half = lane >> 5;
-    const int nsteps = nch * 12;
-    const r1_f32x4* pf = reinterpret_cast<const r1_f32x4*>(J.wgt_r1f) + (size_t(g * 4 + wid) * (nchunks * 12) + chunk0 * 12) * 192 + lane;
-    constexpr int D = 3;
-    r1_f32x4 ring[D][3];
-    int pf_s = 0;
-    auto prefetch = [&](int slot) {
-        ring[slot][0] = ((r1_gf4ptr)(uintptr_t)pf)[0];
-        ring[slot][1] = ((r1_gf4ptr)(uintptr_t)(pf + 64))[0];
-        ring[slot][2] = ((r1_gf4ptr)(uintptr_t)(pf + 128))[0];
-        ++pf_s;
-        pf += pf_s < nsteps ? 192 : 0;
-    };
-#pragma unroll
-    for (int d = 0; d < D; ++d) prefetch(d);
-    {
-        const int q4 = csl / 4, items = 34 * q4;
-        const float* vb = J.in + (size_t(b) * L) * cin + chunk0 * kR1Chunk;
-        const r1_f32x4 zero4 = {0.f, 0.f, 0.f, 0.f};
-        for (int it0 = tid; it0 < items; it0 += 256 * 5) {
-            r1_f32x4 v[5];
-#pragma unroll
-            for (int u = 0; u < 5; ++u) {
-                const int it = it0 + 256 * u, row = it / q4, q = it - row * q4, pos = mtile * 32 - 1 + row;
-                const bool ok = it < items && pos >= 0 && pos < L;
-                v[u] = ((r1_gf4ptr)(uintptr_t)(vb + size_t(ok ? pos : 0) * cin + (ok ? q : 0) * 4))[0];
-                if (!ok) v[u] = zero4;
-            }
-#pragma unroll
-            for (int u = 0; u < 5; ++u) {
-                const int it = it0 + 256 * u, row = it / q4, q = it - row * q4;
-                if (it < items) *reinterpret_cast<r1_f32x4*>(lds_dyn + row * ld + q * 4) = v[u];
-            }
-        }
-    }
-    __syncthreads();
-    r1_f32x16 q[3];
-#pragma unroll
-    for (int o = 0; o < 3; ++o)
-#pragma unroll
-        for (int r = 0; r < 16; ++r) q[o][r] = 0.f;
-    const float* Ab = lds_dyn + i * ld + half * 4 + wid * 32;
-    for (int ch = 0; ch < nch; ++ch) {
-        const float* Ac = Ab + ch * kR1Chunk;
-#pragma unroll
-        for (int st = 0; st < 12; ++st) {
-            const int tap = st >> 2, k8 = st & 3;
-            const r1_f32x4 a4 = *reinterpret_cast<const r1_f32x4*>(Ac + tap * ld + k8 * 8);
-            r1_f32x4 b4[3];
-#pragma unroll
-            for (int o = 0; o < 3; ++o) b4[o] = ring[st % D][o];
-            __builtin_amdgcn_sched_barrier(0);
-#pragma unroll
-            for (int e = 0; e < 4; ++e)
-#pragma unroll
-                for (int o = 0; o < 3; ++o) q[o] = __builtin_amdgcn_mfma_f32_32x32x2f32(a4[e], b4[o][e], q[o], 0, 0, 0);
-            __builtin_amdgcn_sched_barrier(0);
-            prefetch(st % D);
-            __builtin_amdgcn_sched_barrier(0);
-        }
-    }
-    __syncthreads();
-    float* red = lds_dyn;
-#pragma unroll
-    for (int o = 0; o < 3; ++o)
-#pragma unroll
-        for (int r = 0; r < 16; ++r) red[((wid * 3 + o) * 16 + r) * 64 + lane] = q[o][r];
-    __syncthreads();
-    float* out = J.out + size_t(sl) * B * L * 4 * cout;
-#pragma unroll
-    for (int k = 0; k < 4; ++k) {
-        const int it = tid + 256 * k, r = it >> 6, l = it & 63;
-        float u[3];
-#pragma unroll
-        for (int o = 0; o < 3; ++o) {
-            const float* p = red + (o * 16 + r) * 64 + l;
-            u[o] = ((p[0] + p[3 * 1024]) + p[2 * 3 * 1024]) + p[3 * 3 * 1024];
-        }
-        const int row = mtile * 32 + (r & 3) + 8 * (r >> 2) + 4 * (l >> 5), co = g * 32 + (l & 31);
-        if (row < L && co < cout) {
-            float* o4 = out + (size_t(b) * L + row) * 4 * cout + co;
-            o4[0] = (u[0] + u[1]) + u[2]; o4[cout] = u[1] + u[2]; o4[2 * cout] = u[0] + u[1]; o4[3 * cout] = u[1];
-        }
-    }
+    rank1b_block(Rank1bBlock{J.in, J.wgt_r1f, J.out, J.w, J.tiles_per_img, J.n_tiles_n, bid - J.block_begin, args.B, args.cin, args.cout, args.r1_slices}, lds_dyn);
 }
 bool rank1b_takes(const ConvArgs& a) {
     if (a.cin % kR1Chunk != 0) return false;
@@ -608,6 +522,31 @@
     }
 }
 
+static int rank1b_grid(ConvArgs& a) {
+    int blocks = 0;
+    for (int j = 0; j < a.njobs; ++j) {
+        ConvJob& J = a.job[j];
+        J.tiles_x = J.tiles_per_img = (J.w + 31) / 32;
+        J.n_tiles_n = (a.cout + 31) / 32;
+        J.block_begin = blocks;
+        blocks += J.tiles_per_img * a.B * J.n_tiles_n * (a.r1_slices > 1 ? a.r1_slices : 1);
+    }
+    return blocks;
+}
+bool rank1b_rider(ConvArgs& a, ConvRider& r) {
+    if (conv_use_naive() || a.njobs < 1 || a.njobs > kMaxConvJobs || !rank1b_takes(a)) return false;
+    const int blocks = rank1b_grid(a);
+    if (blocks <= 0 || blocks > 3 * device_cus()) return false;
+    r.kind = RIDER_RANK1B; r.n_blocks = blocks; r.gx = 0; r.tile_ranged = 0;
+    Rank1bArgs& q = r.r1b;
+    q.njobs = a.njobs; q.B = a.B; q.cin = a.cin; q.cout = a.cout; q.r1_slices = a.r1_slices;
+    for (int j = 0; j < kMaxConvJobs; ++j) {
+        const ConvJob& J = a.job[j < a.njobs ? j : 0];
+        q.job[j] = Rank1bJob{J.in, J.wgt_r1f, J.out, J.w, J.tiles_per_img, J.n_tiles_n, J.block_begin};
+    }
+    return true;
+}
+
 int launch_rank1(ConvArgs& a, hipStream_t st, bool roll3) {
     S3D_CHECK(a.njobs >= 1 && a.njobs <= kMaxConvJobs && a.cin % KC == 0, S3D_ERR_INVALID, "rank1: bad arguments");
     S3D_CHECK(a.r1_slices <= 1 || (roll3 && !conv_use_naive() && a.r1_slices == 2 && a.cin % kR1Chunk == 0 && a.cin >= 2 * kR1Chunk), S3D_ERR_INVALID, "rank1: two K slices of whole 128-channel chunks");
@@ -618,14 +557,7 @@
         return 0;
     }
     if (roll3 && rank1b_takes(a)) {
-        int blocks = 0;
-        for (int j = 0; j < a.njobs; ++j) {
-            ConvJob& J = a.job[j];
-            J.tiles_x = J.tiles_per_img = (J.w + 31) / 32;
-            J.n_tiles_n = (a.cout + 31) / 32;
-            J.block_begin = blocks;
-            blocks += J.tiles_per_img * a.B * J.n_tiles_n * (a.r1_slices > 1 ? a.r1_slices : 1);
-        }
+        const int blocks = rank1b_grid(a);
         if (!blocks) return 0;
         conv_note_kernel("k_rank1b (three-tap rollout tables, fragment-order weights)");
         hipLaunchKernelGGL(k_rank1b, dim3(blocks), dim3(256), kR1bLdsFloats * sizeof(float), st, a);
@@ -694,34 +626,44 @@
 }
 
 static const char* rider_name(int kind) {
-    return kind == RIDER_GN_PARTIALS_UP ? "k_conv_mfma<1x1> direct MFMA convolution carrying k_gn_partials_up"
+    return kind == RIDER_RANK1B ? "k_conv_mfma<1x1> direct MFMA convolution carrying k_rank1b"
+         : kind == RIDER_GN_PARTIALS_UP ? "k_conv_mfma<1x1> direct MFMA convolution carrying k_gn_partials_up"
          : kind == RIDER_GN_FINALIZE ? "k_conv_mfma<1x1> direct MFMA convolution carrying k_gn_finalize (plain)"
                                      : "k_conv_mfma<1x1> direct MFMA convolution carrying k_gn_finalize_cat";
 }
 template <class CFG>
 static int launch_cfg(ConvArgs& a, hipStream_t st, const ConvRider* rider = nullptr) {
     int blocks = 0;
+    ConvRider r;
+    if (rider) r = *rider;
+    const bool ranged = rider && rider->tile_ranged;
     for (int j = 0; j < a.njobs; ++j) {
         ConvJob& J = a.job[j];
         J.tiles_x = (J.w + CFG::TW - 1) / CFG::TW;
         J.tiles_per_img = J.tiles_x * ((J.h + CFG::TH - 1) / CFG::TH);
         J.n_tiles_n = (a.cout + CFG::BN - 1) / CFG::BN;
         J.block_begin = blocks;
-        blocks += J.tiles_per_img * J.n_tiles_n * a.B;
+        if (!ranged) { r.tile_begin[j] = 0; r.tile_count[j] = J.tiles_per_img; }
+        S3D_CHECK(r.tile_begin[j] >= 0 && r.tile_count[j] >= 0 && r.tile_begin[j] + r.tile_count[j] <= J.tiles_per_img, S3D_ERR_INVALID, "conv: tiles [%d, +%d) of %d", r.tile_begin[j], r.tile_count[j], J.tiles_per_img);
+        blocks += r.tile_count[j] * J.n_tiles_n * a.B;
         S3D_CHECK((long long)J.h * J.w * a.cout < (1LL << 32), S3D_ERR_INVALID, "conv: a plane of one sample must stay below 2^32 elements");
     }
-    if (!blocks) return 0;
+    const int rider_blocks = rider && rider->kind != RIDER_NONE ? rider->n_blocks : 0;
+    if (!blocks && rider_blocks <= 0) return 0;
     a.xcd_swizzle = 1;
     conv_note_kernel(CFG::KH == 3 ? "k_conv_mfma<3x3> direct MFMA convolution" : (CFG::KH == 1 ? (CFG::TR ? "k_conv_mfma<1x1, transposed accumulators> direct MFMA convolution" : "k_conv_mfma<1x1> direct MFMA convolution") : "k_conv_mfma<5x5> direct MFMA convolution"));
     if constexpr (CFG::KH == 1 && !CFG::TR) {
-        if (rider && rider->n_blocks > 0) {
-            conv_note_kernel(rider_name(rider->kind));
-            hipLaunchKernelGGL((k_conv_mfma<CFG, true>), dim3(blocks + rider->n_blocks), dim3(256), 0, st, a, RiderArg<true>{*rider});
+        if (rider_blocks > 0 || ranged) {
+            r.n_blocks = rider_blocks;
+            if (rider_blocks > 0) conv_note_kernel(rider_name(r.kind));
+            if (r.kind == RIDER_RANK1B) hipLaunchKernelGGL((k_conv_mfma<CFG, 2>), dim3(blocks + rider_blocks), dim3(256), 0, st, a, RiderArg<2>{r});
+            else hipLaunchKernelGGL((k_conv_mfma<CFG, 1>), dim3(blocks + rider_blocks), dim3(256), 0, st, a, RiderArg<1>{r});
             S3D_HIP(hipGetLastError());
             return 0;
         }
     }
-    hipLaunchKernelGGL(k_conv_mfma<CFG>, dim3(blocks), dim3(256), 0, st, a, RiderArg<false>());
+    S3D_CHECK(!ranged, S3D_ERR_INTERNAL, "conv: a tile range on a launch that is not the default 1x1 form");
+    hipLaunchKernelGGL(k_conv_mfma<CFG>, dim3(blocks), dim3(256), 0, st, a, RiderArg<0>());
     S3D_HIP(hipGetLastError());
     return 0;
 }
@@ -745,10 +687,13 @@
     const int tr_mode = opt(OPT_CONV1X1_T);
     return tr_mode != 0 && cout % 4 == 0 && (tr_mode == 1 || blocks >= 4 * 768);
 }
+void conv1x1_tiles(const Geo& g, int tiles[3]) {
+    for (int p = 0; p < 3; ++p) tiles[p] = ((g.w[p] + 7) / 8) * ((g.h[p] + 7) / 8);
+}
 static long long conv1x1_blocks(const Geo& g, int B, int cout) {
-    long long blocks = 0;
-    for (int p = 0; p < 3; ++p) blocks += (long long)((g.w[p] + 7) / 8) * ((g.h[p] + 7) / 8) * ((cout + 63) / 64) * B;
-    return blocks;
+    int tiles[3];
+    conv1x1_tiles(g, tiles);
+    return (long long)(tiles[0] + tiles[1] + tiles[2]) * ((cout + 63) / 64) * B;
 }
 bool conv1x1_takes_rider(const Geo& g, int B, int cout) {
     return riders_enabled() && !conv_use_naive() && opt(OPT_CONV1X1_T) == kOptUnset && !conv1x1_transposed(cout, conv1x1_blocks(g, B, cout));
diff --git a/sin3dm_amd/csrc/s3d_kernels.hip b/sin3dm_amd/csrc/s3d_kernels.hip
--- a/sin3dm_amd/csrc/s3d_kernels.hip
+++ b/sin3dm_amd/csrc/s3d_kernels.hip
@@ -251,7 +251,7 @@
 bool gn_finalize_rider(const GnPartials& part, const Geo& g, int C, int B, GnStats out, ConvRider& r) {
     memset(&r, 0, sizeof r);
     if (!B || !gn_finalize_args(part, g, C, out, r.fin)) return false;
-    r.kind = RIDER_GN_FINALIZE; r.gx = 32; r.n_blocks = 32 * 3 * B;
+    r.kind = RIDER_GN_FINALIZE; r.gx = 32; r.n_blocks = 32 * 3 * B; r.tile_ranged = 0;
     return true;
 }
 int launch_gn_finalize(const GnPartials& part, const Geo& g, int C, int B, GnStats out, hipStream_t st) {
@@ -311,7 +311,7 @@
     int maxtiles = 0;
     if (!gn_partials_up_args(u, sg, out, r.up, maxtiles) || !maxtiles || !B) return false;
     if (r.up.cq * r.up.pl != 256 || size_t(r.up.pl) * r.up.C * 2 * sizeof(double) > size_t(kRiderLdsBytes)) return false;
-    r.kind = RIDER_GN_PARTIALS_UP; r.gx = maxtiles; r.n_blocks = maxtiles * 3 * B;
+    r.kind = RIDER_GN_PARTIALS_UP; r.gx = maxtiles; r.n_blocks = maxtiles * 3 * B; r.tile_ranged = 0;
     return true;
 }
 __global__ __launch_bounds__(256) void k_gn_finalize_cat(GnFinCatArgs a) {
@@ -328,7 +328,7 @@
 bool gn_finalize_cat_rider(const GnPartials& pu, const GnPartials& ps, const Geo& g, int C, int B, GnStats out, ConvRider& r) {
     memset(&r, 0, sizeof r);
     if (!B || !gn_finalize_cat_args(pu, ps, g, C, out, r.cat)) return false;
-    r.kind = RIDER_GN_FINALIZE_CAT; r.gx = 32; r.n_blocks = 32 * 3 * B;
+    r.kind = RIDER_GN_FINALIZE_CAT; r.gx = 32; r.n_blocks = 32 * 3 * B; r.tile_ranged = 0;
     return true;
 }
 int launch_gn_finalize_cat(const GnPartials& pu, const GnPartials& ps, const Geo& g, int C, int B, GnStats out, hipStream_t st) {
diff --git a/sin3dm_amd/csrc/s3d_model.h b/sin3dm_amd/csrc/s3d_model.h
--- a/sin3dm_amd/csrc/s3d_model.h
+++ b/sin3dm_amd/csrc/s3d_model.h
@@ -261,9 +261,8 @@
         }
         return 0;
     }
-    int rank1_tables(const Tri& y, const ConvW& cw, const MeanPartials& mp, const MeanVecs& mv, const float* const rrow[3], const float* const rcol[3]) {
-        S3D_TRY(launch_means_finalize(y.g, y.C, B, mp, mv, st));
-        ConvArgs ca; memset(&ca, 0, sizeof ca);
+    void rank1_args(const Tri& y, const ConvW& cw, const MeanVecs& mv, const float* const rrow[3], const float* const rcol[3], ConvArgs& ca) const {
+        memset(&ca, 0, sizeof ca);
         ca.B = B; ca.cin = y.C; ca.cout = cw.cout; ca.njobs = 6;
         ca.r1_slices = r1_slices_for(y, cw);
         const float* rowvec[3] = {mv.rowmean[1], mv.rowmean[0], mv.colmean[0]};
@@ -276,7 +275,32 @@
             jc.in = colvec[p]; jc.wgt = m->dev(cw.rcol[p]); jc.out = const_cast<float*>(rcol[p]); jc.h = 1; jc.w = y.g.w[p];
             jc.wgt_r1f = cw.rcol_f[p] ? m->dev(cw.rcol_f[p]) : nullptr;
         }
+    }
+    struct R1Host { const Tri* y; const ConvW* cw; const Tri* res_up; const Tri* out; int lo, hi; };
+    const R1Host* r1_host = nullptr;
+    int rank1_tables(const Tri& y, const ConvW& cw, const MeanPartials& mp, const MeanVecs& mv, const float* const rrow[3], const float* const rcol[3]) {
+        S3D_TRY(launch_means_finalize(y.g, y.C, B, mp, mv, st));
+        ConvArgs ca;
+        rank1_args(y, cw, mv, rrow, rcol, ca);
+        if (r1_host) {
+            const R1Host h = *r1_host;
+            r1_host = nullptr;
+            ConvRider r;
+            const bool carried = rank1b_rider(ca, r);
+            S3D_TRY(conv1x1_piece(*h.y, *h.cw, h.res_up, *h.out, h.lo, h.hi, carried ? &r : nullptr));
+            if (carried) return 0;
+        }
         return m->timed_conv(2, CONV_1x3_ROLL, ca, st);
+    }
+    int rank1b_rider_blocks(int C, const Geo& g, const ConvW& cw) const {
+        if (!cw.rollout) return 0;
+        Tri y; y.C = C; y.g = g;
+        const MeanVecs mv{};
+        const float* const none[3] = {nullptr, nullptr, nullptr};
+        ConvArgs ca;
+        rank1_args(y, cw, mv, none, none, ca);
+        ConvRider r;
+        return rank1b_rider(ca, r) ? r.n_blocks : 0;
     }
     int norm_act(const Tri& x, const NormW& nw, const float* film_ptr, const ConvW* cw, Tri& y, const float* rrow[3],
                  const float* rcol[3], NormTape* nt = nullptr) {
@@ -307,6 +331,18 @@
 
     bool riders_on() const { return !tape && riders_enabled() && opt_on(OPT_VCAT); }
     bool rides(const ConvW& cw, const Geo& g) const { return riders_on() && cw.k == 1 && conv1x1_takes_rider(g, B, cw.cout); }
+    bool skip_split_cuts(const ResBlockW& rb, int C, const Geo& g, int cut[3]) const {
+        const int nb1 = rank1b_rider_blocks(C, g, rb.c1), nb2 = rank1b_rider_blocks(rb.c1.cout, g, rb.c2);
+        if (!nb1 || !nb2) return false;
+        int tiles[3];
+        conv1x1_tiles(g, tiles);
+        const int T = tiles[0] + tiles[1] + tiles[2], per_tile = (rb.skip_b.cout + 63) / 64 * B, slots = 3 * device_cus();
+        const bool forced = skip_split_mode() == 1;
+        if (!forced && (long long)T * per_tile < slots) return false;
+        const int n2 = forced ? T / 3 : T / 4, n1 = forced ? T / 3 : T - n2;
+        cut[0] = T - n1 - n2; cut[1] = T - n2; cut[2] = T;
+        return true;
+    }
 
     int conv(const Tri& y, const ConvW& cw, const float* bbias, const float* const rrow[3], const float* const rcol[3],
              const Tri* res, Tri& out, int want_stats = 0, hipStream_t on = nullptr, bool no_bias = false, bool res_up = false,
@@ -347,6 +383,25 @@
         return 0;
     }
 
+    int conv1x1_piece(const Tri& y, const ConvW& cw, const Tri* res_up, const Tri& out, int lo, int hi, const ConvRider* rider) {
+        ConvArgs ca; memset(&ca, 0, sizeof ca);
+        ca.B = B; ca.cin = cw.cin; ca.cout = cw.cout; ca.njobs = 3; ca.r1_slices = 1;
+        ConvRider r;
+        if (rider) r = *rider;
+        else { r.kind = RIDER_NONE; r.n_blocks = 0; r.gx = 0; }
+        r.tile_ranged = 1;
+        int tiles[3];
+        conv1x1_tiles(y.g, tiles);
+        for (int p = 0, t0 = 0; p < 3; t0 += tiles[p], ++p) {
+            ConvJob& J = ca.job[p];
+            J.in = y.p[p]; J.wgt = m->dev(cw.dense[p]); J.bias = m->dev(cw.bias[p]); J.bbias_stride = fstride();
+            J.res = res_up ? res_up->p[p] : nullptr; J.res_up = res_up ? 1 : 0; J.out = out.p[p]; J.h = y.g.h[p]; J.w = y.g.w[p];
+            const int a = std::max(lo, t0), b = std::min(hi, t0 + tiles[p]);
+            r.tile_begin[p] = b > a ? a - t0 : 0; r.tile_count[p] = b > a ? b - a : 0;
+        }
+        return m->timed_conv(1, CONV_1x1, ca, st, &r);
+    }
+
     int resblock_cat(const ResBlockW& rb, const Tri& u, const Tri& sk, Tri& out, int out_stats) {
         const bool ssn = m->cfg.use_scale_shift_norm != 0;
         const float* film_ptr = film ? film + rb.film_off : nullptr;
@@ -362,8 +417,15 @@
         ConvRider r_up, r_fin;
         const bool up_rides = !measuring && rides(rb.skip_a, u.g) && gn_partials_up_rider(u, B, sg, pu, r_up);
         const bool fin_rides = up_rides && rides(rb.skip_b, sk.g) && gn_finalize_cat_rider(pu, sk.part, sk.g, C, B, stats, r_fin);
+        int cut[3] = {0, 0, 0};
+        const bool split = fin_rides && skip_split_mode() != 0 && skip_split_cuts(rb, C, sk.g, cut);
         S3D_TRY(conv(u, rb.skip_a, nullptr, nullptr, nullptr, nullptr, z, 0, nullptr, true, false, up_rides ? &r_up : nullptr));
+        if (split) {
+            skip = alloc_tri(rb.skip_b.cout, sk.g);
+            S3D_TRY(conv1x1_piece(sk, rb.skip_b, &z, skip, 0, cut[0], &r_fin));
+        } else
         S3D_TRY(conv(sk, rb.skip_b, nullptr, nullptr, nullptr, &z, skip, 0, nullptr, false, true, fin_rides ? &r_fin : nullptr));
+        const R1Host host1{&sk, &rb.skip_b, &z, &skip, cut[0], cut[1]}, host2{&sk, &rb.skip_b, &z, &skip, cut[1], cut[2]};
         if (!measuring) {
             if (!up_rides) S3D_TRY(launch_gn_partials_up(u, B, sg, pu, st));
             if (!fin_rides) S3D_TRY(launch_gn_finalize_cat(pu, sk.part, sk.g, C, B, stats, st));
@@ -380,10 +442,12 @@
             S3D_TRY(roll_buffers(y1, rb.c1, roll, mp, mv, rr, rc));
             if (!measuring) {
                 S3D_TRY(launch_gn_act_cat(u, sk, B, stats, aa, y1, roll ? &mp : nullptr, st));
+                if (split) r1_host = &host1;
                 if (roll) S3D_TRY(rank1_tables(y1, rb.c1, mp, mv, rr, rc));
             }
         }
         S3D_TRY(conv(y1, rb.c1, ssn ? nullptr : film_ptr, rr, rc, nullptr, h1, 2));
+        if (split) r1_host = &host2;
         S3D_TRY(norm_act(h1, rb.n2, ssn ? film_ptr : nullptr, &rb.c2, y2, rr, rc, nullptr));
         S3D_TRY(conv(y2, rb.c2, nullptr, rr, rc, &skip, out, out_stats));
         return 0;
diff --git a/sin3dm_amd/csrc/s3d_riders.h b/sin3dm_amd/csrc/s3d_riders.h
--- a/sin3dm_amd/csrc/s3d_riders.h
+++ b/sin3dm_amd/csrc/s3d_riders.h
@@ -1,5 +1,6 @@
 #pragma once
 #include "s3d_common.h"
+#include "s3d_rank1.h"
 
 namespace s3d {
 
@@ -127,6 +128,111 @@
     }
 }
 
+__device__ __forceinline__ void rank1b_block(const Rank1bBlock& K, float* lds_dyn) {
+    const int L = K.L, cin = K.cin, cout = K.cout, B = K.B;
+    int local = K.local;
+    const int mtile = local % K.tiles_per_img; local /= K.tiles_per_img;
+    const int b = local % B; local /= B;
+    const int g = local % K.n_tiles_n, sl = local / K.n_tiles_n;
+    const int nchunks = cin / kR1Chunk;
+    int chunk0 = 0, nch = nchunks;
+    if (K.r1_slices > 1) { const int first = (nchunks + 1) / 2; chunk0 = sl ? first : 0; nch = sl ? nchunks - first : first; }
+    const int csl = nch * kR1Chunk, ld = csl + 4;
+    const int tid = threadIdx.x, lane = tid & 63, wid = __builtin_amdgcn_readfirstlane(tid >> 6), i = lane & 31, half = lane >> 5;
+    const int nsteps = nch * 12;
+    const r1_f32x4* pf = reinterpret_cast<const r1_f32x4*>(K.wgt_r1f) + (size_t(g * 4 + wid) * (nchunks * 12) + chunk0 * 12) * 192 + lane;
+    constexpr int D = 3;
+    r1_f32x4 ring[D][3];
+    int pf_s = 0;
+    auto prefetch = [&](int slot) {
+        ring[slot][0] = ((r1_gf4ptr)(uintptr_t)pf)[0];
+        ring[slot][1] = ((r1_gf4ptr)(uintptr_t)(pf + 64))[0];
+        ring[slot][2] = ((r1_gf4ptr)(uintptr_t)(pf + 128))[0];
+        ++pf_s;
+        pf += pf_s < nsteps ? 192 : 0;
+    };
+#pragma unroll
+    for (int d = 0; d < D; ++d) prefetch(d);
+    {
+        const int q4 = csl / 4, items = 34 * q4;
+        const float* vb = K.in + (size_t(b) * L) * cin + chunk0 * kR1Chunk;
+        const r1_f32x4 zero4 = {0.f, 0.f, 0.f, 0.f};
+        for (int it0 = tid; it0 < items; it0 += 256 * 5) {
+            r1_f32x4 v[5];
+#pragma unroll
+            for (int u = 0; u < 5; ++u) {
+                const int it = it0 + 256 * u, row = it / q4, q = it - row * q4, pos = mtile * 32 - 1 + row;
+                const bool ok = it < items && pos >= 0 && pos < L;
+                v[u] = ((r1_gf4ptr)(uintptr_t)(vb + size_t(ok ? pos : 0) * cin + (ok ? q : 0) * 4))[0];
+                if (!ok) v[u] = zero4;
+            }
+#pragma unroll
+            for (int u = 0; u < 5; ++u) {
+                const int it = it0 + 256 * u, row = it / q4, q = it - row * q4;
+                if (it < items) *reinterpret_cast<r1_f32x4*>(lds_dyn + row * ld + q * 4) = v[u];
+            }
+        }
+    }
+    __syncthreads();
+    r1_f32x16 q[3];
+#pragma unroll
+    for (int o = 0; o < 3; ++o)
+#pragma unroll
+        for (int r = 0; r < 16; ++r) q[o][r] = 0.f;
+    const float* Ab = lds_dyn + i * ld + half * 4 + wid * 32;
+    for (int ch = 0; ch < nch; ++ch) {
+        const float* Ac = Ab + ch * kR1Chunk;
+#pragma unroll
+        for (int st = 0; st < 12; ++st) {
+            const int tap = st >> 2, k8 = st & 3;
+            const r1_f32x4 a4 = *reinterpret_cast<const r1_f32x4*>(Ac + tap * ld + k8 * 8);
+            r1_f32x4 b4[3];
+#pragma unroll
+            for (int o = 0; o < 3; ++o) b4[o] = ring[st % D][o];
+            __builtin_amdgcn_sched_barrier(0);
+#pragma unroll
+            for (int e = 0; e < 4; ++e)
+#pragma unroll
+                for (int o = 0; o < 3; ++o) q[o] = __builtin_amdgcn_mfma_f32_32x32x2f32(a4[e], b4[o][e], q[o], 0, 0, 0);
+            __builtin_amdgcn_sched_barrier(0);
+            prefetch(st % D);
+            __builtin_amdgcn_sched_barrier(0);
+        }
+    }
+    __syncthreads();
+    float* red = lds_dyn;
+#pragma unroll
+    for (int o = 0; o < 3; ++o)
+#pragma unroll
+        for (int r = 0; r < 16; ++r) red[((wid * 3 + o) * 16 + r) * 64 + lane] = q[o][r];
+    __syncthreads();
+    float* out = K.out + size_t(sl) * B * L * 4 * cout;
+#pragma unroll
+    for (int k = 0; k < 4; ++k) {
+        const int it = tid + 256 * k, r = it >> 6, l = it & 63;
+        float u[3];
+#pragma unroll
+        for (int o = 0; o < 3; ++o) {
+            const float* p = red + (o * 16 + r) * 64 + l;
+            u[o] = ((p[0] + p[3 * 1024]) + p[2 * 3 * 1024]) + p[3 * 3 * 1024];
+        }
+        const int row = mtile * 32 + (r & 3) + 8 * (r >> 2) + 4 * (l >> 5), co = g * 32 + (l & 31);
+        if (row < L && co < cout) {
+            float* o4 = out + (size_t(b) * L + row) * 4 * cout + co;
+            o4[0] = (u[0] + u[1]) + u[2]; o4[cout] = u[1] + u[2]; o4[2 * cout] = u[0] + u[1]; o4[3 * cout] = u[1];
+        }
+    }
+}
+__device__ __forceinline__ void run_rank1b_rider(const ConvRider& r, int bid, float* lds) {
+    const Rank1bArgs& a = r.r1b;
+    if ((r.n_blocks & 7) == 0) bid = (bid & 7) * (r.n_blocks >> 3) + (bid >> 3);
+    int j = 0;
+#pragma unroll
+    for (int k = 1; k < kMaxConvJobs; ++k) j += (k < a.njobs && bid >= a.job[k].block_begin) ? 1 : 0;
+    const Rank1bJob& J = a.job[j];
+    rank1b_block(Rank1bBlock{J.in, J.wgt_r1f, J.out, J.w, J.tiles_per_img, J.n_tiles_n, bid - J.block_begin, a.B, a.cin, a.cout, a.r1_slices}, lds);
+}
+
 __device__ __forceinline__ void run_rider(const ConvRider& r, int idx, void* lds) {
     const int x = idx % r.gx, p = (idx / r.gx) % 3, b = idx / (3 * r.gx);
     double* sm = static_cast<double*>(lds);
diff --git a/sin3dm_amd/csrc/s3d_runtime.hip b/sin3dm_amd/csrc/s3d_runtime.hip
--- a/sin3dm_amd/csrc/s3d_runtime.hip
+++ b/sin3dm_amd/csrc/s3d_runtime.hip
@@ -79,6 +79,17 @@
     }
     return v != 0;
 }
+static std::atomic<int> g_skip_split{-2};
+int skip_split_mode() {
+    int v = g_skip_split.load(std::memory_order_acquire);
+    if (v == -2) {
+        const char* e = getenv("S3D_SKIP_SPLIT");
+        int expect = -2;
+        g_skip_split.compare_exchange_strong(expect, e && strcmp(e, "0") == 0 ? 0 : (e && strcmp(e, "1") == 0 ? 1 : kOptUnset), std::memory_order_acq_rel);
+        v = g_skip_split.load(std::memory_order_acquire);
+    }
+    return v;
+}
 int device_cus() {
     static std::atomic<int> cache[64];
     int dev = 0;
@@ -118,6 +129,11 @@
 
 int s3d_set_riders(int on) {
     s3d::g_riders.store(on ? 1 : 0, std::memory_order_release);
+    return 0;
+}
+
+int s3d_set_skip_split(int mode) {
+    s3d::g_skip_split.store(mode == 0 ? 0 : (mode == 1 ? 1 : s3d::kOptUnset), std::memory_order_release);
     return 0;
 }
 
```

After: 1.201 samples/s, median of 6. About the same (+0.6%).
